# pinellolab/CRISPR-HAWK

Measured on AMD Instinct MI355X. Metric: candidate guides scored/sec, higher is better.
Workload: dtype u32

## Files before the change

### crispr-hawk_amd/csrc/hawk_api_collapse.hip

```cpp
#include <hip/hip_runtime.h>

#include <algorithm>
#include <cmath>
#include <cstdio>
#include <cstdlib>
#include <cstring>
#include <map>
#include <mutex>
#include <new>
#include <unordered_map>
#include <vector>

#include "hawk_host.h"

extern "C" {

static int collapse_rows(hawk_table* t, uint32_t flank_up, uint32_t flank_down, uint64_t* n_groups, float* kernel_ms);
static int collapse_by_templates(hawk_table* t, uint32_t flank_up, uint32_t flank_down, uint64_t* n_groups, float* kernel_ms);
int hawk_table_collapse_ex(hawk_table* t, uint32_t flank_up, uint32_t flank_down, uint64_t* n_groups, float* kernel_ms) {
  if (!t || !n_groups || !t->hs || hawk_table_stale(t)) return HAWK_E_INVALID;
  if (flank_up > HAWK_PAD || flank_down > HAWK_PAD) return HAWK_E_UNSUPPORTED;
  if (t->by_cluster && t->n_rows) return collapse_by_templates(t, flank_up, flank_down, n_groups, kernel_ms);
  return collapse_rows(t, flank_up, flank_down, n_groups, kernel_ms);
}
static int collapse_rows(hawk_table* t, uint32_t flank_up, uint32_t flank_down, uint64_t* n_groups, float* kernel_ms) {
  hawk_hapset* hs = t->hs;
  hawk_ctx* ctx = hs->ctx;
  HIPCHK(hipSetDevice(ctx->device));
  const uint64_t n = t->n_rows;
  t->collapsed = false;
  *n_groups = 0;
  if (kernel_ms) *kernel_ms = 0.f;
  hs->collapse_gen = t->gen;
  if (n == 0) { t->n_groups = 0; t->collapsed = true; return HAWK_OK; }
  if (n > 0xffffffffull || hs->max_gen - hs->min_gen > 0xffffffffll) return HAWK_E_UNSUPPORTED;
  unsigned end_bit = 32;
  while (end_bit < 64 && ((uint64_t)(hs->max_gen - hs->min_gen) >> (end_bit - 32)) != 0) ++end_bit;
  const unsigned pos_bits = end_bit - 31;
  const unsigned hash_bits = std::min(31u, (pos_bits + 24 + 7) / 8 * 8 - pos_bits);
  const unsigned begin_bit = 31 - hash_bits;
  const size_t temp_bytes = hawk_collapse_temp_bytes(n, begin_bit, end_bit);
  int rc;
  if ((rc = hs->ckeys.reserve(2 * n * 8)) || (rc = hs->cvals.reserve(2 * n * 4)) || (rc = hs->cflags.reserve(n * 4)) ||
      (rc = hs->cgidx.reserve(n * 4)) || (rc = hs->ctemp.reserve(temp_bytes + 16)) || (rc = hs->cgoff.reserve((n + 1) * 8)) ||
      (rc = hs->cgc.reserve(2 * n)) || (rc = hs->ccnt.reserve(32)))
    return rc;
  const char* ex = getenv("HAWK_COLLAPSE_EXACT");
#ifdef HAWK_TEST_HOOKS
  const char* vf = getenv("HAWK_COLLAPSE_VERIFY");
  const char* wk = getenv("HAWK_COLLAPSE_WEAK_HASH");
  const bool verify = !(vf && vf[0] == '0'), weak = wk && wk[0] == '1';
#else
  const bool verify = true, weak = false;
#endif
  bool exact = ex && ex[0] == '1';
  for (int round = 0; round < 2; ++round, exact = true) {
  if (exact && (rc = hs->cfull.reserve(hawk_collapse_full_bytes(n)))) return rc;
  bool verified_bad = false;
  {
    const char* md = getenv("HAWK_COLLAPSE_MODE");
    const bool force_hash = md && md[0] == 'h', force_sort = md && md[0] == 's';
    const uint64_t g_est = hs->last_groups ? hs->last_groups + hs->last_groups / 4 : n / 16;
    uint64_t C = 1024;
    while (C < 2 * g_est) C <<= 1;
    const bool fits = C <= (1ull << 26) && hs->max_gen - hs->min_gen < 0xffffffffll;
    const bool want = !exact && !weak && !force_sort && fits && (force_hash || (n >= (1u << 20) && (hs->last_groups == 0 || hs->last_groups * 8 <= n)));
    if (want) {
      const size_t tb = hawk_collapse_hash_temp_bytes(n, (uint32_t)C);
      if ((rc = hs->ctable.reserve(C * 16)) || (rc = hs->cocc.reserve(C * 4)) || (rc = hs->cdense.reserve(C * 4)) ||
          (rc = hs->cgkey.reserve(2 * C * 8)) || (rc = hs->cgslot.reserve(2 * C * 4)) || (rc = hs->ctemp.reserve(std::max(tb, temp_bytes) + 16)) ||
          (rc = hs->ccnt.reserve(32)))
        return rc;
      for (int attempt = 0; attempt < 2; ++attempt) {
        unsigned long long hc[4] = {0, 0, 0, 0};
        HIPCHK(hipMemsetAsync(hs->ccnt.p, 0, 32, ctx->stream));
        HIPCHK(hipEventRecord(ctx->ev[0], ctx->stream));
        if (hawk_launch_collapse_hash1(ctx->stream, t->cols, hs->d_is_ref, n, (int)t->guidelen, (int)t->pamlen, (int)flank_up, (int)flank_down,
                                       hs->min_gen, 0x9e3779b97f4a7c15ull * (uint64_t)(attempt + 1), hs->ctemp.p, tb, hs->ctable.p, (uint32_t)C,
                                       hs->cocc.as<uint32_t>(), hs->cdense.as<uint32_t>(), hs->cgkey.as<uint64_t>(), hs->cgslot.as<uint32_t>(),
                                       hs->cflags.as<uint32_t>(), hs->ccnt.as<unsigned long long>()))
          return HAWK_E_HIP;
        HIPCHK(hipGetLastError());
        HIPCHK(hipMemcpyAsync(hc, hs->ccnt.p, 24, hipMemcpyDeviceToHost, ctx->stream));
        HIPCHK(hipStreamSynchronize(ctx->stream));
        if (hc[1]) { hs->last_groups = n; if (hs->plan_groups) *hs->plan_groups = n; break; }
        if (hc[0]) continue;
        const uint64_t ng = hc[2];
        if (hawk_launch_collapse_hash2(ctx->stream, t->cols, n, (uint32_t)ng, (int)t->guidelen, (int)t->pamlen, (int)t->right, end_bit, hs->ctemp.p, tb,
                                       hs->cgkey.as<uint64_t>(), hs->cgslot.as<uint32_t>(), (uint32_t)C, hs->cocc.as<uint32_t>(),
                                       hs->cflags.as<uint32_t>(), hs->ckeys.as<uint32_t>(), hs->cvals.as<uint32_t>(), hs->cgoff.as<uint64_t>(),
                                       hs->cgc.as<uint8_t>(), hs->cgc.as<uint8_t>() + n))
          return HAWK_E_HIP;
        if (verify) {
          if ((rc = hs->cfull.reserve(ng * 64 + 64))) return rc;
          hawk_launch_collapse_verify_rows(ctx->stream, t->cols, hs->d_is_ref, n, (uint32_t)ng, (int)t->guidelen, (int)t->pamlen, (int)flank_up,
                                           (int)flank_down, hs->cvals.as<uint32_t>() + n, hs->cflags.as<uint32_t>(), hs->cocc.as<uint32_t>(),
                                           hs->cgoff.as<uint64_t>(), hs->cfull.p, hs->ccnt.as<unsigned long long>() + 3);
        }
        HIPCHK(hipEventRecord(ctx->ev[1], ctx->stream));
        HIPCHK(hipGetLastError());
        HIPCHK(hipMemcpyAsync(hs->cgoff.as<uint64_t>() + ng, &n, 8, hipMemcpyHostToDevice, ctx->stream));
        HIPCHK(hipMemcpyAsync(&hc[3], hs->ccnt.as<unsigned long long>() + 3, 8, hipMemcpyDeviceToHost, ctx->stream));
        HIPCHK(hipStreamSynchronize(ctx->stream));
        if (kernel_ms) { float ms = 0.f; (void)hipEventElapsedTime(&ms, ctx->ev[0], ctx->ev[1]); *kernel_ms += ms; }
        if (hc[3]) { verified_bad = true; break; }
        hs->last_groups = ng;
        if (hs->plan_groups) *hs->plan_groups = ng;
        t->n_groups = ng; t->collapsed = true;
        *n_groups = ng;
        return HAWK_OK;
      }
    }
  }
  if (verified_bad) continue;
  unsigned long long cnt[3] = {0, 0, 0};
  for (int attempt = 0; attempt < 4; ++attempt) {
    HIPCHK(hipMemsetAsync(hs->ccnt.p, 0, 32, ctx->stream));
    HIPCHK(hipEventRecord(ctx->ev[0], ctx->stream));
    if (hawk_launch_collapse(ctx->stream, t->cols, hs->d_is_ref, n, (int)t->guidelen, (int)t->pamlen, (int)t->right, (int)flank_up,
                             (int)flank_down, hs->min_gen, begin_bit, end_bit, 0x9e3779b97f4a7c15ull * (uint64_t)(attempt + 1), hs->ctemp.p,
                             temp_bytes, hs->ckeys.as<uint64_t>(), hs->cvals.as<uint32_t>(), hs->cflags.as<uint32_t>(),
                             hs->cgidx.as<uint32_t>(), hs->ccnt.as<unsigned long long>(), hs->cgoff.as<uint64_t>(), hs->cgc.as<uint8_t>(),
                             hs->cgc.as<uint8_t>() + n, hs->cgidx.as<uint32_t>(), exact ? hs->cfull.p : nullptr, weak && !exact))
      return HAWK_E_HIP;
    if (verify && !exact)
      hawk_launch_collapse_verify(ctx->stream, t->cols, hs->d_is_ref, n, (int)t->guidelen, (int)t->pamlen, (int)flank_up, (int)flank_down,
                                  hs->cvals.as<uint32_t>() + n, hs->cgidx.as<uint32_t>(), hs->cflags.as<uint32_t>(), hs->cgoff.as<uint64_t>(),
                                  hs->ccnt.as<unsigned long long>() + 2);
    HIPCHK(hipEventRecord(ctx->ev[1], ctx->stream));
    HIPCHK(hipGetLastError());
    HIPCHK(hipMemcpyAsync(cnt, hs->ccnt.p, 24, hipMemcpyDeviceToHost, ctx->stream));
    HIPCHK(hipStreamSynchronize(ctx->stream));
    if (kernel_ms) { float ms = 0.f; (void)hipEventElapsedTime(&ms, ctx->ev[0], ctx->ev[1]); *kernel_ms += ms; }
    if (cnt[0] == cnt[1]) break;
  }
  if (cnt[0] != cnt[1]) { if (!exact) continue; return HAWK_E_UNSUPPORTED; }
  if (cnt[2]) continue;
  const uint64_t ng = cnt[1];
  HIPCHK(hipMemcpyAsync(hs->cgoff.as<uint64_t>() + ng, &n, 8, hipMemcpyHostToDevice, ctx->stream));
  HIPCHK(hipStreamSynchronize(ctx->stream));
  hs->last_groups = ng;
  if (hs->plan_groups) *hs->plan_groups = ng;
  t->n_groups = ng; t->collapsed = true;
  *n_groups = ng;
  return HAWK_OK;
  }
  return HAWK_E_UNSUPPORTED;
}

static int collapse_by_templates(hawk_table* t, uint32_t flank_up, uint32_t flank_down, uint64_t* n_groups, float* kernel_ms) {
  hawk_hapset* hs = t->hs;
  hawk_ctx* ctx = hs->ctx;
  HIPCHK(hipSetDevice(ctx->device));
  const hawk_xplan* vx = hs->vplan;
  if (!vx || !vx->cl.usable) return HAWK_E_INVALID;
  const uint64_t n = t->n_rows;
  if (n > 0xffffffffull) return HAWK_E_UNSUPPORTED;
  t->collapsed = false;
  *n_groups = 0;
  if (kernel_ms) *kernel_ms = 0.f;
  const uint32_t nu = vx->cl.n_uniq;
  PoolScope tmp;
  uint32_t* d_ucnt;
  uint64_t* d_moff;
  unsigned long long *d_partial, *d_shards;
  ScanTotals* d_tot;
  TEMPCHK(tmp, &d_ucnt, (size_t)std::max<uint32_t>(nu, 1) * 4);
  TEMPCHK(tmp, &d_moff, ((size_t)nu + 2) * 8);
  TEMPCHK(tmp, &d_partial, ((size_t)nu / 1024 + 2) * 8);
  TEMPCHK(tmp, &d_shards, 512 * 8);
  TEMPCHK(tmp, &d_tot, sizeof(ScanTotals));
  HIPCHK(hipMemsetAsync(d_shards, 0, 512 * 8, ctx->stream));
  HIPCHK(hipMemsetAsync(d_tot, 0, sizeof(ScanTotals), ctx->stream));
  uint64_t r0 = 0;
  ScanTotals tot;
  memset(&tot, 0, sizeof(tot));
  if (nu) {
    hawk_launch_cc_ucnt(ctx->stream, hs->cs_res.p, nu, d_ucnt);
    hawk_launch_mscan(ctx->stream, d_ucnt, nu, d_partial, d_shards, d_moff, d_tot);
    HIPCHK(hipMemcpyAsync(&tot, d_tot, sizeof(tot), hipMemcpyDeviceToHost, ctx->stream));
  }
  HIPCHK(hipMemcpyAsync(&r0, hs->offsets.as<uint64_t>() + t->plane_tiles, 8, hipMemcpyDeviceToHost, ctx->stream));
  HIPCHK(hipStreamSynchronize(ctx->stream));
  HIPCHK(hipGetLastError());
  const uint64_t t_live = tot.n_keep;
  const uint64_t nm = r0 + t_live;
  if (r0 > n || nm == 0 || nm > 0xffffffffull || r0 + 0 > n) return HAWK_E_INVALID;
  int rc;
  GuideCols mini;
  if ((rc = hawk_reserve_cols(hs->cmini, nm, &mini)) || (rc = hs->cm_gid.reserve(nm * 4))) return rc;
  float ms_a = 0.f, ms_b = 0.f, ms_c = 0.f;
  HIPCHK(hipEventRecord(ctx->ev[8], ctx->stream));
  hawk_launch_cc_mini(ctx->stream, t->cols, r0, hs->cs_trows.p, t_live, d_moff, hs->cs_tbase.as<uint32_t>(), nu, hs->ref_startp, mini);
  HIPCHK(hipEventRecord(ctx->ev[9], ctx->stream));
  HIPCHK(hipGetLastError());
  {
    const size_t tb_full = hawk_collapse_expand_temp_bytes(n);
    if ((rc = hs->ckeys.reserve(std::max<size_t>(2 * nm * 8, 2 * n * 4))) || (rc = hs->cvals.reserve(2 * n * 4)) ||
        (rc = hs->cgoff.reserve((nm + 1) * 8)) || (rc = hs->cgc.reserve(2 * n)) || (rc = hs->ctemp.reserve(tb_full + 16)) ||
        (rc = hs->cflags.reserve(n * 4)))
      return rc;
  }
  hawk_table tm;
  tm.hs = hs; tm.ctx = ctx; tm.n_rows = nm; tm.n_cand = tm.n_hits = 0; tm.cap = mini.cap; tm.cols = mini;
  tm.guidelen = t->guidelen; tm.pamlen = t->pamlen; tm.right = t->right; tm.n_groups = 0; tm.collapsed = false; tm.gen = t->gen;
  uint64_t G = 0;
  if ((rc = collapse_rows(&tm, flank_up, flank_down, &G, &ms_b))) return rc;
  HIPCHK(hipStreamSynchronize(ctx->stream));
  (void)hipEventElapsedTime(&ms_a, ctx->ev[8], ctx->ev[9]);
  unsigned gbits = 1;
  while (gbits < 32 && (G >> gbits) != 0) ++gbits;
  const size_t tb = hawk_collapse_expand_temp_bytes(n);
  HIPCHK(hipEventRecord(ctx->ev[8], ctx->stream));
  hawk_launch_cc_gidm(ctx->stream, hs->cvals.as<uint32_t>() + nm, hs->cgoff.as<uint64_t>(), nm, G, hs->cm_gid.as<uint32_t>());
  if ((rc = hs->ckeys.reserve(2 * n * 4)) || (rc = hs->cvals.reserve(2 * n * 4)) || (rc = hs->cgoff.reserve((std::max<uint64_t>(G, nm) + 1) * 8)) ||
      (rc = hs->cgc.reserve(2 * n)) || (rc = hs->ctemp.reserve(tb + 16)) || (rc = hs->cflags.reserve(n * 4)))
    return rc;
  ClDict cd;
  memset(&cd, 0, sizeof(cd));
  cd.n_inst = vx->cl.n_inst; cd.n_uniq = vx->cl.n_uniq; cd.inst_uid = vx->cl.inst_uid.as<uint32_t>();
  hawk_launch_cs_gid(ctx->stream, cd, hs->cs_res.p, d_moff, hs->offsets.as<uint64_t>() + t->plane_tiles, r0, n,
                     hs->cm_gid.as<uint32_t>(), hs->ckeys.as<uint32_t>(), hs->cvals.as<uint32_t>());
  if (hawk_launch_collapse_expand(ctx->stream, t->cols, n, gbits, (int)t->guidelen, (int)t->pamlen, (int)t->right, hs->ctemp.p, tb, hs->ckeys.as<uint32_t>(),
                                  hs->cvals.as<uint32_t>(), hs->cgoff.as<uint64_t>(), hs->cgc.as<uint8_t>(), hs->cgc.as<uint8_t>() + n))
    return HAWK_E_HIP;
  HIPCHK(hipMemcpyAsync(hs->cgoff.as<uint64_t>() + G, &n, 8, hipMemcpyHostToDevice, ctx->stream));
  HIPCHK(hipEventRecord(ctx->ev[9], ctx->stream));
  HIPCHK(hipGetLastError());
  HIPCHK(hipStreamSynchronize(ctx->stream));
  (void)hipEventElapsedTime(&ms_c, ctx->ev[8], ctx->ev[9]);
  if (kernel_ms) *kernel_ms = ms_a + ms_b + ms_c;
  hs->collapse_gen = t->gen;
  hs->last_groups = G;
  if (hs->plan_groups) *hs->plan_groups = G;
  t->n_groups = G; t->collapsed = true;
  *n_groups = G;
  return HAWK_OK;
}

int hawk_table_collapse(hawk_table* t, uint64_t* n_groups, float* kernel_ms) {
  return hawk_table_collapse_ex(t, 0, 0, n_groups, kernel_ms);
}

static bool collapse_valid(const hawk_table* t) {
  return t && t->collapsed && t->hs && !hawk_table_stale(t) && t->hs->collapse_gen == t->gen;
}

int hawk_table_collapse_download(hawk_table* t, uint32_t* perm, uint64_t* group_off, uint8_t* gc_num, uint8_t* gc_den) {
  if (!collapse_valid(t)) return HAWK_E_INVALID;
  hawk_hapset* hs = t->hs;
  hawk_ctx* ctx = hs->ctx;
  HIPCHK(hipSetDevice(ctx->device));
  const uint64_t n = t->n_rows, ng = t->n_groups;
  if (n == 0) { if (group_off) group_off[0] = 0; return HAWK_OK; }
  if (perm) HIPCHK(hipMemcpyAsync(perm, hs->cvals.as<uint32_t>() + n, n * 4, hipMemcpyDefault, ctx->stream));
  if (group_off) HIPCHK(hipMemcpyAsync(group_off, hs->cgoff.p, (ng + 1) * 8, hipMemcpyDefault, ctx->stream));
  if (gc_num) HIPCHK(hipMemcpyAsync(gc_num, hs->cgc.p, ng, hipMemcpyDefault, ctx->stream));
  if (gc_den) HIPCHK(hipMemcpyAsync(gc_den, hs->cgc.as<uint8_t>() + n, ng, hipMemcpyDefault, ctx->stream));
  HIPCHK(hipStreamSynchronize(ctx->stream));
  return HAWK_OK;
}

int hawk_table_collapse_export(hawk_table* t, uint32_t* rep_row, uint32_t* pos, uint8_t* strand, int64_t* start, int64_t* stop,
                               uint8_t* flags, double* cfdon, uint64_t* win, uint32_t* member_hap, float* kernel_ms) {
  if (!collapse_valid(t)) return HAWK_E_INVALID;
  hawk_hapset* hs = t->hs;
  hawk_ctx* ctx = hs->ctx;
  HIPCHK(hipSetDevice(ctx->device));
  const uint64_t n = t->n_rows, ng = t->n_groups;
  if (kernel_ms) *kernel_ms = 0.f;
  if (n == 0) return HAWK_OK;
  GuideCols rep;
  int rc = hawk_reserve_cols(hs->crep, ng, &rep);
  if (rc) return rc;
  uint32_t* d_mem = hs->cflags.as<uint32_t>();
  HIPCHK(hipEventRecord(ctx->ev[0], ctx->stream));
  hawk_launch_collapse_export(ctx->stream, t->cols, n, ng, hs->cvals.as<uint32_t>() + n, hs->cgoff.as<uint64_t>(), rep, d_mem);
  HIPCHK(hipEventRecord(ctx->ev[1], ctx->stream));
  HIPCHK(hipGetLastError());
  hipStream_t st = ctx->stream;
  if (rep_row) HIPCHK(hipMemcpyAsync(rep_row, rep.hap, ng * 4, hipMemcpyDefault, st));
  if (pos) HIPCHK(hipMemcpyAsync(pos, rep.pos, ng * 4, hipMemcpyDefault, st));
  if (strand) HIPCHK(hipMemcpyAsync(strand, rep.strand, ng, hipMemcpyDefault, st));
  if (start) HIPCHK(hipMemcpyAsync(start, rep.start, ng * 8, hipMemcpyDefault, st));
  if (stop) HIPCHK(hipMemcpyAsync(stop, rep.stop, ng * 8, hipMemcpyDefault, st));
  if (flags) HIPCHK(hipMemcpyAsync(flags, rep.flags, ng, hipMemcpyDefault, st));
  if (cfdon) HIPCHK(hipMemcpyAsync(cfdon, rep.cfdon, ng * 8, hipMemcpyDefault, st));
  if (win)
    for (int p = 0; p < HAWK_PLANES; ++p)
      HIPCHK(hipMemcpyAsync(win + (size_t)p * ng, rep.win + (size_t)p * rep.cap, ng * 8, hipMemcpyDefault, st));
  if (member_hap) HIPCHK(hipMemcpyAsync(member_hap, d_mem, n * 4, hipMemcpyDefault, st));
  HIPCHK(hipStreamSynchronize(st));
  if (kernel_ms) (void)hipEventElapsedTime(kernel_ms, ctx->ev[0], ctx->ev[1]);
  return HAWK_OK;
}


}
```

### crispr-hawk_amd/csrc/hawk_api_search.hip

```cpp
#include <hip/hip_runtime.h>

#include <algorithm>
#include <cmath>
#include <cstdio>
#include <cstdlib>
#include <cstring>
#include <map>
#include <mutex>
#include <new>
#include <unordered_map>
#include <vector>

#include "hawk_host.h"

int hawk_reserve_cols(DevBuf (&b)[8], uint64_t cap, GuideCols* c) {
  int rc;
  const size_t sz[8] = {cap * 4, cap * 4, cap, cap * 8, cap * 8, cap, cap * 8, cap * 8 * HAWK_PLANES};
  for (int i = 0; i < 8; ++i) if ((rc = b[i].reserve(std::max<size_t>(sz[i], 16)))) return rc;
  c->hap = b[0].as<uint32_t>(); c->pos = b[1].as<uint32_t>(); c->strand = b[2].as<uint8_t>();
  c->start = b[3].as<int64_t>(); c->stop = b[4].as<int64_t>(); c->flags = b[5].as<uint8_t>();
  c->cfdon = b[6].as<double>(); c->win = b[7].as<uint64_t>(); c->cap = cap;
  c->rows = nullptr; c->startp = 0;
  return HAWK_OK;
}
extern "C" {

#define HAWK_RETRY_TEMPLATES (-100)
static int hawk_search_once(hawk_hapset* hs, const hawk_search_params* p, hawk_table** out, hawk_timing* timing);
int hawk_search(hawk_hapset* hs, const hawk_search_params* p, hawk_table** out, hawk_timing* timing) {
  int rc = hawk_search_once(hs, p, out, timing);
  if (rc == HAWK_RETRY_TEMPLATES) rc = hawk_search_once(hs, p, out, timing);
  return rc == HAWK_RETRY_TEMPLATES ? HAWK_E_CAPACITY : rc;
}
static int hawk_search_once(hawk_hapset* hs, const hawk_search_params* p, hawk_table** out, hawk_timing* timing) {
  if (!hs || !p || !out || !hs->has_meta) return HAWK_E_INVALID;
  if (p->score_cfdon > 2) return HAWK_E_INVALID;
  if (p->score_cfdon && (p->right || !p->cfd_mm || !p->cfd_pam || p->pamlen < 2)) return HAWK_E_INVALID;
  hawk_ctx* ctx = hs->ctx;
  HIPCHK(hipSetDevice(ctx->device));
  ScanParams sp;
  int rc = make_scan_params(hs, p->pam_fwd, p->pam_rev, p->pamlen, p->guidelen, p->right, true, &sp);
  if (rc) return rc;
  const HapSetDev d = make_dev(hs);
  ++hs->cols_gen;
  const uint64_t ntile = (uint64_t)hs->n_hap * sp.bph;
  bool by_cluster = hs->vplan && hs->vplan->cl.built && hs->vplan->cl.usable && hs->ref_index == 0;
  if (by_cluster) { const char* e = getenv("HAWK_VIEW_SEARCH"); if (e && e[0] == 'w') by_cluster = false; }
  const uint64_t nscan = by_cluster ? (uint64_t)sp.bph + ((uint64_t)hs->vplan->cl.n_inst + 63) / 64 : ntile;
  if ((rc = hs->counts.reserve(nscan * 4)) || (rc = hs->offsets.reserve((nscan + 1) * 8)) ||
      (rc = hs->misc.reserve(512 * 8 + 64)) ||
      (rc = hs->cfd.reserve(336 * 8)) || (rc = hs->partial.reserve((nscan / 1024 + 2) * 8)))
    return rc;
  const hawk_xplan* vx = hs->vplan;
  const uint32_t plane_tiles = vx ? sp.bph * (hs->ref_index == 0 ? 1u : 0u) : (uint32_t)ntile;
  if (vx && (hs->ref_index != 0 || hs->n_ref_rows != 1)) return HAWK_E_INVALID;
  const uint64_t n_ref_tiles = (uint64_t)sp.bph * hs->n_ref_rows;
  if ((rc = hs->lists.reserve((size_t)plane_tiles * HAWK_LIST_CAP * 4 + 16)) || (rc = hs->big.reserve(((size_t)plane_tiles + 128 * n_ref_tiles) * 8 + 16))) return rc;
  uint32_t* const d_lists = hs->lists.as<uint32_t>();
  unsigned long long* const d_big = hs->big.as<unsigned long long>();
  if (p->score_cfdon) {
    if (hs->cfd_host.size() != 336 || memcmp(hs->cfd_host.data(), p->cfd_mm, 320 * 8) != 0 ||
        memcmp(hs->cfd_host.data() + 320, p->cfd_pam, 16 * 8) != 0) {
      hs->cfd_host.assign(336, 0.0);
      memcpy(hs->cfd_host.data(), p->cfd_mm, 320 * 8);
      memcpy(hs->cfd_host.data() + 320, p->cfd_pam, 16 * 8);
      HIPCHK(hipMemcpyAsync(hs->cfd.p, hs->cfd_host.data(), 336 * 8, hipMemcpyHostToDevice, ctx->stream));
      HIPCHK(hipStreamSynchronize(ctx->stream));
    }
  }
  HIPCHK(hipMemsetAsync(hs->misc.p, 0, 512 * 8 + 64, ctx->stream));
  unsigned long long* d_shards = hs->misc.as<unsigned long long>();
  int* d_status = reinterpret_cast<int*>(hs->misc.as<char>() + 512 * 8);
  uint32_t* d_big_count = reinterpret_cast<uint32_t*>(hs->misc.as<char>() + 512 * 8 + 16);
  unsigned long long* d_tcount = reinterpret_cast<unsigned long long*>(hs->misc.as<char>() + 512 * 8 + 8);
  static_assert(sizeof(ScanTotals) == 32, "status block layout");
  ScanTotals* d_totals = reinterpret_cast<ScanTotals*>(hs->misc.as<char>() + 512 * 8 + 32);
  const char* d_block = hs->misc.as<char>() + 512 * 8;
  char* h_block = static_cast<char*>(ctx->pinned);
  GuideParams gp;
  gp.pamlen = sp.pamlen; gp.guidelen = sp.guidelen; gp.right = sp.right; gp.L = sp.L;
  gp.score_cfdon = (int32_t)p->score_cfdon;
  gp.cfd_mm = hs->cfd.as<double>(); gp.cfd_pam = hs->cfd.as<double>() + 320; gp.bph = sp.bph;
  RefInfo ri;
  ri.index = hs->ref_index; ri.startp = hs->ref_startp;
  for (int s = 0; s < 2; ++s) {
    ri.lo[s] = 0; ri.hi[s] = 0;
    if (hs->ref_index >= 0) {
      const bool pamfirst = (sp.right != 0) != (s != 0);
      const int po = pamfirst ? 0 : sp.guidelen;
      const int haplen = (int)hs->hap_len[hs->ref_index];
      const int rs = hs->has_partner ? hs->partner_start : hs->scan_start[hs->ref_index];
      const int re = hs->has_partner ? hs->partner_stop : hs->scan_stop[hs->ref_index];
      ri.lo[s] = std::max(rs - po, HAWK_PAD);
      ri.hi[s] = std::min(re - po, haplen - sp.L - HAWK_PAD + 1);
    }
  }
  ri.bits[0] = ri.bits[1] = nullptr;
  ri.n_bits = 0;
  if (hs->ref_index >= 0) {
    const uint64_t key[6] = {p->pam_fwd, p->pam_rev, ((uint64_t)p->pamlen << 32) | p->guidelen, (uint64_t)(p->right ? 1 : 0),
                             ((uint64_t)(uint32_t)ri.lo[0] << 32) | (uint32_t)ri.hi[0], ((uint64_t)(uint32_t)ri.lo[1] << 32) | (uint32_t)ri.hi[1]};
    if ((rc = hs->refbits.reserve((size_t)hs->S * 4 * 2))) return rc;
    ri.bits[0] = hs->refbits.as<uint32_t>();
    ri.bits[1] = hs->refbits.as<uint32_t>() + hs->S;
    ri.n_bits = hs->S * 32u;
    if (vx && ((rc = hs->refhp.reserve(((size_t)hs->S + 1) * 8 * 2)) || (rc = hs->vcnt0.reserve(by_cluster ? 16 : ntile * 4)))) return rc;
    if (!hs->refbits_valid || memcmp(hs->refbits_key, key, sizeof(key)) != 0) {
      hawk_launch_ref_bits(ctx->stream, d, sp, ri, hs->refbits.as<uint32_t>(), hs->refbits.as<uint32_t>() + hs->S);
      if (vx) hawk_launch_ref_hits(ctx->stream, d, sp, hs->ref_index, hs->refhp.p);
      HIPCHK(hipGetLastError());
      memcpy(hs->refbits_key, key, sizeof(key));
      hs->refbits_valid = true;
    }
  }
  VcArgs va;
  memset(&va, 0, sizeof(va));
  if (vx) {
    for (int pl = 0; pl < 4; ++pl) va.ref[pl] = vx->ref5[pl].as<uint32_t>();
    va.ref_S = hs->S;
    va.recs_ = vx->recs.p; va.alt_codes = vx->codes.as<uint8_t>(); va.hv_off = vx->off.as<uint64_t>(); va.tiles_ = vx->tiles.p;
    va.hp = hs->refhp.as<uint4>();
  }
  const uint32_t v_tiles = vx ? (uint32_t)ntile - plane_tiles : 0u;
  ClDict cd;
  memset(&cd, 0, sizeof(cd));
  uint64_t tcap = 0, t_rows_used = 0;
  if (by_cluster) {
    const auto& cl = vx->cl;
    cd.n_inst = cl.n_inst; cd.n_uniq = cl.n_uniq;
    cd.inst_uid = cl.inst_uid.as<uint32_t>(); cd.inst_o = cl.inst_o.as<int32_t>(); cd.inst_row = cl.inst_row.as<uint32_t>();
    cd.inst_pa = cl.inst_pa.as<int32_t>(); cd.inst_rb = cl.inst_rb.as<int32_t>();
    cd.u_rec = cl.u_rec.as<uint32_t>(); cd.u_n = cl.u_n.as<uint32_t>(); cd.u_row = cl.u_row.as<uint32_t>(); cd.u_o = cl.u_o.as<int32_t>();
    cd.u_seg = cl.u_seg.as<uint32_t>();
    const char* e0 = getenv("HAWK_CLUSTER_ROWS0");
    const uint64_t first = e0 ? strtoull(e0, nullptr, 10) : 16ull * cl.n_uniq + 65536;
    tcap = std::max<uint64_t>(std::min<uint64_t>(cl.slots, std::max<uint64_t>(hs->cs_tcap, first)), 1);
    if ((rc = hs->cs_res.reserve((size_t)std::max<uint32_t>(cl.n_uniq, 1) * 32)) || (rc = hs->cs_tbase.reserve((size_t)std::max<uint32_t>(cl.n_uniq, 1) * 4)) ||
        (rc = hs->cs_trows.reserve((size_t)tcap * hawk_cs_row_bytes())) || (rc = hs->cs_itb.reserve((size_t)std::max<uint32_t>(cl.n_inst, 1) * 4)) ||
        (rc = hs->cs_icnt.reserve((size_t)std::max<uint32_t>(cl.n_inst, 1) * 4)))
      return rc;
  }
  uint32_t* const d_counts_v = hs->counts.as<uint32_t>() + plane_tiles;
  auto view_count = [&]() {
    if (by_cluster) {
      hawk_launch_cs_templates(ctx->stream, d, va, cd, sp, gp, ri, hs->cs_res.p, hs->cs_tbase.as<uint32_t>(), hs->cs_trows.p, d_tcount, tcap, d_status);
      (void)hipEventRecord(ctx->ev[8], ctx->stream);
      hawk_launch_cs_count(ctx->stream, d, va, cd, sp, hs->cs_res.p, d_tcount, tcap, d_counts_v, hs->cs_icnt.as<uint32_t>(),
                           hs->cs_itb.as<uint32_t>(), d_shards);
    } else {
      hawk_launch_vsearch(ctx->stream, 0, d, va, sp, gp, ri, hs->d_tile_meta, hs->counts.as<uint32_t>(), hs->vcnt0.as<uint32_t>(), d_shards, nullptr,
                          GuideCols{}, d_status, plane_tiles, v_tiles);
    }
  };
  const uint64_t stage_cap = by_cluster ? 2ull * hs->hap_len[hs->ref_index] + 64 : 0;
  auto emit_all = [&](const GuideCols& cols, const GuideCols& packed) {
    hawk_launch_search(ctx->stream, 1, d, sp, gp, ri, hs->d_tile_meta, hs->counts.as<uint32_t>(), d_shards,
                       hs->offsets.as<uint64_t>(), cols, d_status, d_lists, d_big_count, d_big, ctx->ev[5], plane_tiles);
    if (!vx) return;
    (void)hipEventRecord(ctx->ev[7], ctx->stream);
    if (by_cluster) {
      hawk_launch_rows_pack(ctx->stream, cols, hs->offsets.as<uint64_t>() + plane_tiles, 0, std::min<uint64_t>(stage_cap, packed.cap), packed.rows,
                            packed.startp, d_status);
      (void)hipEventRecord(ctx->ev[9], ctx->stream);
      hawk_launch_cs_emit_rows(ctx->stream, cd, hs->cs_icnt.as<uint32_t>(), hs->cs_itb.as<uint32_t>(), hs->cs_trows.p, hs->offsets.as<uint64_t>() + plane_tiles,
                               d_tcount, tcap, packed.rows, packed.cap, d_status);
    } else {
      hawk_launch_vsearch(ctx->stream, 1, d, va, sp, gp, ri, hs->d_tile_meta, hs->counts.as<uint32_t>(), hs->vcnt0.as<uint32_t>(), d_shards,
                          hs->offsets.as<uint64_t>(), cols, d_status, plane_tiles, v_tiles);
    }
  };
  auto reserve_table = [&](uint64_t cap, GuideCols* cols, GuideCols* table) -> int {
    int r;
    if (!by_cluster) {
      if ((r = hawk_reserve_cols(hs->colsA, cap, cols))) return r;
      *table = *cols;
      return HAWK_OK;
    }
    if ((r = hawk_reserve_cols(hs->colsA, stage_cap, cols)) || (r = hs->rowsA.reserve(cap * 64))) return r;
    memset(table, 0, sizeof(*table));
    table->rows = hs->rowsA.as<uint4>(); table->cap = cap; table->startp = ri.startp;
    return HAWK_OK;
  };
  uint64_t& table_cap = by_cluster ? hs->rows_cap : hs->cols_cap;
  GuideCols none = {};
  hipEvent_t* ev = ctx->ev;
  HIPCHK(hipEventRecord(ev[0], ctx->stream));
  hawk_launch_search(ctx->stream, 0, d, sp, gp, ri, hs->d_tile_meta, hs->counts.as<uint32_t>(), d_shards, nullptr, none, d_status, d_lists, d_big_count, d_big,
                     nullptr, plane_tiles);
  if (vx) HIPCHK(hipEventRecord(ev[6], ctx->stream));
  if (vx) view_count();
  HIPCHK(hipEventRecord(ev[1], ctx->stream));
  hawk_launch_mscan(ctx->stream, hs->counts.as<uint32_t>(), nscan, hs->partial.as<unsigned long long>(), d_shards,
                    hs->offsets.as<uint64_t>(), d_totals);
  HIPCHK(hipEventRecord(ev[2], ctx->stream));
  HIPCHK(hipGetLastError());
  ScanTotals tot;
  GuideCols ca, tc;
  int status = 0;
  uint64_t nrows = 0;
  bool emitted = false;
  auto read_block = [&]() -> int {
    HIPCHK(hipMemcpyAsync(h_block, d_block, 64, hipMemcpyDeviceToHost, ctx->stream));
    HIPCHK(hipStreamSynchronize(ctx->stream));
    memcpy(&tot, h_block + 32, sizeof(tot));
    memcpy(&status, h_block, 4);
    if (!by_cluster) return HAWK_OK;
    uint64_t tcu;
    memcpy(&tcu, h_block + 8, 8);
    if (tcu > tcap) { hs->cs_tcap = std::min<uint64_t>(vx->cl.slots, tcu + tcu / 8 + 64); return HAWK_RETRY_TEMPLATES; }
    t_rows_used = tcu;
    return HAWK_OK;
  };
  if (table_cap) {
    if ((rc = reserve_table(table_cap, &ca, &tc))) return rc;
    HIPCHK(hipEventRecord(ev[3], ctx->stream));
    emit_all(ca, tc);
    HIPCHK(hipEventRecord(ev[4], ctx->stream));
    HIPCHK(hipGetLastError());
    if ((rc = read_block())) return rc;
    nrows = tot.n_keep;
    emitted = nrows <= table_cap;
    if (!emitted) {
      if (status && status != HAWK_E_CAPACITY) return status;
      status = 0;
      HIPCHK(hipMemsetAsync(d_status, 0, 4, ctx->stream));
    }
  } else {
    if ((rc = read_block())) return rc;
    if (status) return status;
    nrows = tot.n_keep;
  }
  if (!emitted) {
    if ((rc = reserve_table(std::max<uint64_t>(std::max<uint64_t>(nrows, 1), table_cap), &ca, &tc))) return rc;
    table_cap = tc.cap;
    HIPCHK(hipEventRecord(ev[3], ctx->stream));
    if (nrows) emit_all(ca, tc);
    HIPCHK(hipEventRecord(ev[4], ctx->stream));
    HIPCHK(hipGetLastError());
    HIPCHK(hipMemcpyAsync(h_block, d_status, 4, hipMemcpyDeviceToHost, ctx->stream));
    HIPCHK(hipStreamSynchronize(ctx->stream));
    memcpy(&status, h_block, 4);
  }
  if (timing) {
    memset(timing, 0, sizeof(*timing));
    (void)hipEventElapsedTime(&timing->count_ms, ev[0], ev[1]);
    (void)hipEventElapsedTime(&timing->offsets_ms, ev[1], ev[2]);
    (void)hipEventElapsedTime(&timing->emit_ms, ev[3], ev[4]);
    if (nrows) (void)hipEventElapsedTime(&timing->emit_list_ms, ev[3], ev[5]);
    (void)hipEventElapsedTime(&timing->total_ms, ev[0], ev[4]);
    if (vx) {
      (void)hipEventElapsedTime(&timing->v_count_ms, ev[6], ev[1]);
      if (nrows) (void)hipEventElapsedTime(&timing->v_emit_ms, ev[7], ev[4]);
      timing->v_path = by_cluster ? 2u : 1u;
      if (by_cluster) (void)hipEventElapsedTime(&timing->v_templates_ms, ev[6], ev[8]);
      if (by_cluster && nrows) (void)hipEventElapsedTime(&timing->v_emit_rows_ms, ev[9], ev[4]);
    }
    uint64_t pos = 0;
    for (uint32_t h = 0; h < hs->n_hap; ++h) pos += (uint64_t)std::max(0, hs->scan_stop[h] - hs->scan_start[h]);
    timing->scanned_positions = pos;
  }
  if (status) return status;
  hawk_table* t = new (std::nothrow) hawk_table();
  if (!t) return HAWK_E_INVALID;
  t->hs = hs; t->ctx = ctx; t->gen = hs->cols_gen;
  t->n_rows = nrows; t->n_cand = tot.n_cand; t->n_hits = tot.n_hits; t->cols = tc; t->cap = tc.cap;
  t->guidelen = p->guidelen; t->pamlen = p->pamlen; t->right = p->right ? 1 : 0; t->n_groups = 0; t->collapsed = false;
  t->by_cluster = by_cluster; t->plane_tiles = plane_tiles; t->t_rows = by_cluster ? t_rows_used : 0;
  *out = t;
  return HAWK_OK;
}

void hawk_table_destroy(hawk_table* t) {
  if (!t) return;
  if (!t->hs) {
    (void)hipSetDevice(t->ctx->device);
    (void)hipStreamSynchronize(t->ctx->stream);
    for (auto& b : t->own) b.release();
  }
  delete t;
}

int hawk_table_counts(const hawk_table* t, uint64_t* n_rows, uint64_t* n_candidates, uint64_t* n_hits) {
  if (!t) return HAWK_E_INVALID;
  if (n_rows) *n_rows = t->n_rows;
  if (n_candidates) *n_candidates = t->n_cand;
  if (n_hits) *n_hits = t->n_hits;
  return HAWK_OK;
}

int hawk_table_download(hawk_table* t, uint32_t* hap, uint32_t* pos, uint8_t* strand, int64_t* start, int64_t* stop,
                        uint8_t* flags, double* cfdon, uint64_t* win) {
  if (!t || hawk_table_stale(t)) return HAWK_E_INVALID;
  hawk_ctx* ctx = t->ctx;
  HIPCHK(hipSetDevice(ctx->device));
  const uint64_t n = t->n_rows;
  if (!n) return HAWK_OK;
  GuideCols c = t->cols;
  PoolScope tmp;
  if (c.rows) {
    GuideCols u;
    memset(&u, 0, sizeof(u));
    u.cap = n;
    if (hap) TEMPCHK(tmp, &u.hap, n * 4);
    if (pos) TEMPCHK(tmp, &u.pos, n * 4);
    if (strand) TEMPCHK(tmp, &u.strand, n);
    if (start) TEMPCHK(tmp, &u.start, n * 8);
    if (stop) TEMPCHK(tmp, &u.stop, n * 8);
    if (flags) TEMPCHK(tmp, &u.flags, n);
    if (cfdon) TEMPCHK(tmp, &u.cfdon, n * 8);
    if (win) TEMPCHK(tmp, &u.win, n * 8 * HAWK_PLANES);
    hawk_launch_rows_unpack(ctx->stream, c.rows, n, c.startp, u);
    HIPCHK(hipGetLastError());
    c = u;
  }
  if (hap) HIPCHK(hipMemcpyAsync(hap, c.hap, n * 4, hipMemcpyDefault, ctx->stream));
  if (pos) HIPCHK(hipMemcpyAsync(pos, c.pos, n * 4, hipMemcpyDefault, ctx->stream));
  if (strand) HIPCHK(hipMemcpyAsync(strand, c.strand, n, hipMemcpyDefault, ctx->stream));
  if (start) HIPCHK(hipMemcpyAsync(start, c.start, n * 8, hipMemcpyDefault, ctx->stream));
  if (stop) HIPCHK(hipMemcpyAsync(stop, c.stop, n * 8, hipMemcpyDefault, ctx->stream));
  if (flags) HIPCHK(hipMemcpyAsync(flags, c.flags, n, hipMemcpyDefault, ctx->stream));
  if (cfdon) HIPCHK(hipMemcpyAsync(cfdon, c.cfdon, n * 8, hipMemcpyDefault, ctx->stream));
  if (win)
    for (int p = 0; p < HAWK_PLANES; ++p)
      HIPCHK(hipMemcpyAsync(win + (size_t)p * n, c.win + (size_t)p * c.cap, n * 8, hipMemcpyDefault, ctx->stream));
  HIPCHK(hipStreamSynchronize(ctx->stream));
  return HAWK_OK;
}

int hawk_table_layout(const hawk_table* t, uint32_t* layout, int64_t* startp) {
  if (!t || !layout) return HAWK_E_INVALID;
  *layout = t->cols.rows ? HAWK_LAYOUT_ROWS : HAWK_LAYOUT_COLUMNS;
  if (startp) *startp = t->cols.rows ? t->cols.startp : 0;
  return HAWK_OK;
}

int hawk_table_download_rows(hawk_table* t, void* rows64) {
  if (!t || hawk_table_stale(t) || !rows64) return HAWK_E_INVALID;
  if (!t->cols.rows) return HAWK_E_UNSUPPORTED;
  HIPCHK(hipSetDevice(t->ctx->device));
  if (t->n_rows) HIPCHK(hipMemcpyAsync(rows64, t->cols.rows, t->n_rows * 64, hipMemcpyDefault, t->ctx->stream));
  HIPCHK(hipStreamSynchronize(t->ctx->stream));
  return HAWK_OK;
}

int hawk_table_device_rows(hawk_table* t, void** rows64, int64_t* startp) {
  if (!t || hawk_table_stale(t) || !rows64) return HAWK_E_INVALID;
  if (!t->cols.rows) return HAWK_E_UNSUPPORTED;
  *rows64 = t->cols.rows;
  if (startp) *startp = t->cols.startp;
  return HAWK_OK;
}

int hawk_table_device_columns(hawk_table* t, void** hap, void** pos, void** strand, void** start, void** stop,
                              void** flags, void** cfdon, void** win, uint64_t* win_plane_stride) {
  if (!t || hawk_table_stale(t)) return HAWK_E_INVALID;
  const GuideCols& c = t->cols;
  if (c.rows) return HAWK_E_UNSUPPORTED;
  if (hap) *hap = c.hap;
  if (pos) *pos = c.pos;
  if (strand) *strand = c.strand;
  if (start) *start = c.start;
  if (stop) *stop = c.stop;
  if (flags) *flags = c.flags;
  if (cfdon) *cfdon = c.cfdon;
  if (win) *win = c.win;
  if (win_plane_stride) *win_plane_stride = c.cap;
  return HAWK_OK;
}

}
```

### crispr-hawk_amd/csrc/hawk_api_xplan.hip

```cpp
#include <hip/hip_runtime.h>

#include <algorithm>
#include <cmath>
#include <cstdio>
#include <cstdlib>
#include <cstring>
#include <map>
#include <mutex>
#include <new>
#include <unordered_map>
#include <vector>

#include "hawk_host.h"

extern "C" {

void hawk_xplan_destroy(hawk_xplan* x) {
  if (!x) return;
  (void)hipSetDevice(x->ctx->device);
  (void)hipStreamSynchronize(x->ctx->stream);
  for (auto& p : x->ref_plane) hawk_pool_free(p);
  for (auto& b : x->ref5) b.release();
  DevBuf* bufs[] = {&x->recs, &x->heads, &x->tiles, &x->codes, &x->off, &x->hlen, &x->hash,
                    &x->m_is_ref, &x->m_ss, &x->m_se, &x->m_seg_off, &x->m_seg_rel, &x->m_seg_gen, &x->m_tile,
                    &x->cl.inst_uid, &x->cl.inst_o, &x->cl.inst_row, &x->cl.inst_pa, &x->cl.inst_rb, &x->cl.u_rec, &x->cl.u_n, &x->cl.u_row,
                    &x->cl.u_o, &x->cl.u_seg};
  for (auto* b : bufs) b->release();
  delete x;
}

static int xplan_build(hawk_hapset* ref_set, uint32_t n_var, const uint32_t* v_r0, const uint32_t* v_span, const uint32_t* v_alt_off,
                       const uint32_t* v_alt_len, const uint8_t* alt_codes, uint32_t alt_codes_len, uint32_t n_hap, const uint64_t* hv_off,
                       const uint32_t* d_idx, const int32_t* d_o, const uint32_t* hap_len, uint32_t maxlen, hawk_xplan** out) {
  hawk_ctx* ctx = ref_set->ctx;
  const uint32_t ref_len = ref_set->hap_len[0];
  const uint64_t ncar = hv_off[n_hap];
  HIPCHK(hipSetDevice(ctx->device));
  hawk_xplan* x = new (std::nothrow) hawk_xplan();
  if (!x) return HAWK_E_INVALID;
  x->ctx = ctx; x->n_var = n_var; x->n_hap = n_hap; x->ref_len = ref_len; x->ncar = ncar;
  x->hap_len.assign(hap_len, hap_len + n_hap);
  x->has_meta = false; x->nseg = 0; x->ref_index = -1; x->ref_startp = 0; x->min_gen = 0; x->max_gen = 0;
  for (auto& p : x->ref_plane) p = nullptr;
  x->ref_S = ref_set->S;
  x->S = ((maxlen + 31) / 32 + 2 + 3) / 4 * 4;
  x->bph = (x->S / 4 + HAWK_BLOCK - 1) / HAWK_BLOCK;
  const size_t nwg = (size_t)n_hap * hawk_hx_tiles_per_row(x->S);
  const size_t nv = std::max<size_t>(n_var, 1), nc = std::max<size_t>(ncar, 1);
  int rc = HAWK_OK;
  for (int p = 0; p < 4 && !rc; ++p) rc = hawk_pool_alloc((void**)&x->ref_plane[p], (size_t)x->ref_S * 4);
  DevBuf t_r0, t_span, t_ao, t_al, t_am;
  DevBuf* temps[] = {&t_r0, &t_span, &t_ao, &t_al, &t_am};
  if (!rc) rc = t_r0.reserve(nv * 4);
  if (!rc) rc = t_span.reserve(nv * 4);
  if (!rc) rc = t_ao.reserve(nv * 4);
  if (!rc) rc = t_al.reserve(nv * 4);
  if (!rc) rc = t_am.reserve(nv * 16);
  if (!rc) rc = x->recs.reserve(nc * hawk_hx_record_bytes());
  if (!rc) rc = x->heads.reserve(nc * 16);
  if (!rc) rc = x->tiles.reserve(nwg * hawk_hx_tile_bytes());
  if (!rc) rc = x->codes.reserve(std::max<size_t>(alt_codes_len, 1));
  if (!rc) rc = x->off.reserve((size_t)(n_hap + 1) * 8);
  if (!rc) rc = x->hlen.reserve((size_t)n_hap * 4);
  if (!rc) rc = x->hash.reserve((size_t)n_hap * 16);
  for (int p = 0; p < HAWK_PLANES && !rc; ++p) rc = x->ref5[p].reserve((size_t)x->S * 4);
  if (rc) { for (auto* b : temps) b->release(); hawk_xplan_destroy(x); return rc; }
  hipStream_t st = ctx->stream;
  hipError_t e = hipSuccess;
  for (int p = 0; p < HAWK_PLANES && e == hipSuccess; ++p) {
    e = hipMemsetAsync(x->ref5[p].p, 0, (size_t)x->S * 4, st);
    if (p < 4 && e == hipSuccess)
      e = hipMemcpyAsync(x->ref5[p].p, ref_set->plane[p], (size_t)std::min(x->S, x->ref_S) * 4, hipMemcpyDeviceToDevice, st);
  }
  std::vector<uint32_t> am(nv * 4, 0);
  for (uint32_t i = 0; i < n_var; ++i)
    for (uint32_t j = 0; j < v_alt_len[i] && j < 32; ++j) {
      const uint8_t c = alt_codes[v_alt_off[i] + j];
      for (int pl = 0; pl < 4; ++pl) am[(size_t)i * 4 + pl] |= (uint32_t)((c >> pl) & 1u) << j;
    }
  for (int p = 0; p < 4 && e == hipSuccess; ++p)
    e = hipMemcpyAsync(x->ref_plane[p], ref_set->plane[p], (size_t)x->ref_S * 4, hipMemcpyDeviceToDevice, st);
  if (n_var && e == hipSuccess) {
    e = hipMemcpyAsync(t_r0.p, v_r0, (size_t)n_var * 4, hipMemcpyHostToDevice, st);
    if (e == hipSuccess) e = hipMemcpyAsync(t_span.p, v_span, (size_t)n_var * 4, hipMemcpyHostToDevice, st);
    if (e == hipSuccess) e = hipMemcpyAsync(t_ao.p, v_alt_off, (size_t)n_var * 4, hipMemcpyHostToDevice, st);
    if (e == hipSuccess) e = hipMemcpyAsync(t_al.p, v_alt_len, (size_t)n_var * 4, hipMemcpyHostToDevice, st);
    if (e == hipSuccess) e = hipMemcpyAsync(x->codes.p, alt_codes, alt_codes_len, hipMemcpyHostToDevice, st);
    if (e == hipSuccess) e = hipMemcpyAsync(t_am.p, am.data(), (size_t)n_var * 16, hipMemcpyHostToDevice, st);
  }
  if (e == hipSuccess) e = hipMemcpyAsync(x->off.p, hv_off, (size_t)(n_hap + 1) * 8, hipMemcpyHostToDevice, st);
  if (e == hipSuccess) e = hipMemcpyAsync(x->hlen.p, hap_len, (size_t)n_hap * 4, hipMemcpyHostToDevice, st);
  if (e == hipSuccess) {
    hawk_launch_hx_prepare(st, x->off.as<uint64_t>(), d_idx, d_o, ncar, t_r0.as<uint32_t>(), t_span.as<uint32_t>(), t_ao.as<uint32_t>(),
                           t_al.as<uint32_t>(), t_am.p, x->hlen.as<uint32_t>(), n_hap, x->S, x->recs.p, x->tiles.p);
    hawk_launch_hx_heads(st, x->recs.p, d_idx, ncar, x->heads.p);
    e = hipGetLastError();
  }
  if (e == hipSuccess) e = hipStreamSynchronize(st);
  for (auto* b : temps) b->release();
  if (e != hipSuccess) {
    snprintf(hawk_hip_err_buf(), 256, "hawk_xplan_create_gt: %s", hipGetErrorString(e));
    hawk_xplan_destroy(x);
    return HAWK_E_HIP;
  }
  *out = x;
  return HAWK_OK;
}

int hawk_xplan_set_ref_partner_range(hawk_xplan* x, int32_t start, int32_t stop) {
  if (!x || !x->has_meta || x->ref_index < 0) return HAWK_E_INVALID;
  if (start < 0 || stop > (int32_t)x->hap_len[x->ref_index] || stop < start) return HAWK_E_INVALID;
  x->has_partner = true; x->partner_start = start; x->partner_stop = stop;
  return HAWK_OK;
}

static int xplan_install(const hawk_xplan* x, hawk_hapset* hs) {
  if (!x->has_meta || hs->n_hap != x->n_hap || hs->S != x->S) return HAWK_E_INVALID;
  hipStream_t st = x->ctx->stream;
  const uint32_t n = x->n_hap;
  hawk_pool_free(hs->d_seg_rel); hs->d_seg_rel = nullptr;
  hawk_pool_free(hs->d_seg_gen); hs->d_seg_gen = nullptr;
  int rc = hawk_pool_alloc((void**)&hs->d_seg_rel, (size_t)x->nseg * 4);
  if (!rc) rc = hawk_pool_alloc((void**)&hs->d_seg_gen, (size_t)x->nseg * 8);
  if (rc) return rc;
  HIPCHK(hipMemcpyAsync(hs->d_is_ref, x->m_is_ref.p, n, hipMemcpyDeviceToDevice, st));
  HIPCHK(hipMemcpyAsync(hs->d_scan_start, x->m_ss.p, (size_t)n * 4, hipMemcpyDeviceToDevice, st));
  HIPCHK(hipMemcpyAsync(hs->d_scan_stop, x->m_se.p, (size_t)n * 4, hipMemcpyDeviceToDevice, st));
  HIPCHK(hipMemcpyAsync(hs->d_seg_off, x->m_seg_off.p, (size_t)(n + 1) * 4, hipMemcpyDeviceToDevice, st));
  HIPCHK(hipMemcpyAsync(hs->d_seg_rel, x->m_seg_rel.p, (size_t)x->nseg * 4, hipMemcpyDeviceToDevice, st));
  HIPCHK(hipMemcpyAsync(hs->d_seg_gen, x->m_seg_gen.p, (size_t)x->nseg * 8, hipMemcpyDeviceToDevice, st));
  HIPCHK(hipMemcpyAsync(hs->d_tile_meta, x->m_tile.p, (size_t)n * x->bph * sizeof(TileMeta), hipMemcpyDeviceToDevice, st));
  hs->ref_startp = x->ref_startp; hs->min_gen = x->min_gen; hs->max_gen = x->max_gen;
  hs->scan_start = x->scan_start; hs->scan_stop = x->scan_stop;
  hs->ref_index = x->ref_index; hs->has_meta = true; hs->n_ref_rows = x->n_ref_rows;
  hs->plan_groups = x->groups; hs->last_groups = *x->groups;
  hs->has_partner = x->has_partner; hs->partner_start = x->partner_start; hs->partner_stop = x->partner_stop;
  hs->refbits_valid = false;
  ++hs->cols_gen;
  return HAWK_OK;
}

int hawk_xplan_run(hawk_xplan* x, hawk_hapset** out, uint64_t* hash_out, float* kernel_ms) {
  if (!x || !out) return HAWK_E_INVALID;
  hawk_ctx* ctx = x->ctx;
  hawk_hapset* hs = nullptr;
  int rc = hapset_create_impl(ctx, x->n_hap, x->hap_len.data(), false, &hs);
  if (rc) return rc;
  if (hs->S != x->S) { hawk_hapset_destroy(hs); return HAWK_E_INVALID; }
  hipStream_t st = ctx->stream;
  hipError_t e = hipMemsetAsync(x->hash.p, 0, (size_t)x->n_hap * 16, st);
  if (e == hipSuccess) e = hipEventRecord(ctx->ev[0], st);
  if (e == hipSuccess) {
    hawk_launch_hx_build(st, x->ref_plane, x->ref_S, x->recs.p, x->codes.as<uint8_t>(), x->off.as<uint64_t>(), hs->d_hap_len, x->n_hap,
                         hs->S, hs->plane, x->tiles.p);
    if (hash_out) hawk_launch_hx_hash(st, hs->plane, x->n_hap, hs->S, x->hash.as<unsigned long long>());
    e = hipEventRecord(ctx->ev[1], st);
  }
  if (e == hipSuccess) e = hipGetLastError();
  if (e == hipSuccess && hash_out) e = hipMemcpyAsync(hash_out, x->hash.p, (size_t)x->n_hap * 16, hipMemcpyDeviceToHost, st);
  if (e == hipSuccess && x->has_meta) {
    rc = xplan_install(x, hs);
    if (rc) { hawk_hapset_destroy(hs); return rc; }
  }
  if (e == hipSuccess && (hash_out || kernel_ms)) e = hipStreamSynchronize(st);
  if (e != hipSuccess) {
    snprintf(hawk_hip_err_buf(), 256, "hawk_xplan_run: %s", hipGetErrorString(e));
    hawk_hapset_destroy(hs);
    return HAWK_E_HIP;
  }
  if (kernel_ms) (void)hipEventElapsedTime(kernel_ms, ctx->ev[0], ctx->ev[1]);
  *out = hs;
  return HAWK_OK;
}

static int xplan_build_dict(hawk_xplan* x) {
  auto& cl = x->cl;
  if (cl.built) return HAWK_OK;
  cl.built = true; cl.usable = false; cl.status = 0; cl.n_inst = cl.n_uniq = cl.n_real = 0; cl.slots = 0; cl.build_ms = 0.f;
  hawk_ctx* ctx = x->ctx;
  hipStream_t st = ctx->stream;
  const uint32_t n = x->n_hap;
  if (x->ncar == 0 || x->ncar >= (1ull << 32) - 2 || n < 2) { cl.status = 4; return HAWK_OK; }
  PoolScope tmp;
  const uint32_t n_var = x->n_var;
  const uint32_t ch_bound = hawk_cl_chunk_bound(x->ncar, n);
  const uint32_t inst_bound = (uint32_t)x->ncar + n;
  const uint32_t bm_words = n_var / 32 + 1;
  uint32_t tsize = 1024;
  while (tsize < 2u * inst_bound && tsize < (1u << 30)) tsize <<= 1;
  uint32_t tsmall = std::min<uint32_t>(1u << 16, tsize);
  { const uint64_t expect = cl.last_uniq ? (uint64_t)cl.last_uniq * 2 : (uint64_t)inst_bound / 8; while (tsmall < expect && tsmall < tsize) tsmall <<= 1; }
  const uint32_t u_bound0 = n_var + std::min<uint32_t>(tsmall, inst_bound);
  auto up = [](size_t v) { return (v + 255) & ~(size_t)255; };
  const size_t z_status = 0, z_counters = 256, z_results = 512, z_cnt = 768,
               z_claim = z_cnt + up(((size_t)ch_bound + 4) * 8), z_vdesc = z_claim + up((size_t)bm_words * 4),
               z_span2 = z_vdesc + up((size_t)std::max<uint32_t>(n_var, 1) * 8), z_tab = z_span2 + up((size_t)u_bound0 * 4),
               z_end = z_tab + (size_t)tsmall * hawk_cl_slot_bytes();
  char* d_zero;
  TEMPCHK(tmp, &d_zero, z_end);
  uint32_t* const d_status = reinterpret_cast<uint32_t*>(d_zero + z_status);
  uint32_t* const d_counters = reinterpret_cast<uint32_t*>(d_zero + z_counters);
  unsigned long long* const d_results = reinterpret_cast<unsigned long long*>(d_zero + z_results);
  uint32_t* const d_cnt = reinterpret_cast<uint32_t*>(d_zero + z_cnt);
  uint32_t* const d_lcnt = d_cnt + ((ch_bound + 3) & ~3u);
  uint32_t* const d_claim = reinterpret_cast<uint32_t*>(d_zero + z_claim);
  void* const d_vdesc = d_zero + z_vdesc;
  uint32_t *d_ch_off, *d_ch_row, *d_base, *d_lbase, *d_state;
  void* d_list;
  TEMPCHK(tmp, &d_ch_off, (size_t)(n + 1) * 4);
  TEMPCHK(tmp, &d_ch_row, (size_t)ch_bound * 4);
  TEMPCHK(tmp, &d_base, (size_t)(ch_bound + 1) * 4);
  TEMPCHK(tmp, &d_lbase, (size_t)(ch_bound + 1) * 4);
  TEMPCHK(tmp, &d_list, (size_t)inst_bound * hawk_cl_listed_bytes());
  TEMPCHK(tmp, &d_state, (size_t)inst_bound * 4);
  int rc;
  if ((rc = cl.inst_uid.reserve((size_t)inst_bound * 4)) || (rc = cl.inst_o.reserve((size_t)inst_bound * 4)) ||
      (rc = cl.inst_row.reserve((size_t)inst_bound * 4)) || (rc = cl.inst_pa.reserve((size_t)inst_bound * 4)) ||
      (rc = cl.inst_rb.reserve((size_t)inst_bound * 4)))
    return rc;
  uint32_t* const t_uid = cl.inst_uid.as<uint32_t>();
  uint32_t* const t_row = cl.inst_row.as<uint32_t>();
  int32_t* const t_o = cl.inst_o.as<int32_t>();
  int32_t* const t_pa = cl.inst_pa.as<int32_t>();
  int32_t* const t_rb = cl.inst_rb.as<int32_t>();
  HIPCHK(hipEventRecord(ctx->ev[8], st));
  HIPCHK(hipMemsetAsync(d_zero, 0, z_end, st));
  hawk_launch_cl_chunks(st, x->off.as<uint64_t>(), x->m_is_ref.as<uint8_t>(), x->m_ss.as<int32_t>(), x->m_se.as<int32_t>(), n, d_ch_off, d_ch_row);
  hawk_launch_cl_count(st, x->heads.p, x->off.as<uint64_t>(), x->hlen.as<uint32_t>(), x->m_ss.as<int32_t>(), x->m_se.as<int32_t>(), d_ch_off, d_ch_row, n,
                       n_var, ch_bound, d_cnt, d_lcnt);
  hawk_launch_scan2_u32(st, d_cnt, d_lcnt, ch_bound, d_base, d_lbase);
  const uint32_t* const d_n_inst = d_base + ch_bound;
  const uint32_t* const d_n_list = d_lbase + ch_bound;
  unsigned long long res[8] = {0, 0, 0, 0, 0, 0, 0, 0};
  uint32_t status = 0, n_inst = 0, n_uniq = 0, n_real = 0;
  auto pass = [&](uint32_t tsz, uint32_t max_probe, uint32_t fail_bit, bool first) -> int {
    const uint32_t u_bound = n_var + std::min<uint32_t>(tsz, inst_bound);
    uint32_t* d_span2 = reinterpret_cast<uint32_t*>(d_zero + z_span2);
    void* d_tab = d_zero + z_tab;
    if (!first) {
      TEMPCHK(tmp, &d_span2, (size_t)u_bound * 4);
      TEMPCHK(tmp, &d_tab, (size_t)tsz * hawk_cl_slot_bytes());
      HIPCHK(hipMemsetAsync(d_tab, 0, (size_t)tsz * hawk_cl_slot_bytes(), st));
      HIPCHK(hipMemsetAsync(d_span2, 0, (size_t)u_bound * 4, st));
      HIPCHK(hipMemsetAsync(d_zero + z_counters, 0, z_cnt - z_counters, st));
      HIPCHK(hipMemsetAsync(d_zero + z_claim, 0, z_span2 - z_claim, st));
    }
    int rc2;
    if ((rc2 = cl.u_rec.reserve((size_t)u_bound * 4)) || (rc2 = cl.u_n.reserve((size_t)u_bound * 4)) || (rc2 = cl.u_row.reserve((size_t)u_bound * 4)) ||
        (rc2 = cl.u_o.reserve((size_t)u_bound * 4)) || (rc2 = cl.u_seg.reserve((size_t)u_bound * 4)))
      return rc2;
    hawk_launch_cl_fill(st, x->heads.p, x->off.as<uint64_t>(), x->hlen.as<uint32_t>(), x->m_ss.as<int32_t>(), x->m_se.as<int32_t>(), n, d_ch_off, d_ch_row,
                        ch_bound, d_base, d_lbase, t_o, t_row, t_pa, t_rb, t_uid, d_vdesc, d_claim, n_var, d_list, d_status);
    hawk_launch_cl_finish(st, inst_bound, d_n_inst, d_n_list, d_counters, d_results, n_var, u_bound, d_tab, tsz - 1, max_probe, fail_bit, d_list, d_state, d_vdesc, x->heads.p,
                          t_uid, t_row, x->m_seg_off.as<uint32_t>(), x->m_seg_rel.as<uint32_t>(), cl.u_rec.as<uint32_t>(), cl.u_n.as<uint32_t>(),
                          cl.u_row.as<uint32_t>(), cl.u_o.as<int32_t>(), cl.u_seg.as<uint32_t>(), d_span2, d_status);
    HIPCHK(hipMemcpyAsync(res, d_results, 64, hipMemcpyDeviceToHost, st));
    HIPCHK(hipEventRecord(ctx->ev[9], st));
    HIPCHK(hipStreamSynchronize(st));
    HIPCHK(hipGetLastError());
    n_inst = (uint32_t)res[0]; status = (uint32_t)res[4];
    n_uniq = std::min<uint32_t>(n_var + (uint32_t)res[1], u_bound);
    n_real = (uint32_t)(res[1] + res[2]);
    return HAWK_OK;
  };
  if ((rc = pass(tsmall, tsmall < tsize ? 64u : 0xffffffffu, tsmall < tsize ? 8u : 2u, true))) return rc;
  if (status & 8u) {
    status &= ~8u;
    HIPCHK(hipMemcpyAsync(d_status, &status, 4, hipMemcpyHostToDevice, st));
    if ((rc = pass(tsize, 0xffffffffu, 2u, false))) return rc;
  }
  if (n_inst == 0) { cl.status = 4; return HAWK_OK; }
  if (n_inst > inst_bound) { snprintf(hawk_hip_err_buf(), 256, "hawk_xplan_view: instance count beyond its bound"); return HAWK_E_HIP; }
  cl.n_inst = n_inst; cl.n_uniq = n_uniq; cl.n_real = n_real; cl.last_uniq = (uint32_t)res[1];
  (void)hipEventElapsedTime(&cl.build_ms, ctx->ev[8], ctx->ev[9]);
  cl.slots = n_uniq ? res[3] : 0;
  cl.status = status;
  const char* e1 = getenv("HAWK_CLUSTER_MAX_SLOTS");
  const char* e2 = getenv("HAWK_CLUSTER_MIN_SHARE");
  const uint64_t max_slots = e1 ? strtoull(e1, nullptr, 10) : (1ull << 27);
  const double min_share = e2 ? atof(e2) : 3.0;
  if (!status && (cl.slots > max_slots || (double)n_inst < min_share * (double)std::max<uint32_t>(n_real, 1))) cl.status = 4;
  cl.usable = cl.status == 0;
  return HAWK_OK;
}

int hawk_xplan_cluster_stats(const hawk_xplan* x, uint32_t* usable, uint32_t* n_instances, uint32_t* n_distinct, uint64_t* template_slots,
                             float* build_ms, uint32_t* status) {
  if (!x) return HAWK_E_INVALID;
  if (usable) *usable = x->cl.built && x->cl.usable ? 1u : 0u;
  if (n_instances) *n_instances = x->cl.n_inst;
  if (n_distinct) *n_distinct = x->cl.n_real;
  if (template_slots) *template_slots = x->cl.slots;
  if (build_ms) *build_ms = x->cl.build_ms;
  if (status) *status = x->cl.built ? x->cl.status : 0xffffffffu;
  return HAWK_OK;
}

int hawk_xplan_cluster_rebuild(hawk_xplan* x) {
  if (!x || !x->has_meta || x->ref_index != 0) return HAWK_E_INVALID;
  HIPCHK(hipSetDevice(x->ctx->device));
  x->cl.built = false;
  return xplan_build_dict(x);
}

int hawk_xplan_view(hawk_xplan* x, hawk_hapset** out) {
  if (!x || !out || !x->has_meta || x->ref_index != 0) return HAWK_E_INVALID;
  hawk_ctx* ctx = x->ctx;
  hawk_hapset* hs = nullptr;
  int rc = hapset_create_impl(ctx, x->n_hap, x->hap_len.data(), false, &hs, false);
  if (rc) return rc;
  if (hs->S != x->S) { hawk_hapset_destroy(hs); return HAWK_E_INVALID; }
  hs->vplan = x;
  for (int p = 0; p < HAWK_PLANES; ++p) hs->plane[p] = x->ref5[p].as<uint32_t>();
  rc = xplan_install(x, hs);
  if (!rc && hipStreamSynchronize(ctx->stream) != hipSuccess) rc = HAWK_E_HIP;
  if (!rc) rc = xplan_build_dict(x);
  if (rc) { hs->vplan = nullptr; for (int p = 0; p < HAWK_PLANES; ++p) hs->plane[p] = nullptr; hawk_hapset_destroy(hs); return rc; }
  *out = hs;
  return HAWK_OK;
}

int hawk_xplan_install_meta(hawk_xplan* x, hawk_hapset* hs) {
  if (!x || !hs || hs->vplan) return HAWK_E_INVALID;
  HIPCHK(hipSetDevice(x->ctx->device));
  int rc = xplan_install(x, hs);
  if (rc) return rc;
  HIPCHK(hipStreamSynchronize(x->ctx->stream));
  return HAWK_OK;
}

int hawk_xplan_create_gt(hawk_hapset* ref_set, hawk_gt* g, uint32_t n_var, const uint32_t* v_r0, const uint32_t* v_span,
                         const uint32_t* v_alt_off, const uint32_t* v_alt_len, const int32_t* v_chain, const uint8_t* alt_codes,
                         uint32_t alt_codes_len, int64_t startp, int check_clamp, int64_t rev_g0, int64_t rev_g1, uint32_t* n_hap_out,
                         hawk_xplan** out) {
  if (!ref_set || !g || !out || !n_hap_out || !g->d_col_off || g->n_var != n_var || !n_var || !v_r0 || !v_span || !v_alt_off || !v_alt_len ||
      !v_chain || !alt_codes)
    return HAWK_E_INVALID;
  hawk_ctx* ctx = ref_set->ctx;
  if (g->ctx != ctx) return HAWK_E_INVALID;
  const uint32_t ref_len = ref_set->hap_len[0];
  for (uint32_t i = 0; i < n_var; ++i) {
    if ((uint64_t)v_r0[i] + v_span[i] > ref_len || v_span[i] == 0 || v_alt_len[i] == 0) return HAWK_E_INVALID;
    if ((uint64_t)v_alt_off[i] + v_alt_len[i] > alt_codes_len) return HAWK_E_INVALID;
    if (i && v_r0[i] < v_r0[i - 1]) return HAWK_E_INVALID;
    if ((int64_t)v_chain[i] != (int64_t)v_alt_len[i] - (int64_t)v_span[i]) return HAWK_E_INVALID;
  }
  const uint32_t n_cols = 2 * g->n_samples;
  std::vector<uint64_t> hv_off(2, 0), ioff(2, 0);
  std::vector<uint32_t> hap_len(1, ref_len);
  uint32_t maxlen = ref_len;
  for (uint32_t c = 0; c < n_cols; ++c) {
    if (g->h_off[c + 1] == g->h_off[c]) continue;
    const int64_t len = (int64_t)ref_len + g->h_delta[c];
    if (len <= 0 || len >= (int64_t)((1u << 31) - 256)) return HAWK_E_UNSUPPORTED;
    hv_off.push_back(g->h_off[c + 1]);
    ioff.push_back(g->h_ioff[c + 1]);
    hap_len.push_back((uint32_t)len);
    maxlen = std::max(maxlen, (uint32_t)len);
  }
  const uint32_t n_hap = (uint32_t)hap_len.size();
  *n_hap_out = n_hap;
  hawk_xplan* x = nullptr;
  int rc = xplan_build(ref_set, n_var, v_r0, v_span, v_alt_off, v_alt_len, alt_codes, alt_codes_len, n_hap, hv_off.data(), g->d_idx, g->d_o,
                       hap_len.data(), maxlen, &x);
  if (rc) return rc;
  hipStream_t st = ctx->stream;
  DevBuf t_r0, t_span, t_ch, t_ioff, t_cnt, t_status, t_rev;
  DevBuf* temps[] = {&t_r0, &t_span, &t_ch, &t_ioff, &t_cnt, &t_status, &t_rev};
  auto done = [&](int code) { for (auto* b : temps) b->release(); if (code) hawk_xplan_destroy(x); return code; };
  if ((rc = t_r0.reserve((size_t)n_var * 4)) || (rc = t_span.reserve((size_t)n_var * 4)) || (rc = t_ch.reserve((size_t)n_var * 4)) ||
      (rc = t_ioff.reserve((size_t)(n_hap + 1) * 8)) || (rc = t_cnt.reserve((size_t)n_hap * 4)) || (rc = t_status.reserve(16)) ||
      (rc = t_rev.reserve((size_t)n_hap * 16)) || (rc = x->m_seg_off.reserve((size_t)(n_hap + 1) * 4)))
    return done(rc);
#define HIPCHK_X(expr)                                                                         \
  do {                                                                                         \
    hipError_t e_ = (expr);                                                                    \
    if (e_ != hipSuccess) {                                                                    \
      snprintf(hawk_hip_err_buf(), 256, "%s: %s (%s:%d)", #expr, hipGetErrorString(e_), __FILE__, __LINE__); \
      return done(HAWK_E_HIP);                                                                 \
    }                                                                                          \
  } while (0)
  HIPCHK_X(hipMemcpyAsync(t_r0.p, v_r0, (size_t)n_var * 4, hipMemcpyHostToDevice, st));
  HIPCHK_X(hipMemcpyAsync(t_span.p, v_span, (size_t)n_var * 4, hipMemcpyHostToDevice, st));
  HIPCHK_X(hipMemcpyAsync(t_ch.p, v_chain, (size_t)n_var * 4, hipMemcpyHostToDevice, st));
  HIPCHK_X(hipMemcpyAsync(t_ioff.p, ioff.data(), (size_t)(n_hap + 1) * 8, hipMemcpyHostToDevice, st));
  HIPCHK_X(hipMemsetAsync(t_status.p, 0, 16, st));
  hawk_launch_list_check(st, x->off.as<uint64_t>(), n_hap, g->d_idx, g->d_o, t_r0.as<int32_t>(), t_span.as<int32_t>(), t_ch.as<int32_t>(), n_var,
                         ref_len, check_clamp, t_status.as<uint32_t>());
  hawk_launch_segments(st, t_ioff.as<uint64_t>(), g->d_indel, g->d_idx, g->d_o, t_r0.as<int32_t>(), t_ch.as<int32_t>(), x->hlen.as<uint32_t>(), n_hap,
                       startp, t_cnt.as<uint32_t>(), x->m_seg_off.as<uint32_t>(), nullptr, nullptr);
  HIPCHK_X(hipGetLastError());
  uint32_t status = 0, nseg = 0;
  HIPCHK_X(hipMemcpyAsync(&status, t_status.p, 4, hipMemcpyDeviceToHost, st));
  HIPCHK_X(hipMemcpyAsync(&nseg, x->m_seg_off.as<uint32_t>() + n_hap, 4, hipMemcpyDeviceToHost, st));
  HIPCHK_X(hipStreamSynchronize(st));
  if (status & 4u) return done(HAWK_E_INVALID);
  if (status & 1u) return done(HAWK_E_OVERLAP);
  if (status & 2u) return done(HAWK_E_CLAMP);
  if ((rc = x->m_seg_rel.reserve((size_t)nseg * 4)) || (rc = x->m_seg_gen.reserve((size_t)nseg * 8))) return done(rc);
  hawk_launch_segments(st, t_ioff.as<uint64_t>(), g->d_indel, g->d_idx, g->d_o, t_r0.as<int32_t>(), t_ch.as<int32_t>(), x->hlen.as<uint32_t>(), n_hap,
                       startp, t_cnt.as<uint32_t>(), x->m_seg_off.as<uint32_t>(), x->m_seg_rel.as<uint32_t>(), x->m_seg_gen.as<int64_t>());
  hawk_launch_rev_lookup(st, x->m_seg_off.as<uint32_t>(), x->m_seg_rel.as<uint32_t>(), x->m_seg_gen.as<int64_t>(), x->hlen.as<uint32_t>(), n_hap,
                         rev_g0, rev_g1, t_rev.as<int64_t>(), t_rev.as<int64_t>() + n_hap);
  HIPCHK_X(hipGetLastError());
  x->rev0.resize(n_hap); x->rev1.resize(n_hap);
  HIPCHK_X(hipMemcpyAsync(x->rev0.data(), t_rev.p, (size_t)n_hap * 8, hipMemcpyDeviceToHost, st));
  HIPCHK_X(hipMemcpyAsync(x->rev1.data(), t_rev.as<int64_t>() + n_hap, (size_t)n_hap * 8, hipMemcpyDeviceToHost, st));
  HIPCHK_X(hipStreamSynchronize(st));
#undef HIPCHK_X
  x->nseg = nseg; x->ref_startp = startp;
  x->min_gen = startp; x->max_gen = startp + (int64_t)ref_len;
  (void)done(HAWK_OK);
  *out = x;
  return HAWK_OK;
}

int hawk_xplan_rows(hawk_xplan* x, uint32_t* hap_len, int64_t* rev0, int64_t* rev1) {
  if (!x) return HAWK_E_INVALID;
  if (hap_len) memcpy(hap_len, x->hap_len.data(), (size_t)x->n_hap * 4);
  if ((rev0 || rev1) && x->rev0.size() != x->n_hap) return HAWK_E_INVALID;
  if (rev0) memcpy(rev0, x->rev0.data(), (size_t)x->n_hap * 8);
  if (rev1) memcpy(rev1, x->rev1.data(), (size_t)x->n_hap * 8);
  return HAWK_OK;
}

int hawk_xplan_finish_meta(hawk_xplan* x, const int32_t* scan_start, const int32_t* scan_stop) {
  if (!x || !scan_start || !scan_stop || !x->nseg) return HAWK_E_INVALID;
  hawk_ctx* ctx = x->ctx;
  HIPCHK(hipSetDevice(ctx->device));
  const uint32_t n = x->n_hap;
  for (uint32_t h = 0; h < n; ++h)
    if (scan_start[h] < 0 || scan_stop[h] > (int32_t)x->hap_len[h]) return HAWK_E_INVALID;
  int rc;
  if ((rc = x->m_is_ref.reserve(n)) || (rc = x->m_ss.reserve((size_t)n * 4)) || (rc = x->m_se.reserve((size_t)n * 4)) ||
      (rc = x->m_tile.reserve((size_t)n * x->bph * sizeof(TileMeta))))
    return rc;
  hipStream_t st = ctx->stream;
  std::vector<uint8_t> is_ref(n, 0);
  is_ref[0] = 1;
  HIPCHK(hipMemcpyAsync(x->m_is_ref.p, is_ref.data(), n, hipMemcpyHostToDevice, st));
  HIPCHK(hipMemcpyAsync(x->m_ss.p, scan_start, (size_t)n * 4, hipMemcpyHostToDevice, st));
  HIPCHK(hipMemcpyAsync(x->m_se.p, scan_stop, (size_t)n * 4, hipMemcpyHostToDevice, st));
  hawk_launch_tile_meta(st, x->m_seg_off.as<uint32_t>(), x->m_seg_rel.as<uint32_t>(), x->hlen.as<uint32_t>(), x->m_is_ref.as<uint8_t>(),
                        x->m_ss.as<int32_t>(), x->m_se.as<int32_t>(), n, x->bph, x->m_tile.as<TileMeta>());
  HIPCHK(hipGetLastError());
  HIPCHK(hipStreamSynchronize(st));
  x->scan_start.assign(scan_start, scan_start + n);
  x->scan_stop.assign(scan_stop, scan_stop + n);
  x->ref_index = 0; x->n_ref_rows = 1; x->has_meta = true; x->cl.built = false; x->cl.usable = false;
  return HAWK_OK;
}

int hawk_xplan_segments(hawk_xplan* x, uint32_t* seg_off, uint32_t* seg_rel, int64_t* seg_gen, uint64_t cap, uint64_t* n_seg) {
  if (!x || !x->nseg) return HAWK_E_INVALID;
  if (n_seg) *n_seg = x->nseg;
  if (!seg_off && !seg_rel && !seg_gen) return HAWK_OK;
  if (cap < x->nseg) return HAWK_E_CAPACITY;
  hawk_ctx* ctx = x->ctx;
  HIPCHK(hipSetDevice(ctx->device));
  if (seg_off) HIPCHK(hipMemcpyAsync(seg_off, x->m_seg_off.p, (size_t)(x->n_hap + 1) * 4, hipMemcpyDeviceToHost, ctx->stream));
  if (seg_rel) HIPCHK(hipMemcpyAsync(seg_rel, x->m_seg_rel.p, (size_t)x->nseg * 4, hipMemcpyDeviceToHost, ctx->stream));
  if (seg_gen) HIPCHK(hipMemcpyAsync(seg_gen, x->m_seg_gen.p, (size_t)x->nseg * 8, hipMemcpyDeviceToHost, ctx->stream));
  HIPCHK(hipStreamSynchronize(ctx->stream));
  return HAWK_OK;
}


}
```

### crispr-hawk_amd/csrc/hawk_csearch.hip

```cpp
#include "hawk_vc.h"

#define CL_LINK 64
#define CL_NONE 0xffffffffu
#define CL_FAR (1 << 29)
#define CL_MAXWALK 4096
#define CS_G 8

struct __attribute__((aligned(16))) CsRow { uint4 a, b, c, d; };
static_assert(sizeof(CsRow) == 64, "template row layout");
size_t hawk_cs_row_bytes() { return sizeof(CsRow); }

__device__ __forceinline__ uint64_t cl_mix(uint64_t h, uint64_t v) {
  h = (h ^ v) * 0x9E3779B97F4A7C15ull;
  return h ^ (h >> 29);
}
struct __attribute__((aligned(16))) HxHead { int32_t o; uint32_t rs; uint32_t alt_len; uint32_t var; };
static_assert(sizeof(HxHead) == 16, "record head layout");
__global__ __launch_bounds__(256) void k_hx_heads(const HxVar* __restrict__ recs, const uint32_t* __restrict__ hv_idx, uint64_t n, uint4* __restrict__ heads) {
  const uint64_t j = (uint64_t)blockIdx.x * 256 + threadIdx.x;
  if (j >= n) return;
  const uint4 r = *reinterpret_cast<const uint4*>(recs + j);
  heads[j] = make_uint4(r.x, r.y, r.z, hv_idx[j]);
}
void hawk_launch_hx_heads(hipStream_t st, const void* recs, const uint32_t* hv_idx, uint64_t n, void* heads) {
// ... 80 lines not shown
    h = cl_mix(h, (uint64_t)r.w | ((uint64_t)r.z << 32));
    h = cl_mix(h, (uint64_t)r.y | ((uint64_t)(uint32_t)((int32_t)r.x - c.o_first) << 32));
    c.o_end = (int32_t)r.x + (int32_t)r.z;
    ++c.n; ++e;
    open = e < hi;
  }
#ifdef HAWK_TEST_HOOKS
  if (cl_weak_hash) h = h_first;
#endif
  const bool outside = c.o_end <= ss - 44 || c.o_first - 43 >= se;
  const bool interior = c.o_first - 43 >= (ss > HAWK_PAD ? ss : HAWK_PAD) && c.o_first >= 64 && c.o_end <= se - 44 &&
                        c.o_end <= hl - 44 - HAWK_PAD + 1 && c.o_end + 128 <= hl;
  c.key = h; c.cls = 1;
  if (outside) { c.cls = 0; c.key = 0; }
  else if (!interior) { c.cls = 2; c.key = cl_mix(h ^ 0xA4093822299F31D0ull, (uint64_t)row + 1u); }
  if (c.cls && c.key == 0) c.key = 1;
  c.run_inside = c.pa >= (ss > HAWK_PAD ? ss : HAWK_PAD) && c.o_first <= se - 44 && c.o_first <= hl - 44 - HAWK_PAD + 1;
  return c;
}
__device__ __forceinline__ uint4 shfl_down4(const uint4& v, int d) {
  return make_uint4((uint32_t)__shfl_down((int)v.x, d), (uint32_t)__shfl_down((int)v.y, d), (uint32_t)__shfl_down((int)v.z, d),
                    (uint32_t)__shfl_down((int)v.w, d));
}

__global__ __launch_bounds__(256) void k_cl_count(const HxHead* __restrict__ recs, const uint64_t* __restrict__ hv_off, const uint32_t* __restrict__ hap_len,
                                                  const int32_t* __restrict__ ss_, const int32_t* __restrict__ se_, const uint32_t* __restrict__ ch_off,
                                                  const uint32_t* __restrict__ ch_row, uint32_t n_rows, uint32_t n_var, uint32_t* __restrict__ cnt,
                                                  uint32_t* __restrict__ lcnt) {
  __shared__ uint32_t s_w[256 / WAVE];
  const uint32_t b = blockIdx.x;
  if (b >= ch_off[n_rows]) return;
  const uint32_t row = ch_row[b];
  const uint64_t lo = hv_off[row], hi = hv_off[row + 1];
  const uint64_t b0 = lo + (uint64_t)(b - ch_off[row]) * CL_CHUNK;
  const int32_t ss = ss_[row], se = se_[row], hl = (int32_t)hap_len[row];
  const uint32_t lane = threadIdx.x & (WAVE - 1);
  uint32_t c = 0;
  if (hi > lo) {
    uint4 r0[CL_ROW_U], rp[CL_ROW_U];
#pragma unroll
    for (int u = 0; u < CL_ROW_U; ++u) {
      const uint64_t j = b0 + u * 256 + threadIdx.x;
      const uint64_t jc = j < hi ? j : hi - 1;
      r0[u] = *reinterpret_cast<const uint4*>(recs + jc);
      rp[u] = *reinterpret_cast<const uint4*>(recs + (jc > lo ? jc - 1 : jc));
    }
    auto one = [&](const int u) __attribute__((always_inline)) {
      const uint4 nx1 = shfl_down4(r0[u], 1), nx2 = shfl_down4(r0[u], 2);
      const uint64_t j = b0 + u * 256 + threadIdx.x;
      if (!(j < hi && (j == lo || (int32_t)r0[u].x - ((int32_t)rp[u].x + (int32_t)rp[u].z) > CL_LINK))) return;
      const ClCut k = cl_cut(recs, lo, hi, j, r0[u], rp[u], nx1, nx2, lane, ss, se, hl, row);
      const bool simple = k.n == 1 && k.cls == 1 && r0[u].w < n_var;
      c += 1u + ((k.cls != 0 && !simple) ? 0x10000u : 0u);
    };
    static_assert(CL_ROW_U == 4, "one call per slice");
    one(0); one(1); one(2); one(3);
  }
  uint32_t tot;
  (void)block_excl_scan<256 / WAVE>(c, s_w, &tot);
  if (threadIdx.x == 0) { cnt[b] = (tot & 0xffffu) + (b + 1 == ch_off[row + 1] ? 1u : 0u); lcnt[b] = tot >> 16; }
}

#define CL_BM_WORDS 4096
__global__ __launch_bounds__(256) void k_cl_fill(const HxHead* __restrict__ recs, const uint64_t* __restrict__ hv_off,
                                                 const uint32_t* __restrict__ hap_len, const int32_t* __restrict__ ss_,
                                                 const int32_t* __restrict__ se_, const uint32_t* __restrict__ ch_off,
                                                 const uint32_t* __restrict__ ch_row, const uint32_t* __restrict__ inst_base,
                                                 const uint32_t* __restrict__ list_base, ClInst ci, unsigned long long* __restrict__ var_desc,
                                                 uint32_t* claim_bits, uint32_t n_var, ClListed* __restrict__ cx_list, uint32_t* __restrict__ status,
                                                 uint32_t b_first, uint32_t n_rows, uint32_t head) {
  __shared__ uint32_t s_c[256 / WAVE][CL_ROW_U];
  __shared__ uint32_t s_l[256 / WAVE][CL_ROW_U];
  __shared__ uint32_t s_bm[CL_BM_WORDS];
  const uint32_t b = b_first + blockIdx.x;
  if (b >= ch_off[n_rows]) return;
  const uint32_t row = ch_row[b];
  const uint64_t lo = hv_off[row], hi = hv_off[row + 1];
  const uint64_t b0 = lo + (uint64_t)(b - ch_off[row]) * CL_CHUNK;
  const int32_t ss = ss_[row], se = se_[row], hl = (int32_t)hap_len[row];
  const uint32_t lane = threadIdx.x & (WAVE - 1), wv = threadIdx.x / WAVE;
  const uint32_t at = inst_base[b], lat = list_base[b];
  uint32_t round_tot = 0;
  if (hi > lo) {
    const uint64_t b1 = b0 + CL_CHUNK < hi ? b0 + CL_CHUNK : hi;
    const uint32_t v_lo = recs[b0].var, v_hi = recs[b1 - 1].var;
    const uint32_t w_lo = v_lo >> 5, n_w = v_hi >= v_lo && v_hi < n_var ? (v_hi >> 5) - w_lo + 1u : 0u;
    const bool bm_lds = !head && n_w != 0u && n_w <= CL_BM_WORDS;
    if (bm_lds) for (uint32_t w = threadIdx.x; w < n_w; w += 256) s_bm[w] = claim_bits[w_lo + w];
    uint4 r0[CL_ROW_U], rp[CL_ROW_U];
    bool st[CL_ROW_U];
    unsigned long long bal[CL_ROW_U];
#pragma unroll
    for (int u = 0; u < CL_ROW_U; ++u) {
      const uint64_t j = b0 + u * 256 + threadIdx.x;
      const uint64_t jc = j < hi ? j : hi - 1;
      r0[u] = *reinterpret_cast<const uint4*>(recs + jc);
      rp[u] = *reinterpret_cast<const uint4*>(recs + (jc > lo ? jc - 1 : jc));
    }
#pragma unroll
    for (int u = 0; u < CL_ROW_U; ++u) {
      const uint64_t j = b0 + u * 256 + threadIdx.x;
      st[u] = j < hi && (j == lo || (int32_t)r0[u].x - ((int32_t)rp[u].x + (int32_t)rp[u].z) > CL_LINK);
      bal[u] = __ballot(st[u]);
      if (lane == 0) s_c[wv][u] = (uint32_t)__popcll(bal[u]);
    }
    __syncthreads();
    uint32_t pre[CL_ROW_U];
#pragma unroll
    for (int u = 0; u < CL_ROW_U; ++u) {
      pre[u] = round_tot;
#pragma unroll
      for (int w = 0; w < 256 / WAVE; ++w) {
        const uint32_t x = s_c[w][u];
        if (w < (int)wv) pre[u] += x;
        round_tot += x;
      }
    }
    uint4 ea[CL_ROW_U], eb[CL_ROW_U];
    bool listed[CL_ROW_U];
    unsigned long long lbal[CL_ROW_U];
    auto cut = [&](const int u) __attribute__((always_inline)) {
      const uint4 nx1 = shfl_down4(r0[u], 1), nx2 = shfl_down4(r0[u], 2);
      listed[u] = false;
      ea[u] = make_uint4(0u, 0u, 0u, 0u); eb[u] = ea[u];
      if (st[u]) {
        const uint64_t j = b0 + u * 256 + threadIdx.x;
        const uint32_t i = at + pre[u] + (uint32_t)__popcll(bal[u] & ((1ull << lane) - 1ull));
        const ClCut k = cl_cut(recs, lo, hi, j, r0[u], rp[u], nx1, nx2, lane, ss, se, hl, row);
        if (k.too_long) atomicOr(status, 1u);
        ci.o[i] = k.o_first; ci.row[i] = row; ci.pa[i] = k.pa | (k.run_inside ? (int32_t)0x80000000 : 0); ci.rb[i] = k.rb;
        const uint32_t v = r0[u].w;
        const bool simple = k.n == 1 && k.cls == 1 && v < n_var;
        if (!k.cls) ci.uid[i] = CL_NONE;
        if (simple) {
          ci.uid[i] = v;
          const uint32_t bit = 1u << (v & 31u);
          const unsigned long long desc = (unsigned long long)(uint32_t)j | ((unsigned long long)row << 32);
          if (head) {
            var_desc[v] = desc;
            (void)__hip_atomic_fetch_or(&claim_bits[v >> 5], bit, __ATOMIC_RELAXED, __HIP_MEMORY_SCOPE_AGENT);
          } else if (!((bm_lds ? s_bm[(v >> 5) - w_lo] : claim_bits[v >> 5]) & bit)) {
            var_desc[v] = desc;
          }
        }
        listed[u] = k.cls != 0 && !simple;
        ea[u] = make_uint4(i, (uint32_t)k.key, (uint32_t)(k.key >> 32), (uint32_t)j);
        eb[u] = make_uint4(k.n | (k.cls << 16), (uint32_t)(k.o_first + k.rb), (uint32_t)k.o_first, v);
      }
      lbal[u] = __ballot(listed[u]);
      if (lane == 0) s_l[wv][u] = (uint32_t)__popcll(lbal[u]);
    };
    static_assert(CL_ROW_U == 4, "one call per slice");
    cut(0); cut(1); cut(2); cut(3);
    __syncthreads();
    uint32_t lpre = lat;
#pragma unroll
    for (int u = 0; u < CL_ROW_U; ++u) {
      uint32_t mine = lpre;
#pragma unroll
      for (int w = 0; w < 256 / WAVE; ++w) {
        const uint32_t x = s_l[w][u];
        if (w < (int)wv) mine += x;
        lpre += x;
      }
      if (listed[u]) {
        uint4* dst = reinterpret_cast<uint4*>(cx_list + mine + (uint32_t)__popcll(lbal[u] & ((1ull << lane) - 1ull)));
        dst[0] = ea[u]; dst[1] = eb[u];
      }
    }
  }
  if (threadIdx.x == 0 && b + 1 == ch_off[row + 1]) {
    const uint32_t i = at + round_tot;
    int32_t pa = 0, rb = 0;
    if (hi > lo) { pa = recs[hi - 1].o + (int32_t)recs[hi - 1].alt_len; rb = (int32_t)recs[hi - 1].rs - pa; }
    ci.o[i] = CL_FAR; ci.row[i] = row; ci.pa[i] = pa; ci.rb[i] = rb; ci.uid[i] = CL_NONE;
  }
}

#define CL_UID_U 4
__global__ __launch_bounds__(256) void k_cl_enter(const ClListed* __restrict__ cx_list, const uint32_t* __restrict__ n_list_dev, uint32_t t_first,
                                                  uint32_t t_end, ClSlot* tab, uint32_t mask, uint32_t max_probe, uint32_t fail_bit,
                                                  uint32_t* __restrict__ inst_uid, const uint32_t* __restrict__ inst_row, uint32_t* __restrict__ cx_state,
                                                  ClUniq cu, uint32_t* n_table, uint32_t n_var, uint32_t u_cap, uint32_t* __restrict__ status) {
  __shared__ uint32_t s_n[256 / WAVE][CL_UID_U];
  __shared__ uint32_t s_base;
  const uint32_t n_list = *n_list_dev < t_end ? *n_list_dev : t_end;
  const uint32_t t0 = t_first + blockIdx.x * (256 * CL_UID_U) + threadIdx.x;
  if (t_first + blockIdx.x * (256 * CL_UID_U) >= n_list) return;
  const uint32_t lane = threadIdx.x & (WAVE - 1), wv = threadIdx.x / WAVE;
  uint4 ent[CL_UID_U], lk[CL_UID_U];
  uint32_t sl[CL_UID_U];
  bool on[CL_UID_U], won[CL_UID_U];
#pragma unroll
  for (int u = 0; u < CL_UID_U; ++u) {
    const uint32_t t = t0 + u * 256;
    on[u] = t < n_list;
    ent[u] = *reinterpret_cast<const uint4*>(cx_list + (on[u] ? t : t_first));
  }
#pragma unroll
  for (int u = 0; u < CL_UID_U; ++u) {
    const unsigned long long k = (unsigned long long)ent[u].y | ((unsigned long long)ent[u].z << 32);
    sl[u] = (uint32_t)(k >> 17) & mask;
    lk[u] = *reinterpret_cast<const uint4*>(tab + sl[u]);
  }
#pragma unroll
  for (int u = 0; u < CL_UID_U; ++u) {
    won[u] = false;
    if (!on[u]) continue;
    const unsigned long long k = (unsigned long long)ent[u].y | ((unsigned long long)ent[u].z << 32);
    uint4 e0 = lk[u];
    uint32_t s = sl[u];
    bool placed = false;
    for (uint32_t probe = 0; probe <= mask && probe < max_probe; ++probe) {
      if (probe) e0 = *reinterpret_cast<const uint4*>(tab + s);
      unsigned long long c = (unsigned long long)e0.x | ((unsigned long long)e0.y << 32);
      if (c == 0ull) {
        c = atomicCAS(&tab[s].key, 0ull, k);
        won[u] = c == 0ull;
      }
      if (c == 0ull || c == k) { placed = true; break; }
      s = (s + 1u) & mask;
    }
    sl[u] = s;
    const uint32_t t = t0 + u * 256;
    if (!placed) { won[u] = false; cx_state[t] = CL_NONE; inst_uid[ent[u].x] = CL_NONE; atomicOr(status, fail_bit); continue; }
    cx_state[t] = won[u] ? CL_NONE : (CL_PENDING | s);
  }
  unsigned long long wb[CL_UID_U];
#pragma unroll
  for (int u = 0; u < CL_UID_U; ++u) { wb[u] = __ballot(won[u]); if (lane == 0) s_n[wv][u] = (uint32_t)__popcll(wb[u]); }
  __syncthreads();
  uint32_t tot = 0, mine[CL_UID_U];
#pragma unroll
  for (int u = 0; u < CL_UID_U; ++u) {
    mine[u] = tot;
#pragma unroll
    for (int w = 0; w < 256 / WAVE; ++w) { const uint32_t x = s_n[w][u]; if (w < (int)wv) mine[u] += x; tot += x; }
  }
  if (!tot) return;
  if (threadIdx.x == 0) s_base = atomicAdd(n_table, tot);
  __syncthreads();
  const uint32_t base = n_var + s_base;
#pragma unroll
  for (int u = 0; u < CL_UID_U; ++u) {
    if (!won[u]) continue;
    const uint32_t un = base + mine[u] + (uint32_t)__popcll(wb[u] & ((1ull << lane) - 1ull));
    const uint32_t i = ent[u].x;
    if (un >= u_cap) { inst_uid[i] = CL_NONE; atomicOr(status, fail_bit); continue; }
    const uint4 e1 = reinterpret_cast<const uint4*>(cx_list + (t0 + u * 256))[1];
    *reinterpret_cast<uint4*>(&tab[sl[u]].up1) = make_uint4(un + 1u, e1.x, e1.y, e1.w);
    inst_uid[i] = un;
    cu.rec[un] = ent[u].w; cu.n[un] = e1.x & 0xffffu; cu.row[un] = inst_row[i]; cu.o[un] = (int32_t)e1.z;
  }
}

__global__ __launch_bounds__(256) void k_cl_describe(const uint32_t* __restrict__ n_table_dev, uint32_t n_var, uint32_t u_cap,
                                                     const unsigned long long* __restrict__ var_desc, ClUniq cu, const HxHead* __restrict__ recs,
                                                     const uint32_t* __restrict__ seg_off, const uint32_t* __restrict__ seg_rel,
                                                     uint32_t* __restrict__ n_variant_clusters, unsigned long long* __restrict__ slots_total) {
  const uint32_t u = blockIdx.x * 256 + threadIdx.x;
  uint32_t span_u = 0;
  const uint32_t nu = n_var + *n_table_dev < u_cap ? n_var + *n_table_dev : u_cap;
  bool variant_cluster = false;
  if (u < nu) {
    uint32_t n, r, row;
    int32_t o_first;
    if (u < n_var) {
      const unsigned long long d = var_desc[u];
      variant_cluster = d != 0ull;
      r = (uint32_t)d; row = (uint32_t)(d >> 32); n = variant_cluster ? 1u : 0u;
      o_first = variant_cluster ? recs[r].o : 0;
      cu.rec[u] = r; cu.n[u] = n; cu.row[u] = row; cu.o[u] = o_first;
    } else {
      n = cu.n[u]; r = cu.rec[u]; row = cu.row[u]; o_first = cu.o[u];
    }
    if (n == 0) { cu.span2[u] = 0; cu.seg[u] = 0; }
    else {
      const int32_t o_end = recs[r + n - 1].o + (int32_t)recs[r + n - 1].alt_len;
      span_u = 2u * ((uint32_t)(o_end - o_first) + CL_LINK);
      cu.span2[u] = span_u;
      const uint32_t rel = o_first > CL_LINK + HAWK_PAD ? (uint32_t)(o_first - CL_LINK - HAWK_PAD) : 0u;
      uint32_t lo = seg_off[row], hi = seg_off[row + 1];
      while (hi - lo > 1) {
        const uint32_t mid = (lo + hi) >> 1;
        if (seg_rel[mid] <= rel) lo = mid; else hi = mid;
      }
      cu.seg[u] = lo;
    }
  }
  __shared__ uint32_t s_red[256 / WAVE][2];
  const unsigned long long vb = __ballot(variant_cluster);
  const uint32_t ssum = wave_sum(span_u);
  if ((threadIdx.x & (WAVE - 1)) == 0) { s_red[threadIdx.x / WAVE][0] = (uint32_t)__popcll(vb); s_red[threadIdx.x / WAVE][1] = ssum; }
  __syncthreads();
  if (threadIdx.x == 0) {
    uint32_t a = 0, b = 0;
#pragma unroll
    for (int w = 0; w < 256 / WAVE; ++w) { a += s_red[w][0]; b += s_red[w][1]; }
    if (a) atomicAdd(n_variant_clusters, a);
    if (b) atomicAdd(slots_total, (unsigned long long)b);
  }
}
__global__ void k_cl_results(const uint32_t* __restrict__ n_inst, const uint32_t* __restrict__ counters, const unsigned long long* __restrict__ slots_total,
                             const uint32_t* __restrict__ status, unsigned long long* __restrict__ out) {
  out[0] = *n_inst; out[1] = counters[0]; out[2] = counters[1]; out[3] = *slots_total; out[4] = *status;
}
__global__ __launch_bounds__(256) void k_cl_uid(const ClListed* __restrict__ cx_list, const uint32_t* __restrict__ n_list_dev, uint32_t t_end,
                                                const uint32_t* __restrict__ cx_state, const ClSlot* __restrict__ tab, uint32_t* __restrict__ inst_uid,
                                                ClUniq cu, const HxHead* __restrict__ recs, uint32_t* __restrict__ status) {
  const uint32_t n_list = *n_list_dev < t_end ? *n_list_dev : t_end;
  if (blockIdx.x * (256 * CL_UID_U) >= n_list) return;
  const uint32_t t0 = blockIdx.x * (256 * CL_UID_U) + threadIdx.x;
  uint32_t v[CL_UID_U];
  bool pend[CL_UID_U];
  bool any = false;
#pragma unroll
  for (int u = 0; u < CL_UID_U; ++u) {
    const uint32_t t = t0 + u * 256;
    v[u] = t < n_list ? cx_state[t] : CL_NONE;
    pend[u] = v[u] != CL_NONE && (v[u] & CL_PENDING);
    any = any || pend[u];
  }
  if (!__any(any)) return;
  uint4 e1[CL_UID_U], la[CL_UID_U], lb[CL_UID_U];
#pragma unroll
  for (int u = 0; u < CL_UID_U; ++u) {
    e1[u] = reinterpret_cast<const uint4*>(tab + (pend[u] ? (v[u] & ~CL_PENDING) : 0u))[1];
    const uint4* l = reinterpret_cast<const uint4*>(cx_list + (pend[u] ? t0 + u * 256 : 0u));
    la[u] = l[0]; lb[u] = l[1];
  }
  uint32_t rrec[CL_UID_U];
#pragma unroll
  for (int u = 0; u < CL_UID_U; ++u) rrec[u] = (pend[u] && e1[u].x != 0u && (lb[u].x & 0xffffu) > 1u) ? cu.rec[e1[u].x - 1u] : 0u;
  bool bad = false;
#pragma unroll
  for (int u = 0; u < CL_UID_U; ++u) {
    if (!pend[u]) continue;
    const uint32_t i = la[u].x, ncls = lb[u].x;
    if (e1[u].x == 0u) { inst_uid[i] = CL_NONE; bad = true; continue; }
    inst_uid[i] = e1[u].x - 1u;
    bool b = ncls != e1[u].y || (ncls >> 16) != 1 || lb[u].y != e1[u].z || lb[u].w != e1[u].w;
    const uint32_t n = ncls & 0xffffu;
    if (!b && n > 1) {
      const HxHead* pa = recs + la[u].w;
      const HxHead* pb = recs + rrec[u];
      const int32_t oa = (int32_t)lb[u].z, ob = pb[0].o;
      for (uint32_t k = 1; k < n; ++k) {
        const uint4 xa = *reinterpret_cast<const uint4*>(pa + k), xb = *reinterpret_cast<const uint4*>(pb + k);
        b = b || xa.w != xb.w || xa.z != xb.z || xa.y != xb.y || (int32_t)xa.x - oa != (int32_t)xb.x - ob;
      }
    }
    bad = bad || b;
  }
  if (bad) atomicOr(status, 2u);
}

uint32_t hawk_cl_chunk_bound(uint64_t n_records, uint32_t n_rows) { return (uint32_t)(n_records / CL_CHUNK) + n_rows; }
void hawk_launch_cl_chunks(hipStream_t st, const uint64_t* hv_off, const uint8_t* is_ref, const int32_t* ss, const int32_t* se, uint32_t n_rows,
                           uint32_t* ch_off, uint32_t* ch_row) {
  hipLaunchKernelGGL(k_cl_chunks, dim3(1), dim3(1024), 0, st, hv_off, is_ref, ss, se, n_rows, ch_off, ch_row);
}
void hawk_launch_cl_count(hipStream_t st, const void* recs, const uint64_t* hv_off, const uint32_t* hap_len, const int32_t* ss, const int32_t* se,
                          const uint32_t* ch_off, const uint32_t* ch_row, uint32_t n_rows, uint32_t n_var, uint32_t ch_bound, uint32_t* cnt ,
                          uint32_t* lcnt ) {
  if (ch_bound)
    hipLaunchKernelGGL(k_cl_count, dim3(ch_bound), dim3(256), 0, st, static_cast<const HxHead*>(recs), hv_off, hap_len, ss, se, ch_off, ch_row, n_rows,
                       n_var, cnt, lcnt);
}
#define CL_HEAD_CHUNKS 96
#define CL_HEAD_LISTED 16384
void hawk_launch_cl_fill(hipStream_t st, const void* recs, const uint64_t* hv_off, const uint32_t* hap_len, const int32_t* ss, const int32_t* se,
                         uint32_t n_rows, const uint32_t* ch_off, const uint32_t* ch_row, uint32_t ch_bound, const uint32_t* inst_base,
                         const uint32_t* list_base, int32_t* o, uint32_t* row, int32_t* pa, int32_t* rb, uint32_t* inst_uid, void* var_desc,
                         uint32_t* claim_bits, uint32_t n_var, void* cx_list, uint32_t* status) {
  ClInst ci{o, row, pa, rb, inst_uid};
#ifdef HAWK_TEST_HOOKS
  {
    const char* wk = getenv("HAWK_CLUSTER_WEAK_HASH");
    const uint32_t weak = wk && wk[0] == '1' ? 1u : 0u;
    (void)hipMemcpyToSymbol(HIP_SYMBOL(cl_weak_hash), &weak, sizeof(weak));
  }
#endif
  const uint32_t n_head = ch_bound < 16 * CL_HEAD_CHUNKS ? 0u : CL_HEAD_CHUNKS;
  if (n_head)
    hipLaunchKernelGGL(k_cl_fill, dim3(n_head), dim3(256), 0, st, static_cast<const HxHead*>(recs), hv_off, hap_len, ss, se, ch_off, ch_row, inst_base,
                       list_base, ci, static_cast<unsigned long long*>(var_desc), claim_bits, n_var, static_cast<ClListed*>(cx_list), status, 0u, n_rows, 1u);
  if (ch_bound > n_head)
    hipLaunchKernelGGL(k_cl_fill, dim3(ch_bound - n_head), dim3(256), 0, st, static_cast<const HxHead*>(recs), hv_off, hap_len, ss, se, ch_off, ch_row,
                       inst_base, list_base, ci, static_cast<unsigned long long*>(var_desc), claim_bits, n_var, static_cast<ClListed*>(cx_list), status,
                       n_head, n_rows, 0u);
}
void hawk_launch_cl_finish(hipStream_t st, uint32_t list_bound, const uint32_t* n_inst_dev, const uint32_t* n_list_dev, uint32_t* counters,
                           unsigned long long* results, uint32_t n_var, uint32_t u_cap, void* tab,
                           uint32_t mask, uint32_t max_probe, uint32_t fail_bit, const void* cx_list, uint32_t* cx_state, const void* var_desc,
                           const void* recs, uint32_t* inst_uid, const uint32_t* inst_row, const uint32_t* seg_off, const uint32_t* seg_rel,
                           uint32_t* u_rec, uint32_t* u_n, uint32_t* u_row, int32_t* u_o, uint32_t* u_seg, uint32_t* u_span2, uint32_t* status) {
  ClUniq cu{u_rec, u_n, u_row, u_o, u_seg, u_span2};
  const uint32_t per = 256 * CL_UID_U;
  const uint32_t head = list_bound < 16 * CL_HEAD_LISTED ? 0u : CL_HEAD_LISTED;
  const ClListed* list = static_cast<const ClListed*>(cx_list);
  if (head)
    hipLaunchKernelGGL(k_cl_enter, dim3((head + per - 1) / per), dim3(256), 0, st, list, n_list_dev, 0u, head, static_cast<ClSlot*>(tab), mask, max_probe,
                       fail_bit, inst_uid, inst_row, cx_state, cu, counters, n_var, u_cap, status);
  if (list_bound > head)
    hipLaunchKernelGGL(k_cl_enter, dim3((list_bound - head + per - 1) / per), dim3(256), 0, st, list, n_list_dev, head, list_bound, static_cast<ClSlot*>(tab),
                       mask, max_probe, fail_bit, inst_uid, inst_row, cx_state, cu, counters, n_var, u_cap, status);
  hipLaunchKernelGGL(k_cl_describe, dim3((u_cap + 255) / 256), dim3(256), 0, st, counters, n_var, u_cap, static_cast<const unsigned long long*>(var_desc), cu,
                     static_cast<const HxHead*>(recs), seg_off, seg_rel, counters + 1, reinterpret_cast<unsigned long long*>(counters + 4));
  if (list_bound)
    hipLaunchKernelGGL(k_cl_uid, dim3((list_bound + per - 1) / per), dim3(256), 0, st, list, n_list_dev, list_bound, cx_state, static_cast<const ClSlot*>(tab),
                       inst_uid, cu, static_cast<const HxHead*>(recs), status);
  hipLaunchKernelGGL(k_cl_results, dim3(1), dim3(1), 0, st, n_inst_dev, counters, reinterpret_cast<const unsigned long long*>(counters + 4), status, results);
}

__device__ __forceinline__ VcRanges cs_ranges(const HapSetDev& hs, const ScanParams& p, uint32_t h) {
  VcRanges rg;
  const int ss = hs.scan_start[h], se = hs.scan_stop[h], haplen = (int)hs.hap_len[h];
  const int poF = p.right ? 0 : p.guidelen, poR = p.right ? p.guidelen : 0;
  const int qmin = HAWK_PAD, qmax = haplen - p.L - HAWK_PAD + 1;
  rg.slo[0] = ss - poF; rg.shi[0] = se - poF; rg.slo[1] = ss - poR; rg.shi[1] = se - poR;
  rg.lo[0] = rg.slo[0] > qmin ? rg.slo[0] : qmin; rg.hi[0] = rg.shi[0] < qmax ? rg.shi[0] : qmax;
  rg.lo[1] = rg.slo[1] > qmin ? rg.slo[1] : qmin; rg.hi[1] = rg.shi[1] < qmax ? rg.shi[1] : qmax;
  return rg;
}
__device__ __forceinline__ uint32_t group_incl_scan(uint32_t v, uint32_t gl) {
#pragma unroll
  for (int d = 1; d < CS_G; d <<= 1) {
    const uint32_t t = (uint32_t)__shfl_up((int)v, d, CS_G);
    if (gl >= (uint32_t)d) v += t;
  }
  return v;
}

__device__ __forceinline__ int64_t posmap_hint(const HapSetDev& hs, uint32_t k0, uint32_t kend, uint32_t rel) {
  uint32_t k = k0;
  while (k + 1 < kend && hs.seg_rel[k + 1] <= rel) ++k;
  return hs.seg_gen[k] + (int64_t)(rel - hs.seg_rel[k]);
}

__global__ __launch_bounds__(256) void k_cs_templates(HapSetDev hs, VcArgs va, ClDict cd, ScanParams p, GuideParams gp, RefInfo ri,
                                                      uint4* __restrict__ res, uint32_t* __restrict__ tbase, CsRow* __restrict__ trows, unsigned long long* __restrict__ t_count, uint64_t t_cap, int* status) {
  __shared__ double s_cfd[336];
  __shared__ uint32_t s_w[256 / WAVE];
  __shared__ unsigned long long s_base;
  __shared__ uint32_t s_X[15][256];
  __shared__ uint32_t s_k[2][256];
  __shared__ uint32_t s_e[256];
  const uint32_t tid = threadIdx.x;
  if (gp.score_cfdon) for (uint32_t i = tid; i < 336; i += 256) s_cfd[i] = gp.cfd_mm[i];
  __syncthreads();
  const uint32_t gl = tid & (CS_G - 1);
  const uint32_t u = (blockIdx.x * 256 + tid) / CS_G;
  const uint32_t nc_u = u < cd.n_uniq ? cd.u_n[u] : 0u;
  const bool live = nc_u != 0u;
  const bool hole = u < cd.n_uniq && !live;
  const HxVar* __restrict__ recs = static_cast<const HxVar*>(va.recs_);
  const uint32_t h = live ? cd.u_row[u] : 0u, r0 = live ? cd.u_rec[u] : 0u, nc = live ? nc_u : 1u;
  const uint32_t seg0 = live ? cd.u_seg[u] : hs.seg_off[0], seg_end = hs.seg_off[h + 1];
  const uint32_t back = (uint64_t)r0 > va.hv_off[h] ? 1u : 0u;
  const HxVar* __restrict__ sv = recs + r0 - back;
  const int nrec = (int)(nc + back);
  const int L = p.L;
  const int32_t haplen = (int32_t)hs.hap_len[h];
  const int32_t o_first = live ? cd.u_o[u] : 0;
  const int32_t o_end = live ? recs[r0 + nc - 1].o + (int32_t)recs[r0 + nc - 1].alt_len : 0;
  const int32_t qa = o_first - (L - 1) > 0 ? o_first - (L - 1) : 0;
  const int32_t qb = o_end < haplen ? o_end : haplen;
  const int nwords = qb > qa ? (qb - qa + 31) / 32 : 0;
  const VcRanges rg = cs_ranges(hs, p, h);
  auto hits_before = [&](int64_t x) -> uint32_t {
    const int64_t xm = (int64_t)va.ref_S * 32;
    const uint32_t xc = (uint32_t)(x < 0 ? 0 : (x > xm ? xm : x));
    const uint4 e = va.hp[xc >> 5];
    const uint32_t m = (1u << (xc & 31u)) - 1u;
    return e.y + (uint32_t)__popc(e.x & m) + e.w + (uint32_t)__popc(e.z & m);
  };
  const int32_t rb_front = back ? (int32_t)sv[0].rs - (sv[0].o + (int32_t)sv[0].alt_len) : 0;
  const uint32_t h_front = hits_before((int64_t)o_first + rb_front - (L - 1)), h_behind = hits_before((int64_t)recs[r0 + nc - 1].rs);
  const int poF = p.right ? 0 : p.guidelen, poR = p.right ? p.guidelen : 0;
  const uint32_t mlo = L >= 32 ? 0xffffffffu : ((1u << L) - 1u), mhi = L <= 32 ? 0u : ((1u << (L - 32)) - 1u);
  const int W = L + 2 * HAWK_PAD;
  const uint32_t whi = W >= 64 ? 0xffffffffu : ((1u << (W - 32)) - 1u);
  const int ncfd = gp.guidelen < 20 ? gp.guidelen : 20;
  const uint32_t cfdmask = (1u << ncfd) - 1u;
  auto ref32 = [&](int pl, uint32_t r) -> uint32_t {
    const uint32_t w = (r >> 5) < va.ref_S - 2 ? (r >> 5) : va.ref_S - 2;
    return ext32_glb(va.ref[pl], (w << 5) | (r & 31u));
  };
  auto word = [&](int32_t q0, uint32_t (&X)[5][3], uint32_t& kF, uint32_t& kR, uint32_t& hits, uint32_t& cand) {
    const int32_t p0 = q0 - HAWK_PAD;
    const int32_t p0c = p0 < 0 ? 0 : p0;
    int32_t shift_run = 0;
    if (!vc_string_fast(va, sv, nrec, p0c, haplen, q0 + 32, X, shift_run))
      hx_words_t<false, 3>(va.alt_codes, sv, sv, nrec, nrec, false, p0c, haplen, ref32, X[0], X[1], X[2], X[3], X[4]);
    if (p0 < 0) {
      const uint32_t sh = (uint32_t)(-p0);
#pragma unroll
      for (int pl = 0; pl < 5; ++pl) {
        X[pl][2] = fsh(X[pl][1], X[pl][2], 32u - sh);
        X[pl][1] = fsh(X[pl][0], X[pl][1], 32u - sh);
        X[pl][0] = X[pl][0] << sh;
      }
    }
    uint32_t v0 = X[4][0], v1 = X[4][1], v2 = X[4][2];
    int r = 1;
    while (2 * r <= L && r < 32) {
      v0 |= fsh(v0, v1, (uint32_t)r); v1 |= fsh(v1, v2, (uint32_t)r); v2 |= v2 >> r;
      r *= 2;
    }
    const int rem = L - r;
    if (rem > 0) {
      if (rem < 32) { v0 |= fsh(v0, v1, (uint32_t)rem); v1 |= fsh(v1, v2, (uint32_t)rem); v2 |= v2 >> rem; }
      else { v0 |= v1; v1 |= v2; }
    }
    const uint32_t E = fsh(v0, v1, HAWK_PAD);
    const uint32_t own = range_mask(q0, qa, qb);
    uint32_t f = pam_match96(X, p.pam_fwd, p.pamlen, HAWK_PAD + poF) & own;
    uint32_t rv = pam_match96(X, p.pam_rev, p.pamlen, HAWK_PAD + poR) & own;
    f &= range_mask(q0, rg.slo[0], rg.shi[0]);
    rv &= range_mask(q0, rg.slo[1], rg.shi[1]);
    hits += __popc(f) + __popc(rv);
    f &= range_mask(q0, rg.lo[0], rg.hi[0]);
    rv &= range_mask(q0, rg.lo[1], rg.hi[1]);
    cand += __popc(f) + __popc(rv);
    kF = f & E;
    kR = rv & E;
  };
  auto classify = [&](int32_t q0, const uint32_t (&X)[5][3], uint32_t kF, uint32_t kR, uint32_t& vF, uint32_t& vR) {
    vF = 0; vR = 0;
#pragma unroll 1
    for (int s = 0; s < 2; ++s) {
      uint32_t m = s ? kR : kF;
      while (m) {
        const uint32_t bpos = (uint32_t)__builtin_ctz(m);
        m &= m - 1u;
        const int64_t start = posmap_hint(hs, seg0, seg_end, (uint32_t)q0 + bpos);
        const int64_t qr64 = start - ri.startp;
        const bool inr = qr64 >= 0 && qr64 < (int64_t)ri.n_bits;
        const uint32_t qr = inr ? (uint32_t)qr64 : 0u;
        const bool has_ref = inr && (((s ? ri.bits[1] : ri.bits[0])[qr >> 5] >> (qr & 31u)) & 1u);
        bool same = has_ref;
        if (has_ref) {
#pragma unroll
          for (int pl = 0; pl < 4; ++pl) {
            W2 wn = ext96(X[pl][0], X[pl][1], X[pl][2], bpos);
            wn.hi &= whi;
            const uint32_t clo = fsh(wn.lo, wn.hi, HAWK_PAD) & mlo, chi = (wn.hi >> HAWK_PAD) & mhi;
            const W2 rc = ext_glb(va.ref[pl], qr);
            same = same && (rc.lo & mlo) == clo && (rc.hi & mhi) == chi;
          }
        }
        if (!same) { if (s) vR |= 1u << bpos; else vF |= 1u << bpos; }
      }
    }
  };
  auto write = [&](int32_t q0, const uint32_t (&X)[5][3], uint32_t vF, uint32_t vR, uint64_t at0, uint64_t at1) {
#pragma unroll 1
    for (int s = 0; s < 2; ++s) {
      uint32_t m = s ? vR : vF;
      while (m) {
        const uint32_t bpos = (uint32_t)__builtin_ctz(m);
        m &= m - 1u;
        const uint32_t q = (uint32_t)q0 + bpos;
        const uint64_t k = s ? at1++ : at0++;
        if (k >= t_cap) { atomicExch(status, -3 ); continue; }
        W2 win[5], core[4], rcore[4];
#pragma unroll
        for (int pl = 0; pl < 5; ++pl) {
          win[pl] = ext96(X[pl][0], X[pl][1], X[pl][2], bpos);
          win[pl].hi &= whi;
          if (pl < 4) {
            core[pl].lo = fsh(win[pl].lo, win[pl].hi, HAWK_PAD) & mlo;
            core[pl].hi = (win[pl].hi >> HAWK_PAD) & mhi;
          }
        }
        const int64_t start = posmap_hint(hs, seg0, seg_end, q), stop = posmap_hint(hs, seg0, seg_end, q + (uint32_t)L);
        const int64_t qr64 = start - ri.startp;
        const bool inr = qr64 >= 0 && qr64 < (int64_t)ri.n_bits;
        const uint32_t qr = inr ? (uint32_t)qr64 : 0u;
        const bool has_ref = inr && (((s ? ri.bits[1] : ri.bits[0])[qr >> 5] >> (qr & 31u)) & 1u);
#pragma unroll
        for (int pl = 0; pl < 4; ++pl) {
          rcore[pl] = ext_glb(va.ref[pl], qr);
          rcore[pl].lo &= mlo; rcore[pl].hi &= mhi;
          if (!has_ref) rcore[pl] = core[pl];
        }
        double score = __longlong_as_double(0x7ff8000000000000ll);
        if (gp.score_cfdon && has_ref) {
          bool err;
          score = cfdon_from_slices(core, rcore, (uint32_t)s, L, cfdmask, s_cfd, err);
          if (err && gp.score_cfdon == 1) atomicExch(status, -5 );
        }
        const bool pamfirst = (p.right != 0) != (s != 0);
        const int64_t ds = start - ri.startp, de = stop - start;
        if (ds < INT32_MIN || ds > INT32_MAX || de < INT32_MIN || de > INT32_MAX) atomicExch(status, -7 );
        const uint64_t sc = (uint64_t)__double_as_longlong(score);
        uint4* __restrict__ tp = reinterpret_cast<uint4*>(trows + k);
        tp[0] = make_uint4((uint32_t)((int32_t)(pamfirst ? q : q + (uint32_t)p.guidelen) - o_first), (uint32_t)s | (has_ref ? 2u : 0u),
                           (uint32_t)(int32_t)ds, (uint32_t)(int32_t)de);
        tp[1] = make_uint4((uint32_t)sc, (uint32_t)(sc >> 32), win[0].lo, win[0].hi);
        tp[2] = make_uint4(win[1].lo, win[1].hi, win[2].lo, win[2].hi);
        tp[3] = make_uint4(win[3].lo, win[3].hi, win[4].lo, win[4].hi);
      }
    }
  };

  const bool one_round = nwords <= CS_G;
  const uint32_t g0 = tid & ~(uint32_t)(CS_G - 1);
  uint32_t X[5][3];
#pragma unroll
  for (int pl = 0; pl < 5; ++pl) X[pl][0] = X[pl][1] = X[pl][2] = 0;
  uint32_t vF = 0, vR = 0, n0 = 0, n1 = 0, hits = 0, cand = 0, TF = 0, TR = 0;
  if (one_round) {
    uint32_t kF = 0, kR = 0;
    if ((int)gl < nwords) word(qa + 32 * (int32_t)gl, X, kF, kR, hits, cand);
    const uint32_t c = (uint32_t)__popc(kF) | ((uint32_t)__popc(kR) << 16);
    const uint32_t inc = group_incl_scan(c, gl);
    const uint32_t tot = (uint32_t)__shfl((int)inc, CS_G - 1, CS_G);
    TF = tot & 0xffffu; TR = tot >> 16;
#pragma unroll
    for (int pl = 0; pl < 5; ++pl) { s_X[pl * 3 + 0][tid] = X[pl][0]; s_X[pl * 3 + 1][tid] = X[pl][1]; s_X[pl * 3 + 2][tid] = X[pl][2]; }
    s_k[0][tid] = kF; s_k[1][tid] = kR; s_e[tid] = inc - c;
  } else {
#pragma unroll 1
    for (int w0 = 0; w0 < nwords; w0 += CS_G) {
      const int w = w0 + (int)gl;
      uint32_t kF = 0, kR = 0;
      vF = 0; vR = 0;
      if (w < nwords) {
        word(qa + 32 * w, X, kF, kR, hits, cand);
        classify(qa + 32 * w, X, kF, kR, vF, vR);
      }
      const uint32_t c = (uint32_t)__popc(vF) | ((uint32_t)__popc(vR) << 16);
      const uint32_t tot = (uint32_t)__shfl((int)group_incl_scan(c, gl), CS_G - 1, CS_G);
      n0 += tot & 0xffffu; n1 += tot >> 16;
    }
  }
  hits = group_incl_scan(hits, gl); cand = group_incl_scan(cand, gl);
  const bool leader = live && gl == CS_G - 1;
  if (hole && gl == CS_G - 1) { res[2 * u] = make_uint4(0u, 0u, 0u, 0u); res[2 * u + 1] = make_uint4(0u, 0u, 0u, 0u); tbase[u] = 0u; }
  const uint32_t want = one_round ? TF + TR : n0 + n1;
  uint32_t btot;
  const uint32_t bex = block_excl_scan<256 / WAVE>(leader ? want : 0u, s_w, &btot);
  if (tid == 0) s_base = btot ? atomicAdd(t_count, (unsigned long long)btot) : 0ull;
  __syncthreads();
  const uint32_t gex = (uint32_t)__shfl((int)bex, CS_G - 1, CS_G);
  const uint64_t tb = s_base + gex;
  if (tb + want > 0xffffffffull) atomicExch(status, -7 );
  if (!one_round) {
    if (leader) { res[2 * u] = make_uint4(n0, n1, hits, cand); res[2 * u + 1] = make_uint4((uint32_t)tb, h_front, h_behind, 0u); tbase[u] = (uint32_t)tb; }
    if (!live || n0 + n1 == 0) return;
    uint32_t b0 = 0, b1 = 0, h2 = 0, c2 = 0;
#pragma unroll 1
    for (int w0 = 0; w0 < nwords; w0 += CS_G) {
      const int w = w0 + (int)gl;
      uint32_t kF = 0, kR = 0;
      vF = 0; vR = 0;
      if (w < nwords) {
        word(qa + 32 * w, X, kF, kR, h2, c2);
        classify(qa + 32 * w, X, kF, kR, vF, vR);
      }
      const uint32_t c = (uint32_t)__popc(vF) | ((uint32_t)__popc(vR) << 16);
      const uint32_t inc = group_incl_scan(c, gl);
      const uint32_t tot = (uint32_t)__shfl((int)inc, CS_G - 1, CS_G);
      const uint32_t ex = inc - c;
      if (w < nwords) write(qa + 32 * w, X, vF, vR, tb + b0 + (ex & 0xffffu), tb + n0 + b1 + (ex >> 16));
      b0 += tot & 0xffffu; b1 += tot >> 16;
    }
    return;
  }
  uint32_t done = 0;
#pragma unroll 1
  for (int sd = 0; sd < 2; ++sd) {
    const uint32_t T = sd ? TR : TF, sh16 = sd ? 16u : 0u;
    uint32_t ns = 0;
#pragma unroll 1
    for (uint32_t j0 = 0; j0 < T; j0 += CS_G) {
      const uint32_t j = j0 + gl;
      const bool act = j < T;
      const uint32_t jj = act ? j : 0u;
      uint32_t l = 0;
#pragma unroll
      for (uint32_t step = CS_G / 2; step; step >>= 1) l += (((s_e[g0 + l + step] >> sh16) & 0xffffu) <= jj) ? step : 0u;
      const uint32_t src = g0 + l;
      const uint32_t bpos = select_bit(s_k[sd][src], jj - ((s_e[src] >> sh16) & 0xffffu));
      const uint32_t q = (uint32_t)(qa + 32 * (int32_t)l) + bpos;
      W2 win[5], core[4], rcore[4];
#pragma unroll
      for (int pl = 0; pl < 5; ++pl) {
        win[pl] = ext96(s_X[pl * 3 + 0][src], s_X[pl * 3 + 1][src], s_X[pl * 3 + 2][src], bpos);
        win[pl].hi &= whi;
        if (pl < 4) {
          core[pl].lo = fsh(win[pl].lo, win[pl].hi, HAWK_PAD) & mlo;
          core[pl].hi = (win[pl].hi >> HAWK_PAD) & mhi;
        }
      }
      const int64_t start = posmap_hint(hs, seg0, seg_end, q), stop = posmap_hint(hs, seg0, seg_end, q + (uint32_t)L);
      const int64_t qr64 = start - ri.startp;
      const bool inr = qr64 >= 0 && qr64 < (int64_t)ri.n_bits;
      const uint32_t qr = inr ? (uint32_t)qr64 : 0u;
      const uint32_t rw = (sd ? ri.bits[1] : ri.bits[0])[qr >> 5];
#pragma unroll
      for (int pl = 0; pl < 4; ++pl) rcore[pl] = ext_glb(va.ref[pl], qr);
      const bool has_ref = inr && ((rw >> (qr & 31u)) & 1u);
      bool same = has_ref;
#pragma unroll
      for (int pl = 0; pl < 4; ++pl) {
        rcore[pl].lo &= mlo; rcore[pl].hi &= mhi;
        same = same && rcore[pl].lo == core[pl].lo && rcore[pl].hi == core[pl].hi;
        if (!has_ref) rcore[pl] = core[pl];
      }
      const bool valid = act && !same;
      const uint32_t vinc = group_incl_scan(valid ? 1u : 0u, gl);
      const uint32_t vtot = (uint32_t)__shfl((int)vinc, CS_G - 1, CS_G);
      if (valid && live) {
        const uint64_t k = tb + done + ns + (vinc - 1u);
        if (k >= t_cap) atomicExch(status, -3 );
        else {
          double score = __longlong_as_double(0x7ff8000000000000ll);
          if (gp.score_cfdon && has_ref) {
            bool err;
            score = cfdon_from_slices(core, rcore, (uint32_t)sd, L, cfdmask, s_cfd, err);
            if (err && gp.score_cfdon == 1) atomicExch(status, -5 );
          }
          const bool pamfirst = (p.right != 0) != (sd != 0);
          const int64_t ds = start - ri.startp, de = stop - start;
          if (ds < INT32_MIN || ds > INT32_MAX || de < INT32_MIN || de > INT32_MAX) atomicExch(status, -7 );
          const uint64_t sc = (uint64_t)__double_as_longlong(score);
          uint4* __restrict__ tp = reinterpret_cast<uint4*>(trows + k);
          tp[0] = make_uint4((uint32_t)((int32_t)(pamfirst ? q : q + (uint32_t)p.guidelen) - o_first), (uint32_t)sd | (has_ref ? 2u : 0u),
                             (uint32_t)(int32_t)ds, (uint32_t)(int32_t)de);
          tp[1] = make_uint4((uint32_t)sc, (uint32_t)(sc >> 32), win[0].lo, win[0].hi);
          tp[2] = make_uint4(win[1].lo, win[1].hi, win[2].lo, win[2].hi);
          tp[3] = make_uint4(win[3].lo, win[3].hi, win[4].lo, win[4].hi);
        }
      }
      ns += vtot;
    }
    if (sd == 0) n0 = ns; else n1 = ns;
    done += ns;
  }
  if (leader) { res[2 * u] = make_uint4(n0, n1, hits, cand); res[2 * u + 1] = make_uint4((uint32_t)tb, h_front, h_behind, 0u); tbase[u] = (uint32_t)tb; }
}

#define CS_CNT_U 4
__global__ __launch_bounds__(256) void k_cs_count(HapSetDev hs, VcArgs va, ClDict cd, ScanParams p, const uint4* __restrict__ res,
                                                  const unsigned long long* __restrict__ t_count, uint64_t t_cap,
                                                  uint32_t* __restrict__ group_counts, uint32_t* __restrict__ counts, uint32_t* __restrict__ inst_tb,
                                                  unsigned long long* __restrict__ shards) {
  __shared__ uint32_t s_red[256 / WAVE][2];
  const uint32_t i0 = blockIdx.x * (256 * CS_CNT_U) + threadIdx.x;
  const uint32_t lane = threadIdx.x & (WAVE - 1);
  const bool ovf = *t_count > t_cap;
  uint32_t uid[CS_CNT_U], below[CS_CNT_U];
  int32_t paf[CS_CNT_U];
  bool in[CS_CNT_U];
#pragma unroll
  for (int u = 0; u < CS_CNT_U; ++u) {
    const uint32_t i = i0 + u * 256;
    in[u] = i < cd.n_inst;
    const uint32_t ic = in[u] ? i : 0u;
    uid[u] = cd.inst_uid[ic]; paf[u] = cd.inst_pa[ic];
    below[u] = CL_NONE;
    if (lane == 0 && in[u] && i > 0) below[u] = cd.inst_uid[i - 1];
  }
  uint4 r[CS_CNT_U], r2[CS_CNT_U];
  uint32_t behind0[CS_CNT_U];
#pragma unroll
  for (int u = 0; u < CS_CNT_U; ++u) {
    const bool has = in[u] && uid[u] != CL_NONE;
    r[u] = make_uint4(0u, 0u, 0u, 0u); r2[u] = r[u]; behind0[u] = 0u;
    if (cd.n_uniq) {
      const uint32_t us = has ? uid[u] : 0u;
      r[u] = res[2 * us]; r2[u] = res[2 * us + 1];
      if (lane == 0 && below[u] != CL_NONE) behind0[u] = res[2 * below[u] + 1].z;
    }
    if (!has) { r[u] = make_uint4(0u, 0u, 0u, 0u); r2[u] = r[u]; }
  }
  uint32_t cand = 0, hits = 0;
#pragma unroll
  for (int u = 0; u < CS_CNT_U; ++u) {
    const uint32_t i = i0 + u * 256;
    uint32_t behind = (uint32_t)__shfl_up((int)r2[u].z, 1);
    if (lane == 0) behind = behind0[u];
    uint32_t rows_i = 0;
    if (in[u]) {
      if (paf[u] < 0) {
        const uint32_t hc = r2[u].y - behind;
        hits += hc; cand += hc;
      } else {
        const int32_t pa = paf[u], pb = cd.inst_o[i] - (p.L - 1);
        if (pb > pa) {
          const VcRanges rg = cs_ranges(hs, p, cd.inst_row[i]);
          vc_count_run(va, rg, pa, pb, cd.inst_rb[i], cand, hits);
        }
      }
      hits += r[u].z; cand += r[u].w;
      rows_i = ovf ? 0u : r[u].x + r[u].y;
      counts[i] = rows_i;
      inst_tb[i] = r2[u].x;
    }
    const uint32_t gsum = wave_sum(rows_i);
    const uint32_t iw = blockIdx.x * (256 * CS_CNT_U) + u * 256 + (threadIdx.x & ~(uint32_t)(WAVE - 1));
    if (lane == 0 && iw < cd.n_inst) group_counts[iw / WAVE] = gsum;
  }
  const uint32_t a = wave_sum(cand), b = wave_sum(hits);
  if (lane == 0) { s_red[threadIdx.x / WAVE][0] = a; s_red[threadIdx.x / WAVE][1] = b; }
  __syncthreads();
  if (threadIdx.x == 0) {
    uint32_t t0 = 0, t1 = 0;
#pragma unroll
    for (int wv = 0; wv < 256 / WAVE; ++wv) { t0 += s_red[wv][0]; t1 += s_red[wv][1]; }
    if (t0 | t1) {
      atomicAdd(&shards[(blockIdx.x & 255u) * 2 + 0], (unsigned long long)t0);
      atomicAdd(&shards[(blockIdx.x & 255u) * 2 + 1], (unsigned long long)t1);
    }
  }
}

__device__ __forceinline__ void nt_store4(uint32_t* q, const uint4& v) {
  __builtin_nontemporal_store(v.x, q); __builtin_nontemporal_store(v.y, q + 1);
  __builtin_nontemporal_store(v.z, q + 2); __builtin_nontemporal_store(v.w, q + 3);
}
template <int NI, int CE_CH>
__global__ __launch_bounds__(256) void k_cs_emit_rows(uint32_t n_inst, const uint32_t* __restrict__ inst_row, const int32_t* __restrict__ inst_o,
                                                      const uint32_t* __restrict__ counts, const uint32_t* __restrict__ inst_tb,
                                                      const CsRow* __restrict__ trows, const uint64_t* __restrict__ offsets,
                                                      const unsigned long long* __restrict__ t_count, uint64_t t_cap, uint4* __restrict__ rows,
                                                      uint64_t cap, int* status) {
  constexpr int NE = NI * WAVE;
  constexpr int CE_SUB = CE_CH / 16;
  __shared__ uint32_t s_ex[4][NE + 1];
  __shared__ uint32_t s_tb[4][NE], s_h[4][NE];
  __shared__ int32_t s_dq[4][NE];
  __shared__ uint32_t s_src[4][2][CE_CH], s_rh[4][2][CE_CH];
  __shared__ int32_t s_rdq[4][2][CE_CH];
  if (*t_count > t_cap) return;
  const uint32_t wv = threadIdx.x / WAVE, lane = threadIdx.x & (WAVE - 1);
  const uint32_t i0 = (blockIdx.x * 4 + wv) * NE;
  if (i0 >= n_inst) return;
  uint32_t cnt[NI], tb[NI], h[NI];
  int32_t dq[NI];
#pragma unroll
  for (int c = 0; c < NI; ++c) {
    const uint32_t i = i0 + c * WAVE + lane;
    const bool in = i < n_inst;
    const uint32_t ii = in ? i : n_inst - 1;
    cnt[c] = counts[ii]; tb[c] = inst_tb[ii]; h[c] = inst_row[ii]; dq[c] = inst_o[ii];
    if (!in) cnt[c] = 0;
  }
  const uint64_t o0 = offsets[i0 / WAVE];
  uint32_t Wt = 0;
#pragma unroll
  for (int c = 0; c < NI; ++c) {
    const uint32_t inc = wave_incl_scan(cnt[c]);
    s_ex[wv][c * WAVE + lane] = Wt + inc - cnt[c];
    s_tb[wv][c * WAVE + lane] = tb[c]; s_h[wv][c * WAVE + lane] = h[c] << HAWK_ROW_HAP_SHIFT; s_dq[wv][c * WAVE + lane] = dq[c];
    Wt += (uint32_t)__builtin_amdgcn_readlane((int)inc, WAVE - 1);
  }
  if (Wt == 0) return;
  if (o0 + Wt > cap) { if (lane == 0) atomicCAS(status, 0, -3 ); return; }
  __builtin_amdgcn_wave_barrier();
  const uint32_t qd = lane & 3u, rq = lane >> 2;
  uint4* __restrict__ const dst = rows + o0 * 4 + qd;
  auto meta = [&](uint32_t c0, uint32_t buf) {
#pragma unroll
    for (uint32_t sub = 0; sub < (CE_CH + WAVE - 1) / WAVE; ++sub) {
      const uint32_t r = sub * WAVE + lane;
      if (CE_CH < WAVE && r >= CE_CH) break;
      const uint32_t t = c0 + r < Wt ? c0 + r : Wt - 1;
      uint32_t l = 0;
#pragma unroll
      for (uint32_t step = NE / 2; step; step >>= 1) l += (s_ex[wv][l + step] <= t) ? step : 0u;
      s_src[wv][buf][r] = s_tb[wv][l] + (t - s_ex[wv][l]);
      s_rh[wv][buf][r] = s_h[wv][l];
      s_rdq[wv][buf][r] = s_dq[wv][l];
    }
    __builtin_amdgcn_wave_barrier();
  };
  auto fetch = [&](uint4 (&v)[CE_SUB], uint32_t buf) {
#pragma unroll
    for (uint32_t j = 0; j < CE_SUB; ++j) v[j] = reinterpret_cast<const uint4*>(trows + s_src[wv][buf][j * 16 + rq])[qd];
  };
  auto store = [&](const uint4 (&v)[CE_SUB], uint32_t c0, uint32_t buf) {
#pragma unroll
    for (uint32_t j = 0; j < CE_SUB; ++j) {
      const uint32_t r = j * 16 + rq;
      uint4 w = v[j];
      if (qd == 0) {
        w.x = (uint32_t)((int32_t)w.x + s_rdq[wv][buf][r]);
        w.y |= s_rh[wv][buf][r];
      }
      if (c0 + r < Wt) nt_store4(reinterpret_cast<uint32_t*>(dst + (size_t)(c0 + r) * 4), w);
    }
  };
  uint4 va[CE_SUB], vb[CE_SUB];
  meta(0, 0);
  fetch(va, 0);
#pragma unroll 1
  for (uint32_t c0 = 0; c0 < Wt; c0 += 2 * CE_CH) {
    const bool more1 = c0 + CE_CH < Wt, more2 = c0 + 2 * CE_CH < Wt;
    if (more1) { meta(c0 + CE_CH, 1); fetch(vb, 1); }
    store(va, c0, 0);
    __builtin_amdgcn_wave_barrier();
    if (more1) {
      if (more2) { meta(c0 + 2 * CE_CH, 0); fetch(va, 0); }
      store(vb, c0 + CE_CH, 1);
      __builtin_amdgcn_wave_barrier();
    }
  }
}
void hawk_launch_cs_emit_rows(hipStream_t st, const ClDict& cd, const uint32_t* counts, const uint32_t* inst_tb, const void* trows, const uint64_t* offsets,
                              const unsigned long long* t_count, uint64_t t_cap, void* rows, uint64_t cap, int* status) {
  if (!cd.n_inst) return;
  constexpr int NI = 4, CH = 256;
  hipLaunchKernelGGL((k_cs_emit_rows<NI, CH>), dim3((cd.n_inst + 256 * NI - 1) / (256 * NI)), dim3(256), 0, st, cd.n_inst, cd.inst_row, cd.inst_o, counts,
                     inst_tb, static_cast<const CsRow*>(trows), offsets, t_count, t_cap, static_cast<uint4*>(rows), cap, status);
}

void hawk_launch_cs_templates(hipStream_t st, const HapSetDev& hs, const VcArgs& va, const ClDict& cd, const ScanParams& p, const GuideParams& gp,
                              const RefInfo& ri, void* res, uint32_t* tbase, void* trows, unsigned long long* t_count, uint64_t t_cap, int* status) {
  if (!cd.n_uniq) return;
  const uint32_t nb = (uint32_t)(((uint64_t)cd.n_uniq * CS_G + 255) / 256);
  hipLaunchKernelGGL(k_cs_templates, dim3(nb), dim3(256), 0, st, hs, va, cd, p, gp, ri, static_cast<uint4*>(res), tbase, static_cast<CsRow*>(trows),
                     t_count, t_cap, status);
}
void hawk_launch_cs_count(hipStream_t st, const HapSetDev& hs, const VcArgs& va, const ClDict& cd, const ScanParams& p, const void* res,
                          const unsigned long long* t_count, uint64_t t_cap, uint32_t* group_counts, uint32_t* counts, uint32_t* inst_tb,
                          unsigned long long* shards) {
  if (!cd.n_inst) return;
  hipLaunchKernelGGL(k_cs_count, dim3((cd.n_inst + 256 * CS_CNT_U - 1) / (256 * CS_CNT_U)), dim3(256), 0, st, hs, va, cd, p, static_cast<const uint4*>(res), t_count, t_cap,
                     group_counts, counts, inst_tb, shards);
}

__global__ __launch_bounds__(256) void k_rows_pack(GuideCols c, const uint64_t* __restrict__ n_dev, uint64_t n_host, uint4* __restrict__ rows, int64_t startp,
                                                   int* status) {
  const uint64_t n = n_dev ? *n_dev : n_host;
  const uint64_t i = (uint64_t)blockIdx.x * 256 + threadIdx.x;
  if (i >= n) return;
  const int64_t start = c.start[i], ds = start - startp, de = c.stop[i] - start;
  const uint32_t h = c.hap[i];
  if (ds < INT32_MIN || ds > INT32_MAX || de < INT32_MIN || de > INT32_MAX || h >= HAWK_ROW_MAX_HAP) atomicCAS(status, 0, -7 );
  const uint64_t sc = (uint64_t)__double_as_longlong(c.cfdon[i]);
  uint64_t w[HAWK_PLANES];
#pragma unroll
  for (int pl = 0; pl < HAWK_PLANES; ++pl) w[pl] = c.win[(size_t)pl * c.cap + i];
  uint4* __restrict__ r = rows + i * 4;
  r[0] = make_uint4(c.pos[i], (uint32_t)(c.strand[i] & 1u) | ((uint32_t)c.flags[i] << 1) | (h << HAWK_ROW_HAP_SHIFT), (uint32_t)(int32_t)ds, (uint32_t)(int32_t)de);
  r[1] = make_uint4((uint32_t)sc, (uint32_t)(sc >> 32), (uint32_t)w[0], (uint32_t)(w[0] >> 32));
  r[2] = make_uint4((uint32_t)w[1], (uint32_t)(w[1] >> 32), (uint32_t)w[2], (uint32_t)(w[2] >> 32));
  r[3] = make_uint4((uint32_t)w[3], (uint32_t)(w[3] >> 32), (uint32_t)w[4], (uint32_t)(w[4] >> 32));
}
__global__ __launch_bounds__(256) void k_rows_unpack(const uint4* __restrict__ rows, uint64_t n, int64_t startp, GuideCols d) {
  const uint64_t i = (uint64_t)blockIdx.x * 256 + threadIdx.x;
  if (i >= n) return;
  const uint4* __restrict__ r = rows + i * 4;
  const uint4 a = r[0], b = r[1], cc = r[2], e = r[3];
  const int64_t start = startp + (int64_t)(int32_t)a.z;
  if (d.hap) d.hap[i] = a.y >> HAWK_ROW_HAP_SHIFT;
  if (d.pos) d.pos[i] = a.x;
  if (d.strand) d.strand[i] = (uint8_t)(a.y & 1u);
  if (d.flags) d.flags[i] = (uint8_t)((a.y >> 1) & 0xffu);
  if (d.start) d.start[i] = start;
  if (d.stop) d.stop[i] = start + (int64_t)(int32_t)a.w;
  if (d.cfdon) d.cfdon[i] = __longlong_as_double((long long)((uint64_t)b.x | ((uint64_t)b.y << 32)));
  if (d.win) {
    d.win[i] = (uint64_t)b.z | ((uint64_t)b.w << 32);
    d.win[d.cap + i] = (uint64_t)cc.x | ((uint64_t)cc.y << 32);
    d.win[2 * d.cap + i] = (uint64_t)cc.z | ((uint64_t)cc.w << 32);
    d.win[3 * d.cap + i] = (uint64_t)e.x | ((uint64_t)e.y << 32);
    d.win[4 * d.cap + i] = (uint64_t)e.z | ((uint64_t)e.w << 32);
  }
}
void hawk_launch_rows_pack(hipStream_t st, const GuideCols& src, const uint64_t* n_dev, uint64_t n_host, uint64_t max_rows, uint4* rows, int64_t startp,
                           int* status) {
  if (!max_rows) return;
  hipLaunchKernelGGL(k_rows_pack, dim3((unsigned)((max_rows + 255) / 256)), dim3(256), 0, st, src, n_dev, n_host, rows, startp, status);
}
void hawk_launch_rows_unpack(hipStream_t st, const uint4* rows, uint64_t n, int64_t startp, const GuideCols& dst) {
  if (!n) return;
  hipLaunchKernelGGL(k_rows_unpack, dim3((unsigned)((n + 255) / 256)), dim3(256), 0, st, rows, n, startp, dst);
}

__global__ __launch_bounds__(256) void k_cc_ucnt(const uint4* __restrict__ res, uint32_t nu, uint32_t* __restrict__ cnt) {
  const uint32_t u = blockIdx.x * 256 + threadIdx.x;
  if (u < nu) { const uint4 r = res[2 * u]; cnt[u] = r.x + r.y; }
}
__global__ __launch_bounds__(256) void k_cc_mini(GuideCols c, uint64_t r0, const CsRow* __restrict__ trows, uint64_t t_rows,
                                                 const uint64_t* __restrict__ moff, const uint32_t* __restrict__ tbase, uint32_t nu, int64_t startp,
                                                 GuideCols m) {
  const uint64_t i = (uint64_t)blockIdx.x * 256 + threadIdx.x;
  if (i >= r0 + t_rows) return;
  if (i < r0) {
    m.hap[i] = gc_hap(c, i); m.pos[i] = gc_pos(c, i); m.strand[i] = (uint8_t)gc_strand(c, i); m.start[i] = gc_start(c, i); m.stop[i] = gc_stop(c, i);
    m.flags[i] = (uint8_t)gc_flags(c, i); m.cfdon[i] = gc_cfdon(c, i);
#pragma unroll
    for (int pl = 0; pl < HAWK_PLANES; ++pl) m.win[(size_t)pl * m.cap + i] = gc_win(c, pl, i);
    return;
  }
  uint32_t lo = 0, hi = nu;
  while (hi - lo > 1) {
    const uint32_t mid = (lo + hi) >> 1;
    if (moff[mid] <= i - r0) lo = mid; else hi = mid;
  }
  const uint4* __restrict__ tp = reinterpret_cast<const uint4*>(trows + (tbase[lo] + (i - r0 - moff[lo])));
  const uint4 a = tp[0], b = tp[1], cc = tp[2], d = tp[3];
  const int64_t start = startp + (int64_t)(int32_t)a.z;
  m.hap[i] = 1u;
  m.pos[i] = a.x; m.strand[i] = (uint8_t)(a.y & 1u); m.flags[i] = (uint8_t)((a.y >> 1) & 0xffu);
  m.start[i] = start; m.stop[i] = start + (int64_t)(int32_t)a.w;
  m.cfdon[i] = __longlong_as_double((long long)((uint64_t)b.x | ((uint64_t)b.y << 32)));
  m.win[0 * m.cap + i] = (uint64_t)b.z | ((uint64_t)b.w << 32);
  m.win[1 * m.cap + i] = (uint64_t)cc.x | ((uint64_t)cc.y << 32);
  m.win[2 * m.cap + i] = (uint64_t)cc.z | ((uint64_t)cc.w << 32);
  m.win[3 * m.cap + i] = (uint64_t)d.x | ((uint64_t)d.y << 32);
  m.win[4 * m.cap + i] = (uint64_t)d.z | ((uint64_t)d.w << 32);
}
__global__ __launch_bounds__(256) void k_cc_gidm(const uint32_t* __restrict__ perm, const uint64_t* __restrict__ goff, uint64_t nm, uint64_t G,
                                                 uint32_t* __restrict__ gidm) {
  const uint64_t j = (uint64_t)blockIdx.x * 256 + threadIdx.x;
  if (j >= nm) return;
  uint64_t lo = 0, hi = G;
  while (hi - lo > 1) {
    const uint64_t mid = (lo + hi) >> 1;
    if (goff[mid] <= j) lo = mid; else hi = mid;
  }
  gidm[perm[j]] = (uint32_t)lo;
}
__global__ __launch_bounds__(256) void k_cs_gid(ClDict cd, const uint4* __restrict__ res, const uint64_t* __restrict__ moff,
                                                const uint64_t* __restrict__ offsets, uint64_t r0, uint64_t n, const uint32_t* __restrict__ gidm,
                                                uint32_t* __restrict__ gid, uint32_t* __restrict__ vals) {
  __shared__ uint32_t s_ex[4][WAVE + 1];
  __shared__ uint32_t s_tb[4][WAVE];
  const uint32_t wv = threadIdx.x / WAVE, lane = threadIdx.x & (WAVE - 1);
  const uint32_t i = blockIdx.x * 256 + threadIdx.x;
  uint32_t cnt = 0, tb = 0;
  if (i < cd.n_inst) {
    const uint32_t u = cd.inst_uid[i];
    if (u != CL_NONE) { const uint4 r = res[2 * u]; cnt = r.x + r.y; tb = (uint32_t)moff[u]; }
  }
  const uint32_t inc = wave_incl_scan(cnt);
  const uint32_t Wt = (uint32_t)__builtin_amdgcn_readlane((int)inc, WAVE - 1);
  const uint32_t i0 = blockIdx.x * 256 + wv * WAVE;
  const uint64_t o0 = i0 < cd.n_inst ? offsets[i0 / WAVE] : 0;
  s_ex[wv][lane] = inc - cnt;
  s_tb[wv][lane] = tb;
  __syncthreads();
  if (o0 + Wt > n) return;
  for (uint32_t t = lane; t < Wt; t += WAVE) {
    uint32_t l = 0;
#pragma unroll
    for (uint32_t step = WAVE / 2; step; step >>= 1) l += (s_ex[wv][l + step] <= t) ? step : 0u;
    const uint64_t o = o0 + t;
    gid[o] = gidm[r0 + s_tb[wv][l] + (t - s_ex[wv][l])];
    vals[o] = (uint32_t)o;
  }
}
__global__ __launch_bounds__(256) void k_cc_refgid(uint64_t r0, const uint32_t* __restrict__ gidm, uint32_t* __restrict__ gid, uint32_t* __restrict__ vals) {
  const uint64_t i = (uint64_t)blockIdx.x * 256 + threadIdx.x;
  if (i < r0) { gid[i] = gidm[i]; vals[i] = (uint32_t)i; }
}
void hawk_launch_cc_ucnt(hipStream_t st, const void* res, uint32_t nu, uint32_t* cnt) {
  hipLaunchKernelGGL(k_cc_ucnt, dim3((nu + 255) / 256), dim3(256), 0, st, static_cast<const uint4*>(res), nu, cnt);
}
void hawk_launch_cc_mini(hipStream_t st, const GuideCols& c, uint64_t r0, const void* trows, uint64_t t_rows, const uint64_t* moff, const uint32_t* tbase,
                         uint32_t nu, int64_t startp, GuideCols m) {
  const uint64_t nm = r0 + t_rows;
  hipLaunchKernelGGL(k_cc_mini, dim3((unsigned)((nm + 255) / 256)), dim3(256), 0, st, c, r0, static_cast<const CsRow*>(trows), t_rows, moff, tbase, nu,
                     startp, m);
}
void hawk_launch_cc_gidm(hipStream_t st, const uint32_t* perm, const uint64_t* goff, uint64_t nm, uint64_t G, uint32_t* gidm) {
  hipLaunchKernelGGL(k_cc_gidm, dim3((unsigned)((nm + 255) / 256)), dim3(256), 0, st, perm, goff, nm, G, gidm);
}
void hawk_launch_cs_gid(hipStream_t st, const ClDict& cd, const void* res, const uint64_t* moff, const uint64_t* offsets, uint64_t r0, uint64_t n,
                        const uint32_t* gidm, uint32_t* gid, uint32_t* vals) {
  if (r0) hipLaunchKernelGGL(k_cc_refgid, dim3((unsigned)((r0 + 255) / 256)), dim3(256), 0, st, r0, gidm, gid, vals);
  if (cd.n_inst) hipLaunchKernelGGL(k_cs_gid, dim3((cd.n_inst + 255) / 256), dim3(256), 0, st, cd, static_cast<const uint4*>(res), moff, offsets, r0, n,
                                    gidm, gid, vals);
}
```

### crispr-hawk_amd/csrc/hawk_device.h

```cpp
#pragma once
#include <hip/hip_runtime.h>
#include <stdint.h>

#define HAWK_PLANES 5
#define HAWK_PAD 10
#define HAWK_BLOCK 256
#define HAWK_WPT 4

struct HapSetDev {
  uint32_t n_hap;
  uint32_t S;
  const uint32_t* plane[HAWK_PLANES];
  const uint32_t* hap_len;
  const uint8_t* is_ref;
  const int32_t* scan_start;
  const int32_t* scan_stop;
  const uint32_t* seg_off;
  const uint32_t* seg_rel;
  const int64_t* seg_gen;
  int32_t ref_index;
};

struct TileMeta {
  uint32_t h, blk;
  uint32_t hap_len;
  int32_t scan_start, scan_stop;
  uint32_t is_ref;
  uint32_t seg0, seg_end;
};

struct ScanParams {
  uint64_t pam_fwd, pam_rev;
  int32_t pamlen, guidelen, right;
  int32_t L;
  uint32_t bph;
  uint32_t need;
  int32_t poF, poR;
};

struct ScanTotals {
  uint64_t n_keep;
  uint64_t n_keep_fwd;
  uint64_t n_cand;
  uint64_t n_hits;
};

struct GuideCols {
  uint32_t* hap;
  uint32_t* pos;
  uint8_t* strand;
  int64_t* start;
  int64_t* stop;
  uint8_t* flags;
  double* cfdon;
  uint64_t* win;
  uint64_t cap;
  uint4* rows;
  int64_t startp;
};
#define HAWK_ROW_HAP_SHIFT 9
#define HAWK_ROW_MAX_HAP (1u << 23)
#ifdef __HIPCC__
__device__ __forceinline__ const uint32_t* gc_roww(const GuideCols& c, uint64_t i) { return reinterpret_cast<const uint32_t*>(c.rows) + i * 16; }
__device__ __forceinline__ uint32_t gc_hap(const GuideCols& c, uint64_t i) { return c.rows ? gc_roww(c, i)[1] >> HAWK_ROW_HAP_SHIFT : c.hap[i]; }
__device__ __forceinline__ uint32_t gc_pos(const GuideCols& c, uint64_t i) { return c.rows ? gc_roww(c, i)[0] : c.pos[i]; }
__device__ __forceinline__ uint32_t gc_strand(const GuideCols& c, uint64_t i) { return c.rows ? (gc_roww(c, i)[1] & 1u) : (uint32_t)c.strand[i]; }
__device__ __forceinline__ uint32_t gc_flags(const GuideCols& c, uint64_t i) { return c.rows ? ((gc_roww(c, i)[1] >> 1) & 0xffu) : (uint32_t)c.flags[i]; }
__device__ __forceinline__ int64_t gc_start(const GuideCols& c, uint64_t i) { return c.rows ? c.startp + (int64_t)(int32_t)gc_roww(c, i)[2] : c.start[i]; }
__device__ __forceinline__ int64_t gc_stop(const GuideCols& c, uint64_t i) {
  if (!c.rows) return c.stop[i];
  const uint32_t* w = gc_roww(c, i);
  return c.startp + (int64_t)(int32_t)w[2] + (int64_t)(int32_t)w[3];
}
__device__ __forceinline__ double gc_cfdon(const GuideCols& c, uint64_t i) {
  if (!c.rows) return c.cfdon[i];
  const uint32_t* w = gc_roww(c, i);
  return __longlong_as_double((long long)((uint64_t)w[4] | ((uint64_t)w[5] << 32)));
}
__device__ __forceinline__ uint64_t gc_win(const GuideCols& c, int pl, uint64_t i) {
  if (!c.rows) return c.win[(size_t)pl * c.cap + i];
  const uint32_t* w = gc_roww(c, i);
  return (uint64_t)w[6 + 2 * pl] | ((uint64_t)w[7 + 2 * pl] << 32);
}
#endif
void hawk_launch_rows_pack(hipStream_t st, const GuideCols& src, const uint64_t* n_dev, uint64_t n_host, uint64_t max_rows, uint4* rows, int64_t startp,
                           int* status);
void hawk_launch_rows_unpack(hipStream_t st, const uint4* rows, uint64_t n, int64_t startp, const GuideCols& dst);

struct GuideParams {
  int32_t pamlen, guidelen, right, L;
  int32_t score_cfdon;
  const double* cfd_mm;
  const double* cfd_pam;
  uint32_t bph;
};

struct RefInfo {
  int32_t index;
  int32_t lo[2], hi[2];
  int64_t startp;
  const uint32_t* bits[2];
  uint32_t n_bits;
};
struct VcArgs {
  const uint32_t* ref[4];
  uint32_t ref_S;
  const void* recs_;
  const uint8_t* alt_codes;
  const uint64_t* hv_off;
  const void* tiles_;
  const uint4* hp;
};
void hawk_launch_vsearch(hipStream_t st, int pass, const HapSetDev& hs, const VcArgs& va, const ScanParams& p, const struct GuideParams& gp,
                         const struct RefInfo& ri, const TileMeta* tmeta, uint32_t* counts, uint32_t* counts0, unsigned long long* shards,
                         const uint64_t* offsets, struct GuideCols out, int* status, uint32_t tile0, uint32_t n_tiles);
void hawk_launch_ref_hits(hipStream_t st, const HapSetDev& hs, const ScanParams& p, int32_t ref_index, void* hp);
struct ClDict {
  uint32_t n_inst, n_uniq;
  const uint32_t* inst_uid;
  const int32_t* inst_o;
  const uint32_t* inst_row;
  const int32_t* inst_pa;
  const int32_t* inst_rb;
  const uint32_t* u_rec;
  const uint32_t* u_n;
  const uint32_t* u_row;
  const int32_t* u_o;
  const uint32_t* u_seg;
};
size_t hawk_cs_row_bytes();
void hawk_launch_scan2_u32(hipStream_t st, const uint32_t* cnt_a, const uint32_t* cnt_b, uint32_t n, uint32_t* off_a, uint32_t* off_b);
void hawk_launch_hx_heads(hipStream_t st, const void* recs, const uint32_t* hv_idx, uint64_t n, void* heads);
uint32_t hawk_cl_chunk_bound(uint64_t n_records, uint32_t n_rows);
void hawk_launch_cl_chunks(hipStream_t st, const uint64_t* hv_off, const uint8_t* is_ref, const int32_t* ss, const int32_t* se, uint32_t n_rows,
                           uint32_t* ch_off, uint32_t* ch_row);
void hawk_launch_cl_count(hipStream_t st, const void* recs, const uint64_t* hv_off, const uint32_t* hap_len, const int32_t* ss, const int32_t* se,
                          const uint32_t* ch_off, const uint32_t* ch_row, uint32_t n_rows, uint32_t n_var, uint32_t ch_bound, uint32_t* cnt ,
                          uint32_t* lcnt );
void hawk_launch_cl_fill(hipStream_t st, const void* recs, const uint64_t* hv_off, const uint32_t* hap_len, const int32_t* ss, const int32_t* se,
                         uint32_t n_rows, const uint32_t* ch_off, const uint32_t* ch_row, uint32_t ch_bound, const uint32_t* inst_base,
                         const uint32_t* list_base, int32_t* o, uint32_t* row, int32_t* pa, int32_t* rb, uint32_t* inst_uid,
                         void* var_desc , uint32_t* claim_bits , uint32_t n_var,
                         void* cx_list , uint32_t* status);
size_t hawk_cl_slot_bytes();
size_t hawk_cl_listed_bytes();
void hawk_launch_cl_finish(hipStream_t st, uint32_t list_bound, const uint32_t* n_inst_dev, const uint32_t* n_list_dev, uint32_t* counters ,
                           unsigned long long* results , uint32_t n_var, uint32_t u_cap,
                           void* tab , uint32_t mask, uint32_t max_probe, uint32_t fail_bit, const void* cx_list, uint32_t* cx_state,
                           const void* var_desc, const void* recs, uint32_t* inst_uid, const uint32_t* inst_row, const uint32_t* seg_off,
                           const uint32_t* seg_rel, uint32_t* u_rec, uint32_t* u_n, uint32_t* u_row, int32_t* u_o, uint32_t* u_seg, uint32_t* u_span2,
                           uint32_t* status);
void hawk_launch_cs_templates(hipStream_t st, const HapSetDev& hs, const VcArgs& va, const ClDict& cd, const ScanParams& p, const struct GuideParams& gp,
                              const struct RefInfo& ri, void* res , uint32_t* tbase, void* trows,
                              unsigned long long* t_count, uint64_t t_cap, int* status);
void hawk_launch_cs_count(hipStream_t st, const HapSetDev& hs, const VcArgs& va, const ClDict& cd, const ScanParams& p, const void* res,
                          const unsigned long long* t_count, uint64_t t_cap, uint32_t* group_counts, uint32_t* counts, uint32_t* inst_tb,
                          unsigned long long* shards);
void hawk_launch_cs_emit_rows(hipStream_t st, const ClDict& cd, const uint32_t* counts, const uint32_t* inst_tb, const void* trows, const uint64_t* offsets,
                              const unsigned long long* t_count, uint64_t t_cap, void* rows, uint64_t cap, int* status);
void hawk_launch_list_check(hipStream_t st, const uint64_t* row_off, uint32_t n_rows, const uint32_t* hv_idx, const int32_t* hv_o,
                            const int32_t* v_r0, const int32_t* v_span, const int32_t* v_chain, uint32_t n_var, uint32_t ref_len,
                            int check_clamp, uint32_t* status);
void hawk_launch_segments(hipStream_t st, const uint64_t* ioff, const uint32_t* indel, const uint32_t* hv_idx, const int32_t* hv_o,
                          const int32_t* v_r0, const int32_t* v_chain, const uint32_t* hap_len, uint32_t n_rows, int64_t startp,
                          uint32_t* seg_cnt, uint32_t* seg_off, uint32_t* seg_rel , int64_t* seg_gen);
void hawk_launch_rev_lookup(hipStream_t st, const uint32_t* seg_off, const uint32_t* seg_rel, const int64_t* seg_gen, const uint32_t* hap_len,
                            uint32_t n_rows, int64_t g0, int64_t g1, int64_t* out0, int64_t* out1);
void hawk_launch_tile_meta(hipStream_t st, const uint32_t* seg_off, const uint32_t* seg_rel, const uint32_t* hap_len, const uint8_t* is_ref,
                           const int32_t* scan_start, const int32_t* scan_stop, uint32_t n_rows, uint32_t bph, TileMeta* tm);
void hawk_launch_ref_bits(hipStream_t st, const HapSetDev& hs, const ScanParams& p, const RefInfo& ri, uint32_t* bitsF, uint32_t* bitsR);

struct OtSite {
  uint64_t code;
  uint32_t nmask;
  uint32_t q;
  uint32_t row;
  uint32_t pad;
};
struct OtHit { uint64_t site; uint32_t guide; uint32_t mm; };
#define OT_MAX_BLOCKS 8
struct OtSeeds {
  int32_t nb;
  int32_t start[OT_MAX_BLOCKS], klen[OT_MAX_BLOCKS];
  uint32_t off_base[OT_MAX_BLOCKS];
  uint64_t pmask2[OT_MAX_BLOCKS];
};

#define OT_MAX_PAIRS (OT_MAX_BLOCKS * (OT_MAX_BLOCKS - 1) / 2)
struct OtPairSeeds {
  int32_t nb, n_pairs;
  int32_t start[OT_MAX_BLOCKS], klen[OT_MAX_BLOCKS];
  uint64_t pmask2[OT_MAX_BLOCKS];
  uint8_t pi[OT_MAX_PAIRS], pj[OT_MAX_PAIRS];
  uint32_t off_base[OT_MAX_PAIRS];
};
void hawk_launch_ot_match_pairs(hipStream_t st, const OtSite* sites, uint64_t n_sites, const OtPairSeeds& sd, const uint32_t* goff,
                                const uint64_t* gcode, const uint32_t* gid, uint32_t n_guides, int guidelen, int sp0, int max_mm,
                                OtHit* hits, uint64_t cap, unsigned long long* n_hits);

void hawk_launch_ot_onehot(hipStream_t st, uint32_t* const* plane, uint64_t nwords);
void hawk_launch_ot_sites(hipStream_t st, const HapSetDev& hs, const ScanParams& p, const uint32_t* keepF, const uint32_t* keepR,
                          const uint64_t* offsets, OtSite* sites);
void hawk_launch_ot_match(hipStream_t st, const OtSite* sites, uint64_t n_sites, const uint64_t* guides, uint32_t n_guides,
                          int guidelen, int sp0, int max_mm, OtHit* hits, uint64_t cap, unsigned long long* n_hits);
void hawk_launch_ot_match_seeded(hipStream_t st, const OtSite* sites, uint64_t n_sites, const OtSeeds& sd, const uint32_t* goff,
                                 const uint64_t* gcode, const uint32_t* gid, uint32_t n_guides, int guidelen, int sp0, int max_mm,
                                 OtHit* hits, uint64_t cap, unsigned long long* n_hits);
void hawk_launch_ot_gather(hipStream_t st, const OtSite* sites, const OtHit* hits, uint64_t n_hits, OtSite* out);
struct OtSummary {
  const OtSite* sites;
  const double* tab;
  uint32_t* hist;
  unsigned long long* cfd_e4;
  unsigned long long* counters;
  uint32_t stride;
  int32_t sp0, pam2, ncmp;
};
void hawk_launch_ot_match_sum(hipStream_t st, const OtSite* sites, uint64_t n_sites, const uint64_t* guides, uint32_t n_guides,
                              int guidelen, int sp0, int max_mm, const OtSummary& sm);
void hawk_launch_ot_match_seeded_sum(hipStream_t st, const OtSite* sites, uint64_t n_sites, const OtSeeds& sd, const uint32_t* goff,
                                     const uint64_t* gcode, const uint32_t* gid, uint32_t n_guides, int guidelen, int sp0, int max_mm,
                                     const OtSummary& sm);
void hawk_launch_ot_match_pairs_sum(hipStream_t st, const OtSite* sites, uint64_t n_sites, const OtPairSeeds& sd, const uint32_t* goff,
                                    const uint64_t* gcode, const uint32_t* gid, uint32_t n_guides, int guidelen, int sp0, int max_mm,
                                    const OtSummary& sm);
void hawk_launch_pack(hipStream_t st, const uint8_t* ascii, const uint64_t* seq_off, uint32_t hap0, uint32_t n_hap_batch,
                      uint64_t batch_base, const uint32_t* hap_len, uint32_t S, uint32_t* const* plane,
                      unsigned long long* bad_index);
void hawk_launch_scan_raw(hipStream_t st, const HapSetDev& hs, const ScanParams& p, uint32_t* keepF, uint32_t* keepR,
                          uint32_t* counts);
void hawk_launch_emit_hits(hipStream_t st, const HapSetDev& hs, uint32_t bph, const uint32_t* keepF, const uint32_t* keepR,
                           const uint64_t* offsets, uint64_t n_fwd_total, uint32_t* hits_fwd, uint32_t* hits_rev);
void hawk_launch_search(hipStream_t st, int pass, const HapSetDev& hs, const ScanParams& p, const GuideParams& gp,
                        const RefInfo& ri, const TileMeta* tmeta, uint32_t* counts, unsigned long long* shards,
                        const uint64_t* offsets, GuideCols out, int* status, uint32_t* lists, uint32_t* big_count,
                        unsigned long long* big_list, hipEvent_t mid = nullptr, uint32_t n_tiles = 0xffffffffu);
size_t hawk_collapse_temp_bytes(uint64_t n, unsigned begin_bit, unsigned end_bit);
int hawk_launch_collapse(hipStream_t st, const GuideCols& c, const uint8_t* is_ref, uint64_t n, int guidelen, int pamlen, int right,
                         int flank_up, int flank_down, int64_t base, unsigned begin_bit, unsigned end_bit, uint64_t seed, void* temp, size_t temp_bytes, uint64_t* keys, uint32_t* vals,
                         uint32_t* flags, uint32_t* gidx, unsigned long long* counters, uint64_t* group_off, uint8_t* gc_num,
                         uint8_t* gc_den, uint32_t* id2 , void* full , int weak_hash = 0);
void hawk_launch_collapse_verify(hipStream_t st, const GuideCols& c, const uint8_t* is_ref, uint64_t n, int guidelen, int pamlen, int flank_up,
                                 int flank_down, const uint32_t* perm, const uint32_t* grp_a, const uint32_t* grp_b, const uint64_t* group_off,
                                 unsigned long long* mismatches);
void hawk_launch_collapse_verify_rows(hipStream_t st, const GuideCols& c, const uint8_t* is_ref, uint64_t n, uint32_t G, int guidelen, int pamlen,
                                      int flank_up, int flank_down, const uint32_t* perm, const uint32_t* slot_of_row, const uint32_t* slot2rank,
                                      const uint64_t* group_off, void* full , unsigned long long* mismatches);
void hawk_launch_rows_equal(hipStream_t st, const HapSetDev& hs, uint32_t n_pairs, const uint32_t* ra, const uint32_t* rb, uint8_t* equal);
size_t hawk_collapse_full_bytes(uint64_t n);
size_t hawk_collapse_expand_temp_bytes(uint64_t n);
int hawk_launch_collapse_expand(hipStream_t st, const GuideCols& c, uint64_t n, unsigned gbits, int guidelen, int pamlen, int right, void* temp,
                                size_t temp_bytes, uint32_t* gid, uint32_t* vals, uint64_t* group_off, uint8_t* gc_num, uint8_t* gc_den);
void hawk_launch_cc_ucnt(hipStream_t st, const void* res, uint32_t nu, uint32_t* cnt);
void hawk_launch_cc_mini(hipStream_t st, const GuideCols& c, uint64_t r0, const void* trows, uint64_t t_rows, const uint64_t* moff, const uint32_t* tbase,
                         uint32_t nu, int64_t startp, GuideCols m);
void hawk_launch_cc_gidm(hipStream_t st, const uint32_t* perm, const uint64_t* goff, uint64_t nm, uint64_t G, uint32_t* gidm);
void hawk_launch_cs_gid(hipStream_t st, const ClDict& cd, const void* res, const uint64_t* moff, const uint64_t* offsets, uint64_t r0, uint64_t n,
                        const uint32_t* gidm, uint32_t* gid, uint32_t* vals);
size_t hawk_collapse_hash_temp_bytes(uint64_t n, uint32_t C);
int hawk_launch_collapse_hash1(hipStream_t st, const GuideCols& c, const uint8_t* is_ref, uint64_t n, int guidelen, int pamlen, int flank_up,
                               int flank_down, int64_t base, uint64_t seed, void* temp, size_t temp_bytes, void* table, uint32_t C,
                               uint32_t* flags, uint32_t* dense, uint64_t* gkey, uint32_t* gslot, uint32_t* slot_of_row,
                               unsigned long long* counters);
int hawk_launch_collapse_hash2(hipStream_t st, const GuideCols& c, uint64_t n, uint32_t G, int guidelen, int pamlen, int right, unsigned key_end_bit,
                               void* temp, size_t temp_bytes, uint64_t* gkey, uint32_t* gslot, uint32_t C, uint32_t* slot2rank,
                               const uint32_t* slot_of_row, uint32_t* gid, uint32_t* vals, uint64_t* group_off, uint8_t* gc_num,
                               uint8_t* gc_den);
void hawk_launch_collapse_export(hipStream_t st, const GuideCols& c, uint64_t n, uint64_t ng, const uint32_t* perm,
                                 const uint64_t* group_off, const GuideCols& rep, uint32_t* member_hap);
void hawk_launch_gt_parse(hipStream_t st, const uint8_t* text, const uint64_t* line_off, const uint64_t* gt_off, uint64_t n_lines,
                          uint32_t n_samples, uint8_t* codes, uint8_t* flags);
void hawk_launch_gt_count(hipStream_t st, const uint8_t* codes, uint32_t n_cols, const uint32_t* var_line, const uint8_t* var_allele,
                          const int32_t* var_chain, uint32_t n_var, unsigned long long* ballots, uint32_t* col_count );
void hawk_launch_gt_fill(hipStream_t st, uint32_t n_cols, const int32_t* var_r0, const int32_t* var_chain, uint32_t n_var,
                         const unsigned long long* ballots, const uint64_t* col_off, uint32_t* hv_idx, int32_t* hv_o, int64_t* col_delta,
                         const uint64_t* indel_off, uint32_t* indel_entry);
#define HAWK_LIST_CAP 512
void hawk_launch_mscan(hipStream_t st, const uint32_t* counts, uint64_t n, unsigned long long* partial,
                       const unsigned long long* shards, uint64_t* offsets, ScanTotals* totals);
void hawk_launch_cfd(hipStream_t st, const char* wt, const char* sg, uint32_t len, const char* pam2, uint64_t n,
                     const double* mm, const double* pamtab, double* out, int* status);
void hawk_launch_deepcpf1(hipStream_t st, const char* seqs, uint64_t n, const float* w, float* out, int* status);
void hawk_launch_tm_nn(hipStream_t st, const char* seqs, uint32_t len, uint64_t n, double* out, int* status);
void hawk_launch_azimuth(hipStream_t st, const char* seqs, uint64_t n, uint32_t n_trees, const int32_t* tree_off,
                         const int32_t* feature, const int32_t* left, const int32_t* right, const double* threshold,
                         const double* value, double init, double lr, double* out, double* feats_out, int* status);
void hawk_launch_gbt(hipStream_t st, const double* feats, uint64_t n, uint32_t nf, uint32_t n_trees, const int32_t* tree_off,
                     const int32_t* feature, const int32_t* left, const int32_t* right, const double* threshold, const double* value,
                     double init, double lr, int cast_f32, double* out);
uint32_t hawk_hx_tiles_per_row(uint32_t S);
size_t hawk_hx_record_bytes();
size_t hawk_hx_tile_bytes();
void hawk_launch_hx_prepare(hipStream_t st, const uint64_t* hv_off, const uint32_t* hv_idx, const int32_t* hv_o, uint64_t ncar,
                            const uint32_t* v_r0, const uint32_t* v_span, const uint32_t* v_alt_off, const uint32_t* v_alt_len,
                            const void* v_am , const uint32_t* hap_len, uint32_t n_hap, uint32_t S, void* recs,
                            void* tiles);
void hawk_launch_hx_build(hipStream_t st, const uint32_t* const* ref, uint32_t ref_S, const void* recs, const uint8_t* alt_codes,
                          const uint64_t* hv_off, const uint32_t* hap_len, uint32_t n_hap, uint32_t S, uint32_t* const* plane,
                          const void* tiles);
void hawk_launch_hx_hash(hipStream_t st, uint32_t* const* plane, uint32_t n_hap, uint32_t S, unsigned long long* hash);

struct AnnDev {
  const int64_t *start, *end;
  const int64_t* rmax;
  const int64_t* bmax;
  const uint64_t* loff;
  const uint8_t* blob;
  uint64_t n;
};
uint64_t hawk_ann_scan_blocks(uint64_t n);
void hawk_launch_ann_index(hipStream_t st, const int64_t* end, uint64_t n, int64_t* partial, int64_t* rmax, int64_t* bmax);
void hawk_launch_ann_count(hipStream_t st, const AnnDev& A, const int64_t* qs, const int64_t* qe, uint64_t nq, uint64_t* off,
                           unsigned long long* totals);
void hawk_launch_ann_offsets(hipStream_t st, uint64_t* off, uint64_t nq, uint64_t* partial);
void hawk_launch_ann_fill(hipStream_t st, const AnnDev& A, const int64_t* qs, const int64_t* qe, uint64_t nq, const uint64_t* off, uint8_t* out);
```

### crispr-hawk_amd/csrc/hawk_host.h

```cpp
#pragma once
#include <hip/hip_runtime.h>

#include <cstdio>
#include <memory>
#include <vector>

#include "../../include/hawk.h"
#include "hawk_device.h"

#define HAWK_MAX_DEVICES 16
char* hawk_hip_err_buf();

#define HIPCHK(expr)                                                                         \
  do {                                                                                       \
    hipError_t e_ = (expr);                                                                  \
    if (e_ != hipSuccess) {                                                                  \
      snprintf(hawk_hip_err_buf(), 256, "%s: %s (%s:%d)", #expr, hipGetErrorString(e_), __FILE__, __LINE__); \
      return HAWK_E_HIP;                                                                     \
    }                                                                                        \
  } while (0)

struct hawk_ctx {
  int device;
  hipStream_t stream;
  hipEvent_t ev[10];
  void* pinned = nullptr;
};

int hawk_pool_alloc(void** p, size_t bytes);
void hawk_pool_free(void* p);
void hawk_pool_trim();
#define POOLCHK(ptr, bytes)                                                      \
  do {                                                                           \
    int rc_ = hawk_pool_alloc(reinterpret_cast<void**>(ptr), (bytes));           \
    if (rc_) return rc_;                                                         \
  } while (0)

struct PoolScope {
  std::vector<void*> held;
  ~PoolScope() { for (void* q : held) hawk_pool_free(q); }
  int alloc(void** out, size_t bytes) {
    int rc = hawk_pool_alloc(out, bytes);
    if (!rc) held.push_back(*out);
    return rc;
  }
};
#define TEMPCHK(scope, ptr, bytes)                                               \
  do {                                                                           \
    int rc_ = (scope).alloc(reinterpret_cast<void**>(ptr), (bytes));             \
    if (rc_) return rc_;                                                         \
  } while (0)

struct DevBuf {
  void* p = nullptr;
  size_t bytes = 0;
  int reserve(size_t need) {
    if (need <= bytes) return HAWK_OK;
    if (p) { hawk_pool_free(p); p = nullptr; bytes = 0; }
    size_t want = need + need / 8 + 256;
    int rc = hawk_pool_alloc(&p, want);
    if (rc) return rc;
    bytes = want;
    return HAWK_OK;
  }
  void release() { if (p) hawk_pool_free(p); p = nullptr; bytes = 0; }
  template <class T> T* as() const { return reinterpret_cast<T*>(p); }
};

struct hawk_hapset {
  hawk_ctx* ctx;
  uint32_t n_hap, S;
  uint64_t total_len;
  std::vector<uint32_t> hap_len;
  std::vector<int32_t> scan_start, scan_stop;
  uint32_t* plane[HAWK_PLANES];
  uint32_t* d_hap_len;
  uint8_t* d_is_ref;
  int32_t *d_scan_start, *d_scan_stop;
  uint32_t *d_seg_off, *d_seg_rel;
  int64_t* d_seg_gen;
  int32_t ref_index;
  uint32_t n_ref_rows = 0;
  bool has_meta;
  bool has_partner = false;
  int32_t partner_start = 0, partner_stop = 0;
  uint32_t bph;
  TileMeta* d_tile_meta;
  int64_t ref_startp;
  int64_t min_gen, max_gen;
  uint64_t cols_cap = 0;
  uint64_t cols_gen = 0;
  uint64_t collapse_gen = 0;
  std::vector<double> cfd_host;
  DevBuf keepF, keepR, counts, offsets, totals, misc, cfd, partial, sites, hits, guides, lists;
  DevBuf ckeys, cvals, cflags, cgidx, ctemp, cgoff, cgc, ccnt, cfull;
  DevBuf ctable, cocc, cdense, cgkey, cgslot;
  uint64_t last_groups = 0;
  std::shared_ptr<uint64_t> plan_groups;
  DevBuf otoff, otcode, otid, othit;
  DevBuf otsum;
  DevBuf big;
  DevBuf refbits;
  bool refbits_valid = false;
  uint64_t refbits_key[6] = {0, 0, 0, 0, 0, 0};
  const struct hawk_xplan* vplan = nullptr;
  DevBuf vcnt0;
  DevBuf refhp;
  uint64_t cs_tcap = 0;
  DevBuf cs_res, cs_tbase, cs_trows, cs_itb, cs_icnt;
  DevBuf cmini[8], cm_gid;
  DevBuf colsA[8];
  DevBuf rowsA;
  uint64_t rows_cap = 0;
  DevBuf crep[8];
};

struct hawk_xplan {
  hawk_ctx* ctx;
  uint32_t n_var, n_hap, ref_len;
  uint64_t ncar;
  std::vector<uint32_t> hap_len;
  uint32_t* ref_plane[4];
  uint32_t ref_S;
  DevBuf ref5[HAWK_PLANES];
  DevBuf recs, tiles, codes, off, hlen, hash;
  DevBuf heads;
  bool has_meta;
  std::vector<int32_t> scan_start, scan_stop;
  DevBuf m_is_ref, m_ss, m_se, m_seg_off, m_seg_rel, m_seg_gen, m_tile;
  uint32_t nseg, bph, S;
  int32_t ref_index;
  int64_t ref_startp, min_gen, max_gen;
  bool has_partner = false;
  int32_t partner_start = 0, partner_stop = 0;
  uint32_t n_ref_rows = 0;
  std::vector<int64_t> rev0, rev1;
  std::shared_ptr<uint64_t> groups = std::make_shared<uint64_t>(0);
  struct {
    bool built = false, usable = false;
    uint32_t n_inst = 0, n_uniq = 0;
    uint32_t n_real = 0;
    uint32_t last_uniq = 0;
    uint64_t slots = 0;
    uint32_t status = 0;
    float build_ms = 0.f;
    DevBuf inst_uid, inst_o, inst_row, inst_pa, inst_rb, u_rec, u_n, u_row, u_o, u_seg;
  } cl;
};

struct hawk_gt {
  hawk_ctx* ctx;
  uint64_t n_lines;
  uint32_t n_samples, n_var;
  uint8_t* d_codes;
  uint8_t* d_flags;
  uint64_t n_entries;
  uint64_t* d_col_off; uint32_t* d_idx; int32_t* d_o; int64_t* d_delta;
  uint64_t n_indel = 0;
  uint32_t* d_indel = nullptr;
  uint64_t* d_ioff = nullptr;
  std::vector<uint64_t> h_off, h_ioff;
  std::vector<int64_t> h_delta;
};

struct hawk_table {
  hawk_hapset* hs;
  hawk_ctx* ctx;
  uint64_t n_rows, n_cand, n_hits, cap;
  GuideCols cols;
  uint32_t guidelen, pamlen, right;
  uint64_t n_groups;
  bool collapsed;
  uint64_t gen;
  DevBuf own[8];
  bool by_cluster = false;
  uint32_t plane_tiles = 0;
  uint64_t t_rows = 0;
};
inline bool hawk_table_stale(const hawk_table* t) { return t->hs && t->gen != t->hs->cols_gen; }

int hawk_reserve_cols(DevBuf (&b)[8], uint64_t cap, GuideCols* c);

int hapset_create_impl(hawk_ctx* ctx, uint32_t n_hap, const uint32_t* hap_len, bool zero_planes, hawk_hapset** out, bool alloc_planes = true);
HapSetDev make_dev(const hawk_hapset* hs);
int make_scan_params(const hawk_hapset* hs, uint64_t pam_fwd, uint64_t pam_rev, uint32_t pamlen, uint32_t guidelen,
                            uint32_t right, bool need_v, ScanParams* sp);
int meta_build(uint32_t n, const std::vector<uint32_t>& hap_len, uint32_t bph, const uint8_t* is_ref, const int32_t* scan_start,
                      const int32_t* scan_stop, const uint32_t* seg_off, const uint32_t* seg_rel, const int64_t* seg_gen,
                      int32_t ref_index, std::vector<TileMeta>* t0, int64_t* min_gen, int64_t* max_gen);
```

Measured before the change: 560.3 billion.

## Defer cluster dictionary build resolution and search speculatively on device-side counts

The cluster dictionary build no longer synchronizes on the host to read its results. It leaves a pending job, records events and has the device write its true counts into a small buffer. Search then launches speculatively using upper bounds for instance and unique counts, and the kernels read the true counts on device and exit early. Resolution happens at the first readback; if the speculative pass turns out invalid (a table retry or an unusable dictionary), the search is rerun. This removes a host-device round trip between plan build and search, at the cost of oversized launches, bound-sized reservations and a possible extra search pass.

```diff
diff --git a/crispr-hawk_amd/csrc/hawk_api_collapse.hip b/crispr-hawk_amd/csrc/hawk_api_collapse.hip
--- a/crispr-hawk_amd/csrc/hawk_api_collapse.hip
+++ b/crispr-hawk_amd/csrc/hawk_api_collapse.hip
@@ -153,6 +153,7 @@
   hawk_ctx* ctx = hs->ctx;
   HIPCHK(hipSetDevice(ctx->device));
   const hawk_xplan* vx = hs->vplan;
+  if (vx) { const int rr = hawk_xplan_resolve(const_cast<hawk_xplan*>(vx)); if (rr) return rr; }
   if (!vx || !vx->cl.usable) return HAWK_E_INVALID;
   const uint64_t n = t->n_rows;
   if (n > 0xffffffffull) return HAWK_E_UNSUPPORTED;
diff --git a/crispr-hawk_amd/csrc/hawk_api_search.hip b/crispr-hawk_amd/csrc/hawk_api_search.hip
--- a/crispr-hawk_amd/csrc/hawk_api_search.hip
+++ b/crispr-hawk_amd/csrc/hawk_api_search.hip
@@ -26,11 +26,13 @@
 extern "C" {
 
 #define HAWK_RETRY_TEMPLATES (-100)
+#define HAWK_RETRY_RESOLVED (-101)
 static int hawk_search_once(hawk_hapset* hs, const hawk_search_params* p, hawk_table** out, hawk_timing* timing);
 int hawk_search(hawk_hapset* hs, const hawk_search_params* p, hawk_table** out, hawk_timing* timing) {
   int rc = hawk_search_once(hs, p, out, timing);
+  if (rc == HAWK_RETRY_RESOLVED) rc = hawk_search_once(hs, p, out, timing);
   if (rc == HAWK_RETRY_TEMPLATES) rc = hawk_search_once(hs, p, out, timing);
-  return rc == HAWK_RETRY_TEMPLATES ? HAWK_E_CAPACITY : rc;
+  return rc == HAWK_RETRY_TEMPLATES || rc == HAWK_RETRY_RESOLVED ? HAWK_E_CAPACITY : rc;
 }
 static int hawk_search_once(hawk_hapset* hs, const hawk_search_params* p, hawk_table** out, hawk_timing* timing) {
   if (!hs || !p || !out || !hs->has_meta) return HAWK_E_INVALID;
@@ -44,9 +46,18 @@
   const HapSetDev d = make_dev(hs);
   ++hs->cols_gen;
   const uint64_t ntile = (uint64_t)hs->n_hap * sp.bph;
-  bool by_cluster = hs->vplan && hs->vplan->cl.built && hs->vplan->cl.usable && hs->ref_index == 0;
-  if (by_cluster) { const char* e = getenv("HAWK_VIEW_SEARCH"); if (e && e[0] == 'w') by_cluster = false; }
-  const uint64_t nscan = by_cluster ? (uint64_t)sp.bph + ((uint64_t)hs->vplan->cl.n_inst + 63) / 64 : ntile;
+  hawk_xplan* const vplan = const_cast<hawk_xplan*>(hs->vplan);
+  const bool cl_wanted = [&]() {
+    if (!vplan || hs->ref_index != 0 || hs->n_hap >= HAWK_ROW_MAX_HAP) return false;
+    const char* e = getenv("HAWK_VIEW_SEARCH");
+    return !(e && e[0] == 'w');
+  }();
+  if (vplan && vplan->cl.pending && !cl_wanted && (rc = hawk_xplan_resolve(vplan))) return rc;
+  const bool speculative = vplan && vplan->cl.pending;
+  const bool by_cluster = cl_wanted && vplan->cl.built && (speculative || vplan->cl.usable);
+  const uint32_t cl_n_inst = by_cluster ? (speculative ? vplan->cl.inst_bound : vplan->cl.n_inst) : 0u;
+  const uint32_t cl_n_uniq = by_cluster ? (speculative ? vplan->cl.u_bound : vplan->cl.n_uniq) : 0u;
+  const uint64_t nscan = by_cluster ? (uint64_t)sp.bph + ((uint64_t)cl_n_inst + 63) / 64 : ntile;
   if ((rc = hs->counts.reserve(nscan * 4)) || (rc = hs->offsets.reserve((nscan + 1) * 8)) ||
       (rc = hs->misc.reserve(512 * 8 + 64)) ||
       (rc = hs->cfd.reserve(336 * 8)) || (rc = hs->partial.reserve((nscan / 1024 + 2) * 8)))
@@ -127,17 +138,18 @@
   uint64_t tcap = 0, t_rows_used = 0;
   if (by_cluster) {
     const auto& cl = vx->cl;
-    cd.n_inst = cl.n_inst; cd.n_uniq = cl.n_uniq;
+    cd.n_inst = cl_n_inst; cd.n_uniq = cl_n_uniq;
+    cd.dev = speculative ? cl.dev.as<uint32_t>() : nullptr;
     cd.inst_uid = cl.inst_uid.as<uint32_t>(); cd.inst_o = cl.inst_o.as<int32_t>(); cd.inst_row = cl.inst_row.as<uint32_t>();
     cd.inst_pa = cl.inst_pa.as<int32_t>(); cd.inst_rb = cl.inst_rb.as<int32_t>();
     cd.u_rec = cl.u_rec.as<uint32_t>(); cd.u_n = cl.u_n.as<uint32_t>(); cd.u_row = cl.u_row.as<uint32_t>(); cd.u_o = cl.u_o.as<int32_t>();
     cd.u_seg = cl.u_seg.as<uint32_t>();
     const char* e0 = getenv("HAWK_CLUSTER_ROWS0");
-    const uint64_t first = e0 ? strtoull(e0, nullptr, 10) : 16ull * cl.n_uniq + 65536;
-    tcap = std::max<uint64_t>(std::min<uint64_t>(cl.slots, std::max<uint64_t>(hs->cs_tcap, first)), 1);
-    if ((rc = hs->cs_res.reserve((size_t)std::max<uint32_t>(cl.n_uniq, 1) * 32)) || (rc = hs->cs_tbase.reserve((size_t)std::max<uint32_t>(cl.n_uniq, 1) * 4)) ||
-        (rc = hs->cs_trows.reserve((size_t)tcap * hawk_cs_row_bytes())) || (rc = hs->cs_itb.reserve((size_t)std::max<uint32_t>(cl.n_inst, 1) * 4)) ||
-        (rc = hs->cs_icnt.reserve((size_t)std::max<uint32_t>(cl.n_inst, 1) * 4)))
+    const uint64_t first = e0 ? strtoull(e0, nullptr, 10) : 16ull * cl_n_uniq + 65536;
+    tcap = std::max<uint64_t>(std::min<uint64_t>(speculative ? ~0ull : cl.slots, std::max<uint64_t>(hs->cs_tcap, first)), 1);
+    if ((rc = hs->cs_res.reserve((size_t)std::max<uint32_t>(cl_n_uniq, 1) * 32)) || (rc = hs->cs_tbase.reserve((size_t)std::max<uint32_t>(cl_n_uniq, 1) * 4)) ||
+        (rc = hs->cs_trows.reserve((size_t)tcap * hawk_cs_row_bytes())) || (rc = hs->cs_itb.reserve((size_t)std::max<uint32_t>(cl_n_inst, 1) * 4)) ||
+        (rc = hs->cs_icnt.reserve((size_t)std::max<uint32_t>(cl_n_inst, 1) * 4)))
       return rc;
   }
   uint32_t* const d_counts_v = hs->counts.as<uint32_t>() + plane_tiles;
@@ -202,6 +214,12 @@
   auto read_block = [&]() -> int {
     HIPCHK(hipMemcpyAsync(h_block, d_block, 64, hipMemcpyDeviceToHost, ctx->stream));
     HIPCHK(hipStreamSynchronize(ctx->stream));
+    if (speculative) {
+      const bool repeat = (vplan->cl.h_res[4] & 8u) != 0, searched = vplan->cl.h_res[5] != 0;
+      const int r = hawk_xplan_resolve(vplan, true);
+      if (r) return r;
+      if (repeat || !searched || !vplan->cl.usable) return HAWK_RETRY_RESOLVED;
+    }
     memcpy(&tot, h_block + 32, sizeof(tot));
     memcpy(&status, h_block, 4);
     if (!by_cluster) return HAWK_OK;
diff --git a/crispr-hawk_amd/csrc/hawk_api_xplan.hip b/crispr-hawk_amd/csrc/hawk_api_xplan.hip
--- a/crispr-hawk_amd/csrc/hawk_api_xplan.hip
+++ b/crispr-hawk_amd/csrc/hawk_api_xplan.hip
@@ -6,6 +6,7 @@
 #include <cstdlib>
 #include <cstring>
 #include <map>
+#include <memory>
 #include <mutex>
 #include <new>
 #include <unordered_map>
@@ -13,12 +14,30 @@
 
 #include "hawk_host.h"
 
+struct hawk_cl_build {
+  PoolScope tmp;
+  uint64_t max_slots = 0;
+  double min_share = 0.0;
+  uint32_t n_var = 0, ch_bound = 0, inst_bound = 0, tsize = 0;
+  size_t z_counters = 0, z_cnt = 0, z_claim = 0, z_span2 = 0, z_tab = 0;
+  char* d_zero = nullptr;
+  uint32_t *d_status = nullptr, *d_counters = nullptr, *d_claim = nullptr;
+  unsigned long long* d_results = nullptr;
+  void *d_vdesc = nullptr, *d_list = nullptr;
+  uint32_t *d_ch_off = nullptr, *d_ch_row = nullptr, *d_base = nullptr, *d_lbase = nullptr, *d_state = nullptr;
+};
+
 extern "C" {
 
 void hawk_xplan_destroy(hawk_xplan* x) {
   if (!x) return;
   (void)hipSetDevice(x->ctx->device);
   (void)hipStreamSynchronize(x->ctx->stream);
+  delete x->cl.job;
+  x->cl.job = nullptr; x->cl.pending = false;
+  for (auto& e : x->cl.ev) if (e) (void)hipEventDestroy(e);
+  if (x->cl.h_res) (void)hipHostFree(x->cl.h_res);
+  x->cl.dev.release();
   for (auto& p : x->ref_plane) hawk_pool_free(p);
   for (auto& b : x->ref5) b.release();
   DevBuf* bufs[] = {&x->recs, &x->heads, &x->tiles, &x->codes, &x->off, &x->hlen, &x->hash,
@@ -173,6 +192,42 @@
   return HAWK_OK;
 }
 
+
+static int cl_pass(hawk_xplan* x, hawk_cl_build& j, uint32_t tsz, uint32_t max_probe, uint32_t fail_bit, bool first) {
+  auto& cl = x->cl;
+  hipStream_t st = x->ctx->stream;
+  const uint32_t n = x->n_hap, n_var = j.n_var, inst_bound = j.inst_bound;
+  const uint32_t u_bound = n_var + std::min<uint32_t>(tsz, inst_bound);
+  uint32_t* d_span2 = reinterpret_cast<uint32_t*>(j.d_zero + j.z_span2);
+  void* d_tab = j.d_zero + j.z_tab;
+  if (!first) {
+    TEMPCHK(j.tmp, &d_span2, (size_t)u_bound * 4);
+    TEMPCHK(j.tmp, &d_tab, (size_t)tsz * hawk_cl_slot_bytes());
+    HIPCHK(hipMemsetAsync(d_tab, 0, (size_t)tsz * hawk_cl_slot_bytes(), st));
+    HIPCHK(hipMemsetAsync(d_span2, 0, (size_t)u_bound * 4, st));
+    HIPCHK(hipMemsetAsync(j.d_zero + j.z_counters, 0, j.z_cnt - j.z_counters, st));
+    HIPCHK(hipMemsetAsync(j.d_zero + j.z_claim, 0, j.z_span2 - j.z_claim, st));
+  }
+  int rc;
+  if ((rc = cl.u_rec.reserve((size_t)u_bound * 4)) || (rc = cl.u_n.reserve((size_t)u_bound * 4)) || (rc = cl.u_row.reserve((size_t)u_bound * 4)) ||
+      (rc = cl.u_o.reserve((size_t)u_bound * 4)) || (rc = cl.u_seg.reserve((size_t)u_bound * 4)))
+    return rc;
+  cl.u_bound = u_bound;
+  uint32_t* const t_uid = cl.inst_uid.as<uint32_t>();
+  uint32_t* const t_row = cl.inst_row.as<uint32_t>();
+  hawk_launch_cl_fill(st, x->heads.p, x->off.as<uint64_t>(), x->hlen.as<uint32_t>(), x->m_ss.as<int32_t>(), x->m_se.as<int32_t>(), n, j.d_ch_off, j.d_ch_row,
+                      j.ch_bound, j.d_base, j.d_lbase, cl.inst_o.as<int32_t>(), t_row, cl.inst_pa.as<int32_t>(), cl.inst_rb.as<int32_t>(), t_uid, j.d_vdesc,
+                      j.d_claim, n_var, j.d_list, j.d_status);
+  hawk_launch_cl_finish(st, inst_bound, j.d_base + j.ch_bound, j.d_lbase + j.ch_bound, j.d_counters, j.d_results, n_var, u_bound, d_tab, tsz - 1, max_probe, fail_bit,
+                        j.d_list, j.d_state, j.d_vdesc, x->heads.p, t_uid, t_row, x->m_seg_off.as<uint32_t>(), x->m_seg_rel.as<uint32_t>(),
+                        cl.u_rec.as<uint32_t>(), cl.u_n.as<uint32_t>(), cl.u_row.as<uint32_t>(), cl.u_o.as<int32_t>(), cl.u_seg.as<uint32_t>(), d_span2,
+                        j.d_status, inst_bound, j.max_slots, j.min_share, cl.dev.as<uint32_t>());
+  HIPCHK(hipMemcpyAsync(cl.h_res, j.d_results, 64, hipMemcpyDeviceToHost, st));
+  HIPCHK(hipEventRecord(cl.ev[1], st));
+  HIPCHK(hipGetLastError());
+  return HAWK_OK;
+}
+
 static int xplan_build_dict(hawk_xplan* x) {
   auto& cl = x->cl;
   if (cl.built) return HAWK_OK;
@@ -180,113 +235,113 @@
   hawk_ctx* ctx = x->ctx;
   hipStream_t st = ctx->stream;
   const uint32_t n = x->n_hap;
-  if (x->ncar == 0 || x->ncar >= (1ull << 32) - 2 || n < 2) { cl.status = 4; return HAWK_OK; }
-  PoolScope tmp;
-  const uint32_t n_var = x->n_var;
-  const uint32_t ch_bound = hawk_cl_chunk_bound(x->ncar, n);
-  const uint32_t inst_bound = (uint32_t)x->ncar + n;
+  if (x->ncar == 0 || x->ncar >= (1ull << 32) - 2 || x->ncar + n >= (1ull << 32) || n < 2) { cl.status = 4; return HAWK_OK; }
+  if (!cl.ev[0]) HIPCHK(hipEventCreate(&cl.ev[0]));
+  if (!cl.ev[1]) HIPCHK(hipEventCreate(&cl.ev[1]));
+  if (!cl.h_res) HIPCHK(hipHostMalloc(reinterpret_cast<void**>(&cl.h_res), 64, hipHostMallocDefault));
+  int rc;
+  if ((rc = cl.dev.reserve(16))) return rc;
+  std::unique_ptr<hawk_cl_build> job(new (std::nothrow) hawk_cl_build());
+  if (!job) return HAWK_E_INVALID;
+  hawk_cl_build& j = *job;
+  const char* e1 = getenv("HAWK_CLUSTER_MAX_SLOTS");
+  const char* e2 = getenv("HAWK_CLUSTER_MIN_SHARE");
+  j.max_slots = e1 ? strtoull(e1, nullptr, 10) : (1ull << 27);
+  j.min_share = e2 ? atof(e2) : 3.0;
+  const uint32_t n_var = j.n_var = x->n_var;
+  const uint32_t ch_bound = j.ch_bound = hawk_cl_chunk_bound(x->ncar, n);
+  const uint32_t inst_bound = j.inst_bound = (uint32_t)x->ncar + n;
   const uint32_t bm_words = n_var / 32 + 1;
   uint32_t tsize = 1024;
   while (tsize < 2u * inst_bound && tsize < (1u << 30)) tsize <<= 1;
   uint32_t tsmall = std::min<uint32_t>(1u << 16, tsize);
   { const uint64_t expect = cl.last_uniq ? (uint64_t)cl.last_uniq * 2 : (uint64_t)inst_bound / 8; while (tsmall < expect && tsmall < tsize) tsmall <<= 1; }
+  j.tsize = tsize;
   const uint32_t u_bound0 = n_var + std::min<uint32_t>(tsmall, inst_bound);
   auto up = [](size_t v) { return (v + 255) & ~(size_t)255; };
   const size_t z_status = 0, z_counters = 256, z_results = 512, z_cnt = 768,
                z_claim = z_cnt + up(((size_t)ch_bound + 4) * 8), z_vdesc = z_claim + up((size_t)bm_words * 4),
                z_span2 = z_vdesc + up((size_t)std::max<uint32_t>(n_var, 1) * 8), z_tab = z_span2 + up((size_t)u_bound0 * 4),
                z_end = z_tab + (size_t)tsmall * hawk_cl_slot_bytes();
-  char* d_zero;
-  TEMPCHK(tmp, &d_zero, z_end);
-  uint32_t* const d_status = reinterpret_cast<uint32_t*>(d_zero + z_status);
-  uint32_t* const d_counters = reinterpret_cast<uint32_t*>(d_zero + z_counters);
-  unsigned long long* const d_results = reinterpret_cast<unsigned long long*>(d_zero + z_results);
+  j.z_counters = z_counters; j.z_cnt = z_cnt; j.z_claim = z_claim; j.z_span2 = z_span2; j.z_tab = z_tab;
+  TEMPCHK(j.tmp, &j.d_zero, z_end);
+  char* const d_zero = j.d_zero;
+  j.d_status = reinterpret_cast<uint32_t*>(d_zero + z_status);
+  j.d_counters = reinterpret_cast<uint32_t*>(d_zero + z_counters);
+  j.d_results = reinterpret_cast<unsigned long long*>(d_zero + z_results);
   uint32_t* const d_cnt = reinterpret_cast<uint32_t*>(d_zero + z_cnt);
   uint32_t* const d_lcnt = d_cnt + ((ch_bound + 3) & ~3u);
-  uint32_t* const d_claim = reinterpret_cast<uint32_t*>(d_zero + z_claim);
-  void* const d_vdesc = d_zero + z_vdesc;
-  uint32_t *d_ch_off, *d_ch_row, *d_base, *d_lbase, *d_state;
-  void* d_list;
-  TEMPCHK(tmp, &d_ch_off, (size_t)(n + 1) * 4);
-  TEMPCHK(tmp, &d_ch_row, (size_t)ch_bound * 4);
-  TEMPCHK(tmp, &d_base, (size_t)(ch_bound + 1) * 4);
-  TEMPCHK(tmp, &d_lbase, (size_t)(ch_bound + 1) * 4);
-  TEMPCHK(tmp, &d_list, (size_t)inst_bound * hawk_cl_listed_bytes());
-  TEMPCHK(tmp, &d_state, (size_t)inst_bound * 4);
-  int rc;
+  j.d_claim = reinterpret_cast<uint32_t*>(d_zero + z_claim);
+  j.d_vdesc = d_zero + z_vdesc;
+  TEMPCHK(j.tmp, &j.d_ch_off, (size_t)(n + 1) * 4);
+  TEMPCHK(j.tmp, &j.d_ch_row, (size_t)ch_bound * 4);
+  TEMPCHK(j.tmp, &j.d_base, (size_t)(ch_bound + 1) * 4);
+  TEMPCHK(j.tmp, &j.d_lbase, (size_t)(ch_bound + 1) * 4);
+  TEMPCHK(j.tmp, &j.d_list, (size_t)inst_bound * hawk_cl_listed_bytes());
+  TEMPCHK(j.tmp, &j.d_state, (size_t)inst_bound * 4);
   if ((rc = cl.inst_uid.reserve((size_t)inst_bound * 4)) || (rc = cl.inst_o.reserve((size_t)inst_bound * 4)) ||
       (rc = cl.inst_row.reserve((size_t)inst_bound * 4)) || (rc = cl.inst_pa.reserve((size_t)inst_bound * 4)) ||
       (rc = cl.inst_rb.reserve((size_t)inst_bound * 4)))
     return rc;
-  uint32_t* const t_uid = cl.inst_uid.as<uint32_t>();
-  uint32_t* const t_row = cl.inst_row.as<uint32_t>();
-  int32_t* const t_o = cl.inst_o.as<int32_t>();
-  int32_t* const t_pa = cl.inst_pa.as<int32_t>();
-  int32_t* const t_rb = cl.inst_rb.as<int32_t>();
-  HIPCHK(hipEventRecord(ctx->ev[8], st));
+  cl.inst_bound = inst_bound;
+  HIPCHK(hipEventRecord(cl.ev[0], st));
   HIPCHK(hipMemsetAsync(d_zero, 0, z_end, st));
-  hawk_launch_cl_chunks(st, x->off.as<uint64_t>(), x->m_is_ref.as<uint8_t>(), x->m_ss.as<int32_t>(), x->m_se.as<int32_t>(), n, d_ch_off, d_ch_row);
-  hawk_launch_cl_count(st, x->heads.p, x->off.as<uint64_t>(), x->hlen.as<uint32_t>(), x->m_ss.as<int32_t>(), x->m_se.as<int32_t>(), d_ch_off, d_ch_row, n,
+  hawk_launch_cl_chunks(st, x->off.as<uint64_t>(), x->m_is_ref.as<uint8_t>(), x->m_ss.as<int32_t>(), x->m_se.as<int32_t>(), n, j.d_ch_off, j.d_ch_row);
+  hawk_launch_cl_count(st, x->heads.p, x->off.as<uint64_t>(), x->hlen.as<uint32_t>(), x->m_ss.as<int32_t>(), x->m_se.as<int32_t>(), j.d_ch_off, j.d_ch_row, n,
                        n_var, ch_bound, d_cnt, d_lcnt);
-  hawk_launch_scan2_u32(st, d_cnt, d_lcnt, ch_bound, d_base, d_lbase);
-  const uint32_t* const d_n_inst = d_base + ch_bound;
-  const uint32_t* const d_n_list = d_lbase + ch_bound;
-  unsigned long long res[8] = {0, 0, 0, 0, 0, 0, 0, 0};
+  hawk_launch_scan2_u32(st, d_cnt, d_lcnt, ch_bound, j.d_base, j.d_lbase);
+  if ((rc = cl_pass(x, j, tsmall, tsmall < tsize ? 64u : 0xffffffffu, tsmall < tsize ? 8u : 2u, true))) return rc;
+  cl.job = job.release();
+  cl.pending = true;
+  return HAWK_OK;
+}
+
+}
+
+int hawk_xplan_resolve(hawk_xplan* x, bool synced) {
+  auto& cl = x->cl;
+  if (!cl.pending) return HAWK_OK;
+  std::unique_ptr<hawk_cl_build> job(cl.job);
+  cl.job = nullptr; cl.pending = false;
+  hawk_cl_build& j = *job;
+  hawk_ctx* ctx = x->ctx;
+  hipStream_t st = ctx->stream;
+  HIPCHK(hipSetDevice(ctx->device));
+  if (!synced) HIPCHK(hipStreamSynchronize(st));
+  HIPCHK(hipGetLastError());
   uint32_t status = 0, n_inst = 0, n_uniq = 0, n_real = 0;
-  auto pass = [&](uint32_t tsz, uint32_t max_probe, uint32_t fail_bit, bool first) -> int {
-    const uint32_t u_bound = n_var + std::min<uint32_t>(tsz, inst_bound);
-    uint32_t* d_span2 = reinterpret_cast<uint32_t*>(d_zero + z_span2);
-    void* d_tab = d_zero + z_tab;
-    if (!first) {
-      TEMPCHK(tmp, &d_span2, (size_t)u_bound * 4);
-      TEMPCHK(tmp, &d_tab, (size_t)tsz * hawk_cl_slot_bytes());
-      HIPCHK(hipMemsetAsync(d_tab, 0, (size_t)tsz * hawk_cl_slot_bytes(), st));
-      HIPCHK(hipMemsetAsync(d_span2, 0, (size_t)u_bound * 4, st));
-      HIPCHK(hipMemsetAsync(d_zero + z_counters, 0, z_cnt - z_counters, st));
-      HIPCHK(hipMemsetAsync(d_zero + z_claim, 0, z_span2 - z_claim, st));
-    }
-    int rc2;
-    if ((rc2 = cl.u_rec.reserve((size_t)u_bound * 4)) || (rc2 = cl.u_n.reserve((size_t)u_bound * 4)) || (rc2 = cl.u_row.reserve((size_t)u_bound * 4)) ||
-        (rc2 = cl.u_o.reserve((size_t)u_bound * 4)) || (rc2 = cl.u_seg.reserve((size_t)u_bound * 4)))
-      return rc2;
-    hawk_launch_cl_fill(st, x->heads.p, x->off.as<uint64_t>(), x->hlen.as<uint32_t>(), x->m_ss.as<int32_t>(), x->m_se.as<int32_t>(), n, d_ch_off, d_ch_row,
-                        ch_bound, d_base, d_lbase, t_o, t_row, t_pa, t_rb, t_uid, d_vdesc, d_claim, n_var, d_list, d_status);
-    hawk_launch_cl_finish(st, inst_bound, d_n_inst, d_n_list, d_counters, d_results, n_var, u_bound, d_tab, tsz - 1, max_probe, fail_bit, d_list, d_state, d_vdesc, x->heads.p,
-                          t_uid, t_row, x->m_seg_off.as<uint32_t>(), x->m_seg_rel.as<uint32_t>(), cl.u_rec.as<uint32_t>(), cl.u_n.as<uint32_t>(),
-                          cl.u_row.as<uint32_t>(), cl.u_o.as<int32_t>(), cl.u_seg.as<uint32_t>(), d_span2, d_status);
-    HIPCHK(hipMemcpyAsync(res, d_results, 64, hipMemcpyDeviceToHost, st));
-    HIPCHK(hipEventRecord(ctx->ev[9], st));
+  const unsigned long long* res = cl.h_res;
+  auto decode = [&]() {
+    n_inst = (uint32_t)res[0]; status = (uint32_t)res[4];
+    n_uniq = std::min<uint32_t>(j.n_var + (uint32_t)res[1], cl.u_bound);
+    n_real = (uint32_t)(res[1] + res[2]);
+  };
+  decode();
+  if (status & 8u) {
+    status &= ~8u;
+    HIPCHK(hipMemcpyAsync(j.d_status, &status, 4, hipMemcpyHostToDevice, st));
+    int rc = cl_pass(x, j, j.tsize, 0xffffffffu, 2u, false);
+    if (rc) return rc;
     HIPCHK(hipStreamSynchronize(st));
     HIPCHK(hipGetLastError());
-    n_inst = (uint32_t)res[0]; status = (uint32_t)res[4];
-    n_uniq = std::min<uint32_t>(n_var + (uint32_t)res[1], u_bound);
-    n_real = (uint32_t)(res[1] + res[2]);
-    return HAWK_OK;
-  };
-  if ((rc = pass(tsmall, tsmall < tsize ? 64u : 0xffffffffu, tsmall < tsize ? 8u : 2u, true))) return rc;
-  if (status & 8u) {
-    status &= ~8u;
-    HIPCHK(hipMemcpyAsync(d_status, &status, 4, hipMemcpyHostToDevice, st));
-    if ((rc = pass(tsize, 0xffffffffu, 2u, false))) return rc;
+    decode();
   }
   if (n_inst == 0) { cl.status = 4; return HAWK_OK; }
-  if (n_inst > inst_bound) { snprintf(hawk_hip_err_buf(), 256, "hawk_xplan_view: instance count beyond its bound"); return HAWK_E_HIP; }
+  if (n_inst > j.inst_bound) { snprintf(hawk_hip_err_buf(), 256, "hawk_xplan_view: instance count beyond its bound"); return HAWK_E_HIP; }
   cl.n_inst = n_inst; cl.n_uniq = n_uniq; cl.n_real = n_real; cl.last_uniq = (uint32_t)res[1];
-  (void)hipEventElapsedTime(&cl.build_ms, ctx->ev[8], ctx->ev[9]);
+  (void)hipEventElapsedTime(&cl.build_ms, cl.ev[0], cl.ev[1]);
   cl.slots = n_uniq ? res[3] : 0;
   cl.status = status;
-  const char* e1 = getenv("HAWK_CLUSTER_MAX_SLOTS");
-  const char* e2 = getenv("HAWK_CLUSTER_MIN_SHARE");
-  const uint64_t max_slots = e1 ? strtoull(e1, nullptr, 10) : (1ull << 27);
-  const double min_share = e2 ? atof(e2) : 3.0;
-  if (!status && (cl.slots > max_slots || (double)n_inst < min_share * (double)std::max<uint32_t>(n_real, 1))) cl.status = 4;
+  if (!status && (cl.slots > j.max_slots || (double)n_inst < j.min_share * (double)std::max<uint32_t>(n_real, 1))) cl.status = 4;
   cl.usable = cl.status == 0;
   return HAWK_OK;
 }
 
+extern "C" {
 int hawk_xplan_cluster_stats(const hawk_xplan* x, uint32_t* usable, uint32_t* n_instances, uint32_t* n_distinct, uint64_t* template_slots,
                              float* build_ms, uint32_t* status) {
   if (!x) return HAWK_E_INVALID;
+  { const int rc = hawk_xplan_resolve(const_cast<hawk_xplan*>(x)); if (rc) return rc; }
   if (usable) *usable = x->cl.built && x->cl.usable ? 1u : 0u;
   if (n_instances) *n_instances = x->cl.n_inst;
   if (n_distinct) *n_distinct = x->cl.n_real;
@@ -299,6 +354,7 @@
 int hawk_xplan_cluster_rebuild(hawk_xplan* x) {
   if (!x || !x->has_meta || x->ref_index != 0) return HAWK_E_INVALID;
   HIPCHK(hipSetDevice(x->ctx->device));
+  { const int rc = hawk_xplan_resolve(x); if (rc) return rc; }
   x->cl.built = false;
   return xplan_build_dict(x);
 }
@@ -428,6 +484,7 @@
   if (!x || !scan_start || !scan_stop || !x->nseg) return HAWK_E_INVALID;
   hawk_ctx* ctx = x->ctx;
   HIPCHK(hipSetDevice(ctx->device));
+  { const int rc = hawk_xplan_resolve(x); if (rc) return rc; }
   const uint32_t n = x->n_hap;
   for (uint32_t h = 0; h < n; ++h)
     if (scan_start[h] < 0 || scan_stop[h] > (int32_t)x->hap_len[h]) return HAWK_E_INVALID;
diff --git a/crispr-hawk_amd/csrc/hawk_csearch.hip b/crispr-hawk_amd/csrc/hawk_csearch.hip
--- a/crispr-hawk_amd/csrc/hawk_csearch.hip
+++ b/crispr-hawk_amd/csrc/hawk_csearch.hip
@@ -406,8 +406,16 @@
   }
 }
 __global__ void k_cl_results(const uint32_t* __restrict__ n_inst, const uint32_t* __restrict__ counters, const unsigned long long* __restrict__ slots_total,
-                             const uint32_t* __restrict__ status, unsigned long long* __restrict__ out) {
-  out[0] = *n_inst; out[1] = counters[0]; out[2] = counters[1]; out[3] = *slots_total; out[4] = *status;
+                             const uint32_t* __restrict__ status, unsigned long long* __restrict__ out, uint32_t n_var, uint32_t u_cap,
+                             uint32_t inst_bound, unsigned long long max_slots, double min_share, uint32_t* __restrict__ dict_dev) {
+  const uint32_t ni = *n_inst, nt = counters[0], nv = counters[1], st = *status;
+  const unsigned long long sl = *slots_total;
+  out[0] = ni; out[1] = nt; out[2] = nv; out[3] = sl; out[4] = st;
+  const uint32_t nu = n_var + nt < u_cap ? n_var + nt : u_cap, n_real = nt + nv;
+  const bool usable = st == 0u && ni != 0u && ni <= inst_bound && (nu ? sl : 0ull) <= max_slots &&
+                      !((double)ni < min_share * (double)(n_real > 1u ? n_real : 1u));
+  dict_dev[0] = ni; dict_dev[1] = nu; dict_dev[2] = usable ? 1u : 0u;
+  out[5] = usable ? 1u : 0u;
 }
 __global__ __launch_bounds__(256) void k_cl_uid(const ClListed* __restrict__ cx_list, const uint32_t* __restrict__ n_list_dev, uint32_t t_end,
                                                 const uint32_t* __restrict__ cx_state, const ClSlot* __restrict__ tab, uint32_t* __restrict__ inst_uid,
@@ -498,7 +506,8 @@
                            unsigned long long* results, uint32_t n_var, uint32_t u_cap, void* tab,
                            uint32_t mask, uint32_t max_probe, uint32_t fail_bit, const void* cx_list, uint32_t* cx_state, const void* var_desc,
                            const void* recs, uint32_t* inst_uid, const uint32_t* inst_row, const uint32_t* seg_off, const uint32_t* seg_rel,
-                           uint32_t* u_rec, uint32_t* u_n, uint32_t* u_row, int32_t* u_o, uint32_t* u_seg, uint32_t* u_span2, uint32_t* status) {
+                           uint32_t* u_rec, uint32_t* u_n, uint32_t* u_row, int32_t* u_o, uint32_t* u_seg, uint32_t* u_span2, uint32_t* status,
+                           uint32_t inst_bound, uint64_t max_slots, double min_share, uint32_t* dict_dev) {
   ClUniq cu{u_rec, u_n, u_row, u_o, u_seg, u_span2};
   const uint32_t per = 256 * CL_UID_U;
   const uint32_t head = list_bound < 16 * CL_HEAD_LISTED ? 0u : CL_HEAD_LISTED;
@@ -514,9 +523,18 @@
   if (list_bound)
     hipLaunchKernelGGL(k_cl_uid, dim3((list_bound + per - 1) / per), dim3(256), 0, st, list, n_list_dev, list_bound, cx_state, static_cast<const ClSlot*>(tab),
                        inst_uid, cu, static_cast<const HxHead*>(recs), status);
-  hipLaunchKernelGGL(k_cl_results, dim3(1), dim3(1), 0, st, n_inst_dev, counters, reinterpret_cast<const unsigned long long*>(counters + 4), status, results);
-}
-
+  hipLaunchKernelGGL(k_cl_results, dim3(1), dim3(1), 0, st, n_inst_dev, counters, reinterpret_cast<const unsigned long long*>(counters + 4), status, results,
+                     n_var, u_cap, inst_bound, (unsigned long long)max_slots, min_share, dict_dev);
+}
+
+__device__ __forceinline__ void cl_true_counts(const ClDict& cd, uint32_t& n_inst, uint32_t& n_uniq) {
+  n_inst = cd.n_inst; n_uniq = cd.n_uniq;
+  if (cd.dev) {
+    const bool ok = cd.dev[2] != 0u;
+    n_inst = ok ? (cd.dev[0] < cd.n_inst ? cd.dev[0] : cd.n_inst) : 0u;
+    n_uniq = ok ? (cd.dev[1] < cd.n_uniq ? cd.dev[1] : cd.n_uniq) : 0u;
+  }
+}
 __device__ __forceinline__ VcRanges cs_ranges(const HapSetDev& hs, const ScanParams& p, uint32_t h) {
   VcRanges rg;
   const int ss = hs.scan_start[h], se = hs.scan_stop[h], haplen = (int)hs.hap_len[h];
@@ -551,13 +569,16 @@
   __shared__ uint32_t s_k[2][256];
   __shared__ uint32_t s_e[256];
   const uint32_t tid = threadIdx.x;
+  uint32_t n_inst_true, n_uniq_true;
+  cl_true_counts(cd, n_inst_true, n_uniq_true);
+  if (blockIdx.x * (256 / CS_G) >= n_uniq_true) return;
   if (gp.score_cfdon) for (uint32_t i = tid; i < 336; i += 256) s_cfd[i] = gp.cfd_mm[i];
   __syncthreads();
   const uint32_t gl = tid & (CS_G - 1);
   const uint32_t u = (blockIdx.x * 256 + tid) / CS_G;
-  const uint32_t nc_u = u < cd.n_uniq ? cd.u_n[u] : 0u;
+  const uint32_t nc_u = u < n_uniq_true ? cd.u_n[u] : 0u;
   const bool live = nc_u != 0u;
-  const bool hole = u < cd.n_uniq && !live;
+  const bool hole = u < n_uniq_true && !live;
   const HxVar* __restrict__ recs = static_cast<const HxVar*>(va.recs_);
   const uint32_t h = live ? cd.u_row[u] : 0u, r0 = live ? cd.u_rec[u] : 0u, nc = live ? nc_u : 1u;
   const uint32_t seg0 = live ? cd.u_seg[u] : hs.seg_off[0], seg_end = hs.seg_off[h + 1];
@@ -855,6 +876,15 @@
   __shared__ uint32_t s_red[256 / WAVE][2];
   const uint32_t i0 = blockIdx.x * (256 * CS_CNT_U) + threadIdx.x;
   const uint32_t lane = threadIdx.x & (WAVE - 1);
+  uint32_t n_inst, n_uniq;
+  cl_true_counts(cd, n_inst, n_uniq);
+  if (blockIdx.x * (256 * CS_CNT_U) >= n_inst) {
+    if (threadIdx.x < 4 * CS_CNT_U) {
+      const uint32_t iw = blockIdx.x * (256 * CS_CNT_U) + threadIdx.x * WAVE;
+      if (iw < cd.n_inst) group_counts[iw / WAVE] = 0u;
+    }
+    return;
+  }
   const bool ovf = *t_count > t_cap;
   uint32_t uid[CS_CNT_U], below[CS_CNT_U];
   int32_t paf[CS_CNT_U];
@@ -862,7 +892,7 @@
 #pragma unroll
   for (int u = 0; u < CS_CNT_U; ++u) {
     const uint32_t i = i0 + u * 256;
-    in[u] = i < cd.n_inst;
+    in[u] = i < n_inst;
     const uint32_t ic = in[u] ? i : 0u;
     uid[u] = cd.inst_uid[ic]; paf[u] = cd.inst_pa[ic];
     below[u] = CL_NONE;
@@ -874,7 +904,7 @@
   for (int u = 0; u < CS_CNT_U; ++u) {
     const bool has = in[u] && uid[u] != CL_NONE;
     r[u] = make_uint4(0u, 0u, 0u, 0u); r2[u] = r[u]; behind0[u] = 0u;
-    if (cd.n_uniq) {
+    if (n_uniq) {
       const uint32_t us = has ? uid[u] : 0u;
       r[u] = res[2 * us]; r2[u] = res[2 * us + 1];
       if (lane == 0 && below[u] != CL_NONE) behind0[u] = res[2 * below[u] + 1].z;
@@ -927,7 +957,7 @@
   __builtin_nontemporal_store(v.z, q + 2); __builtin_nontemporal_store(v.w, q + 3);
 }
 template <int NI, int CE_CH>
-__global__ __launch_bounds__(256) void k_cs_emit_rows(uint32_t n_inst, const uint32_t* __restrict__ inst_row, const int32_t* __restrict__ inst_o,
+__global__ __launch_bounds__(256) void k_cs_emit_rows(uint32_t n_inst_bound, const uint32_t* __restrict__ dict_dev, const uint32_t* __restrict__ inst_row, const int32_t* __restrict__ inst_o,
                                                       const uint32_t* __restrict__ counts, const uint32_t* __restrict__ inst_tb,
                                                       const CsRow* __restrict__ trows, const uint64_t* __restrict__ offsets,
                                                       const unsigned long long* __restrict__ t_count, uint64_t t_cap, uint4* __restrict__ rows,
@@ -940,6 +970,8 @@
   __shared__ uint32_t s_src[4][2][CE_CH], s_rh[4][2][CE_CH];
   __shared__ int32_t s_rdq[4][2][CE_CH];
   if (*t_count > t_cap) return;
+  uint32_t n_inst = n_inst_bound;
+  if (dict_dev) n_inst = dict_dev[2] ? (dict_dev[0] < n_inst_bound ? dict_dev[0] : n_inst_bound) : 0u;
   const uint32_t wv = threadIdx.x / WAVE, lane = threadIdx.x & (WAVE - 1);
   const uint32_t i0 = (blockIdx.x * 4 + wv) * NE;
   if (i0 >= n_inst) return;
@@ -1018,7 +1050,7 @@
                               const unsigned long long* t_count, uint64_t t_cap, void* rows, uint64_t cap, int* status) {
   if (!cd.n_inst) return;
   constexpr int NI = 4, CH = 256;
-  hipLaunchKernelGGL((k_cs_emit_rows<NI, CH>), dim3((cd.n_inst + 256 * NI - 1) / (256 * NI)), dim3(256), 0, st, cd.n_inst, cd.inst_row, cd.inst_o, counts,
+  hipLaunchKernelGGL((k_cs_emit_rows<NI, CH>), dim3((cd.n_inst + 256 * NI - 1) / (256 * NI)), dim3(256), 0, st, cd.n_inst, cd.dev, cd.inst_row, cd.inst_o, counts,
                      inst_tb, static_cast<const CsRow*>(trows), offsets, t_count, t_cap, static_cast<uint4*>(rows), cap, status);
 }
 
diff --git a/crispr-hawk_amd/csrc/hawk_device.h b/crispr-hawk_amd/csrc/hawk_device.h
--- a/crispr-hawk_amd/csrc/hawk_device.h
+++ b/crispr-hawk_amd/csrc/hawk_device.h
@@ -117,6 +117,7 @@
 void hawk_launch_ref_hits(hipStream_t st, const HapSetDev& hs, const ScanParams& p, int32_t ref_index, void* hp);
 struct ClDict {
   uint32_t n_inst, n_uniq;
+  const uint32_t* dev;
   const uint32_t* inst_uid;
   const int32_t* inst_o;
   const uint32_t* inst_row;
@@ -149,7 +150,8 @@
                            void* tab , uint32_t mask, uint32_t max_probe, uint32_t fail_bit, const void* cx_list, uint32_t* cx_state,
                            const void* var_desc, const void* recs, uint32_t* inst_uid, const uint32_t* inst_row, const uint32_t* seg_off,
                            const uint32_t* seg_rel, uint32_t* u_rec, uint32_t* u_n, uint32_t* u_row, int32_t* u_o, uint32_t* u_seg, uint32_t* u_span2,
-                           uint32_t* status);
+                           uint32_t* status, uint32_t inst_bound, uint64_t max_slots, double min_share,
+                           uint32_t* dict_dev );
 void hawk_launch_cs_templates(hipStream_t st, const HapSetDev& hs, const VcArgs& va, const ClDict& cd, const ScanParams& p, const struct GuideParams& gp,
                               const struct RefInfo& ri, void* res , uint32_t* tbase, void* trows,
                               unsigned long long* t_count, uint64_t t_cap, int* status);
diff --git a/crispr-hawk_amd/csrc/hawk_host.h b/crispr-hawk_amd/csrc/hawk_host.h
--- a/crispr-hawk_amd/csrc/hawk_host.h
+++ b/crispr-hawk_amd/csrc/hawk_host.h
@@ -145,8 +145,15 @@
     uint32_t status = 0;
     float build_ms = 0.f;
     DevBuf inst_uid, inst_o, inst_row, inst_pa, inst_rb, u_rec, u_n, u_row, u_o, u_seg;
+    bool pending = false;
+    struct hawk_cl_build* job = nullptr;
+    uint32_t inst_bound = 0, u_bound = 0;
+    DevBuf dev;
+    hipEvent_t ev[2] = {nullptr, nullptr};
+    unsigned long long* h_res = nullptr;
   } cl;
 };
+int hawk_xplan_resolve(hawk_xplan* x, bool synced = false);
 
 struct hawk_gt {
   hawk_ctx* ctx;
```

Measured after the change: 567.7 billion (median of 6 runs). 1.3% higher.
